# HybridRobotics/car-racing

Measured on AMD Instinct MI355X. Metric: NLP solves/sec (N=12, 6-state bicycle); p50 per-step solve latency, higher is better.
Workload: dtype f64

## Files before the change

car-racing_amd/csrc/crx_api.hip:

```cpp
#include <hip/hip_runtime.h>
#include <math.h>
#include <stdarg.h>
#include <stdio.h>
#include <string.h>

#include <dlfcn.h>

#include <chrono>
#include <mutex>
#include <vector>

#if __has_include(<rccl/rccl.h>)
#include <rccl/rccl.h>
#else
extern "C" {
typedef struct ncclComm* ncclComm_t;
typedef struct { char internal[128]; } ncclUniqueId;
typedef enum { ncclSuccess = 0 } ncclResult_t;
typedef enum { ncclInt8 = 0, ncclUint8 = 1, ncclInt32 = 2, ncclUint32 = 3, ncclInt64 = 4, ncclUint64 = 5, ncclFloat16 = 6, ncclFloat32 = 7, ncclFloat64 = 8 } ncclDataType_t;
}
#endif

#include "crx_kparams.h"

namespace {

thread_local char g_err[512] = "";
std::mutex g_mu;
int g_device = -1;
bool g_init = false;
hipStream_t g_stream = nullptr;

int fail(int code, const char* fmt, ...) {
    va_list ap;
    va_start(ap, fmt);
    vsnprintf(g_err, sizeof(g_err), fmt, ap);
    va_end(ap);
    return code;
}

#define HIP_TRY(expr)                                                                             \
    do {                                                                                          \
        hipError_t e_ = (expr);                                                                   \
        if (e_ != hipSuccess) return fail(CRX_ERR_HIP, "%s: %s", #expr, hipGetErrorString(e_));   \
    } while (0)

struct DevMem {
    static constexpr const char* name = "hipMalloc";
    static hipError_t alloc(void** p, size_t bytes) { return hipMalloc(p, bytes); }
    static hipError_t release(void* p) { return hipFree(p); }
};
struct PinMem {
    static constexpr const char* name = "hipHostMalloc";
    static hipError_t alloc(void** p, size_t bytes) { return hipHostMalloc(p, bytes, hipHostMallocDefault); }
    static hipError_t release(void* p) { return hipHostFree(p); }
};
template <typename Mem>
struct Buf {
    void* p = nullptr;
    size_t cap = 0;
    int ensure(size_t bytes) {
        if (bytes <= cap) return 0;
        release();
        size_t want = bytes + bytes / 2 + 256;
        hipError_t e = Mem::alloc(&p, want);
        if (e != hipSuccess) return fail(CRX_ERR_HIP, "%s(%zu): %s", Mem::name, want, hipGetErrorString(e));
        cap = want;
        return 0;
    }
    void release() {
        if (p) (void)Mem::release(p);
        p = nullptr;
        cap = 0;
    }
};
using DevBuf = Buf<DevMem>;
using PinBuf = Buf<PinMem>;
DevBuf g_in, g_out;
PinBuf g_hin, g_hout;
DevBuf g_trace;
int g_poison = 0;
int g_kkt_unscaled = 0;
int g_spec = 0;
int g_trace_rows = 0, g_trace_problem = 0;

int ensure_init() {
    if (g_init) return 0;
    return fail(CRX_ERR_NOT_INIT, "crx_init() has not been called (or failed)");
}

using arr = const void*;
template <typename... P>
bool any_null(const P*... p) { return (... || !p); }

struct Stage {
    enum Kind { IN, INOUT, OUT, SCRATCH };
    template <typename T>
    struct Ref { int i = -1; };
    struct Slot { Kind kind; const void* src; void* dst; size_t bytes, off; };
    static constexpr int MAX_SLOTS = 24;
    Slot slots[MAX_SLOTS];
    int n = 0;
    bool overrun = false;
    size_t end[4] = {0, 0, 0, 0};

    template <typename T>
    Ref<T> add(Kind kind, const T* src, T* dst, size_t count) {
        if (n == MAX_SLOTS) { overrun = true; return {}; }
        slots[n] = Slot{kind, src, dst, count * sizeof(T), 0};
        return Ref<T>{n++};
    }
    template <typename T>
    Ref<T> in(const T* src, size_t count) { return add(IN, src, (T*)nullptr, count); }
    template <typename T>
    Ref<T> out(T* host, size_t count) { return add(OUT, (const T*)nullptr, host, count); }
    template <typename T>
    Ref<T> inout(T* host, size_t count) { return add(INOUT, (const T*)host, host, count); }
    Ref<char> scratch(size_t bytes) { return add(SCRATCH, (const char*)nullptr, (char*)nullptr, bytes); }
    template <typename T>
    T* operator[](Ref<T> r) const {
        return r.i < 0 ? nullptr : (T*)((char*)(slots[r.i].kind == IN ? g_in.p : g_out.p) + slots[r.i].off);
    }

    int up(hipStream_t st) {
        if (overrun) return fail(CRX_ERR_ARG, "internal: more than %d staged arrays in one call", MAX_SLOTS);
        size_t cur = 0;
        for (int k = IN; k <= SCRATCH; k++) {
            if (k == INOUT) cur = 0;
            for (int i = 0; i < n; i++)
                if (slots[i].kind == k) {
                    slots[i].off = cur = (cur + 255) & ~size_t(255);
                    cur += slots[i].bytes;
                }
            end[k] = cur;
        }
        if (int rc = g_in.ensure(end[IN])) return rc;
        if (int rc = g_hin.ensure(end[IN])) return rc;
        if (int rc = g_out.ensure(end[SCRATCH])) return rc;
        if (int rc = g_hout.ensure(end[OUT])) return rc;
        for (int i = 0; i < n; i++) {
            const Slot& s = slots[i];
            if (s.kind > INOUT || !s.bytes) continue;
            char* pin = (char*)(s.kind == IN ? g_hin.p : g_hout.p) + s.off;
            if (s.src) memcpy(pin, s.src, s.bytes); else memset(pin, 0, s.bytes);
        }
        if (end[IN]) HIP_TRY(hipMemcpyAsync(g_in.p, g_hin.p, end[IN], hipMemcpyHostToDevice, st));
        if (end[INOUT]) HIP_TRY(hipMemcpyAsync(g_out.p, g_hout.p, end[INOUT], hipMemcpyHostToDevice, st));
        return 0;
    }
    int down(hipStream_t st) {
        if (end[OUT]) HIP_TRY(hipMemcpyAsync(g_hout.p, g_out.p, end[OUT], hipMemcpyDeviceToHost, st));
        HIP_TRY(hipStreamSynchronize(st));
        for (int i = 0; i < n; i++)
            if (slots[i].dst && slots[i].bytes) memcpy(slots[i].dst, (char*)g_hout.p + slots[i].off, slots[i].bytes);
        return 0;
    }
};

int check_opts(const crx_ipm_opts& o) {
    if (!(o.tol > 0) || o.max_iter < 1 || !(o.mu_init > 0) || !(o.tau_min > 0 && o.tau_min < 1) ||
        !(o.slack_push > 0) || !(o.kappa_mu > 0 && o.kappa_mu < 1) || !(o.theta_mu > 1) || !(o.grad_scale_max > 0) ||
        o.slack_start < 0 || o.slack_start > 3 || !(o.dual_inf_tol > 0) || !(o.constr_viol_tol > 0) || !(o.compl_inf_tol > 0) || o.stall_iters < 1 || o.qp_method < 0 || o.qp_method > 1)
        return fail(CRX_ERR_ARG, "invalid crx_ipm_opts (a descriptor built for libcrx <= 0.3.x? crx_ipm_opts grew in 0.2 and in 0.4: include/crx.h)");
    return 0;
}

void reach_bound(const double* A, const double* B, double delta_max, double a_max, int row, int n, double* gain, double (*rows)[6]) {
    double w[6] = {0, 0, 0, 0, 0, 0}, acc = 0.0;
    w[row] = 1.0;
    gain[0] = 0.0;
    if (rows) memcpy(rows[0], w, sizeof(w));
    for (int j = 1; j <= n; j++) {
        double v0 = 0.0, v1 = 0.0, wn[6] = {0, 0, 0, 0, 0, 0};
        for (int i = 0; i < 6; i++) { v0 += w[i] * B[i * 2]; v1 += w[i] * B[i * 2 + 1]; }
        acc += fabs(v0) * delta_max + fabs(v1) * a_max;
        gain[j] = acc;
        for (int a = 0; a < 6; a++)
            for (int i = 0; i < 6; i++) wn[a] += w[i] * A[i * 6 + a];
        memcpy(w, wn, sizeof(w));
        if (rows) memcpy(rows[j], w, sizeof(w));
    }
}

int fill_planner(crx_kparams& kp, const crx_planner_desc* d, int batch) {
    if (!d) return fail(CRX_ERR_ARG, "desc is NULL");
    if (d->N < 3 || d->N > CRX_MAX_N) return fail(CRX_ERR_ARG, "N=%d outside [3,%d]", d->N, CRX_MAX_N);
    if (batch < 0) return fail(CRX_ERR_ARG, "batch < 0");
    if (int rc = check_opts(d->opts)) return rc;
    memset(&kp, 0, sizeof(kp));
    kp.N = d->N; kp.batch = batch; kp.mode = 0; kp.n_obs_max = 0; kp.degree = 6;
    memcpy(kp.A, d->A, sizeof(kp.A)); memcpy(kp.B, d->B, sizeof(kp.B));
    kp.wq[4] = d->w_ref; kp.wq[5] = d->w_ref;
    kp.w_dey = d->w_dey; kp.w_prog = d->w_prog; kp.w_slack = 0.0;
    kp.delta_max = d->delta_max; kp.a_max = d->a_max; kp.v_min = -INFINITY; kp.v_max = d->vx_max; kp.ey_max = INFINITY;
    kp.alpha = 0.0; kp.margin = 0.0; kp.l_sum = 1.0; kp.w_sum = 1.0;
    kp.dt_ref = d->dt_ref; kp.fallback_gain = d->fallback_gain; kp.opts = d->opts;
    kp.reach_screen = d->opts.reach_screen ? 1 : 0;
    reach_bound(d->A, d->B, d->delta_max, d->a_max, 5, d->N - 1, kp.reach_gain, kp.reach_row);
    return 0;
}

int fill_cbf(crx_kparams& kp, const crx_cbf_desc* d, int batch) {
    if (!d) return fail(CRX_ERR_ARG, "desc is NULL");
    if (d->N < 3 || d->N > CRX_MAX_N) return fail(CRX_ERR_ARG, "N=%d outside [3,%d]", d->N, CRX_MAX_N);
    if (d->n_obs_max < 0 || d->n_obs_max > CRX_MAX_OBS) return fail(CRX_ERR_ARG, "n_obs_max=%d outside [0,%d]", d->n_obs_max, CRX_MAX_OBS);
    if (d->degree < 2 || d->degree > 8 || (d->degree & 1)) return fail(CRX_ERR_ARG, "degree must be 2, 4, 6 or 8");
    if (batch < 0) return fail(CRX_ERR_ARG, "batch < 0");
    if (!(d->alpha > 0.0 && d->alpha <= 1.0)) return fail(CRX_ERR_ARG, "alpha outside (0,1]");
    if (int rc = check_opts(d->opts)) return rc;
    memset(&kp, 0, sizeof(kp));
    kp.N = d->N; kp.batch = batch; kp.mode = 1; kp.per_stage_target = d->per_stage_target ? 1 : 0;
    kp.n_obs_max = d->n_obs_max; kp.degree = d->degree;
    memcpy(kp.A, d->A, sizeof(kp.A)); memcpy(kp.B, d->B, sizeof(kp.B));
    memcpy(kp.wq, d->Q, sizeof(kp.wq)); kp.wr[0] = d->R[0]; kp.wr[1] = d->R[1];
    kp.w_dey = 0.0; kp.w_prog = 0.0; kp.w_slack = d->w_slack;
    kp.delta_max = d->delta_max; kp.a_max = d->a_max; kp.v_min = d->v_min; kp.v_max = d->v_max; kp.ey_max = d->ey_max;
    kp.alpha = d->alpha; kp.margin = d->margin; kp.l_sum = d->l_sum; kp.w_sum = d->w_sum;
    kp.dt_ref = 0.1; kp.fallback_gain = 1.1; kp.opts = d->opts;
    kp.slack_start = d->opts.slack_start;
    reach_bound(d->A, d->B, d->delta_max, d->a_max, 4, d->N, kp.reach_s, nullptr);
    reach_bound(d->A, d->B, d->delta_max, d->a_max, 5, d->N, kp.reach_gain, nullptr);
    return 0;
}

int launched(hipError_t e, const char* what) {
    return e == hipSuccess ? CRX_OK : fail(CRX_ERR_HIP, "%s launch: %s", what, hipGetErrorString(e));
}

void apply_diagnostics(crx_kparams& kp) {
    if (g_trace_rows != 0) { kp.trace = (double*)g_trace.p; kp.trace_problem = g_trace_problem; kp.trace_rows = g_trace_rows; }
    kp.poison = g_poison;
    kp.kkt_unscaled = g_kkt_unscaled;
}
void apply_diagnostics(crx_lmpc_kparams& kp) {
    if (g_trace_rows > 0) { kp.trace = (double*)g_trace.p; kp.trace_problem = g_trace_problem; kp.trace_rows = g_trace_rows; }
    kp.poison = g_poison;
}

int launch_solve(const crx_kparams& kp, int tmpl, hipStream_t st) {
    crx_kparams kq = kp;
    apply_diagnostics(kq);
    size_t lds = crx_solve_lds_bytes(kp.N, tmpl);
    if (lds > 160 * 1024) return fail(CRX_ERR_ARG, "N=%d with %d obstacles needs %zu B of LDS (> 160 KiB)", kp.N, tmpl, lds);
    const bool spec = tmpl == 1 && kq.mode == 1 && kq.degree == 6 && (kq.N == 12 || kq.N == 10) && g_spec > 0;
    kq.spec_idle = g_spec == 2;
    return launched(spec ? crx_launch_solve_spec(kq, st) : crx_launch_solve(kq, tmpl, st), "solver");
}

}

extern "C" {

int crx_version(void) { return CRX_VERSION; }

const char* crx_last_error(void) { return g_err; }

int crx_device_count(void) {
    int n = 0;
    if (hipGetDeviceCount(&n) != hipSuccess) return 0;
    return n;
}

int crx_init(int device) {
    std::lock_guard<std::mutex> lk(g_mu);
    int n = 0;
    hipError_t e = hipGetDeviceCount(&n);
    if (e != hipSuccess || n <= 0)
        return fail(CRX_ERR_NO_DEVICE, "no HIP device visible (%s); libcrx has no CPU back-end",
                    e == hipSuccess ? "count = 0" : hipGetErrorString(e));
    if (device < 0 || device >= n) return fail(CRX_ERR_ARG, "device %d outside [0,%d)", device, n);
    HIP_TRY(hipSetDevice(device));
    if (g_init && g_device == device) return CRX_OK;
    if (g_init && g_device >= 0) {
        (void)hipSetDevice(g_device);
        if (g_stream) { (void)hipStreamDestroy(g_stream); g_stream = nullptr; }
        g_in.release(); g_out.release(); g_hin.release(); g_hout.release(); g_trace.release();
        g_trace_rows = 0;
        HIP_TRY(hipSetDevice(device));
    }
    HIP_TRY(hipStreamCreateWithFlags(&g_stream, hipStreamNonBlocking));
    g_device = device;
    g_init = true;
    return CRX_OK;
}

void crx_shutdown(void) {
    std::lock_guard<std::mutex> lk(g_mu);
    if (!g_init) return;
    (void)hipSetDevice(g_device);
    g_in.release(); g_out.release(); g_hin.release(); g_hout.release(); g_trace.release();
    g_trace_rows = 0;
    if (g_stream) (void)hipStreamDestroy(g_stream);
    g_stream = nullptr;
    g_init = false; g_device = -1;
}

int crx_trace_enable(int problem, int rows) {
    if (int rc = ensure_init()) return rc;
    g_trace_rows = 0;
    const bool sub = rows < 0;
    if (rows < 0) rows = -rows;
    if (rows == 0) return CRX_OK;
    if (int rc = g_trace.ensure((size_t)rows * 16 * sizeof(double))) return rc;
    HIP_TRY(hipMemset(g_trace.p, 0, (size_t)rows * 16 * sizeof(double)));
    g_trace_rows = sub ? -rows : rows; g_trace_problem = problem;
    return CRX_OK;
}
int crx_trace_read(double* host, int rows) {
    { int cap = g_trace_rows < 0 ? -g_trace_rows : g_trace_rows; if (rows > cap) rows = cap; }
    HIP_TRY(hipDeviceSynchronize());
    HIP_TRY(hipMemcpy(host, g_trace.p, (size_t)rows * 16 * sizeof(double), hipMemcpyDeviceToHost));
    return CRX_OK;
}

void crx_debug_poison_lds(int enable) { g_poison = enable != 0; }

void crx_debug_speculation(int mode) { g_spec = mode < 0 ? 0 : (mode > 2 ? 1 : mode); }

void crx_debug_kkt_unscaled(int mode) { g_kkt_unscaled = (mode >= 0 && mode <= 4) ? mode : 0; }

int crx_debug_wave_reduce(const double* in, double* out) {
    if (int rc = ensure_init()) return rc;
    if (!in || !out) return fail(CRX_ERR_ARG, "NULL array argument");
    std::lock_guard<std::mutex> lk(g_mu);
    HIP_TRY(hipSetDevice(g_device));
    Stage sg;
    auto din = sg.in(in, 256);
    auto dout = sg.out(out, 208);
    if (int rc = sg.up(g_stream)) return rc;
    hipError_t e = crx_launch_debug_reduce(sg[din], sg[dout], g_stream);
    if (e != hipSuccess) return fail(CRX_ERR_HIP, "debug reduce launch: %s", hipGetErrorString(e));
    return sg.down(g_stream);
}

long crx_debug_lds_bytes(int kind, int N, int n) {
    return kind == 0 ? (long)crx_solve_lds_bytes(N, n) : (long)crx_lmpc_lds_bytes(N, n);
}

int crx_debug_resident_per_cu(int kind, int N, int n) {
    if (ensure_init() != CRX_OK) return -1;
    return kind == 0 ? crx_solve_resident_per_cu(N, n) : crx_lmpc_resident_per_cu(N, n);
}

struct CrxTimer { hipEvent_t e0, e1; bool armed; };

int crx_timer_create(void** timer) {
    if (int rc = ensure_init()) return rc;
    if (!timer) return fail(CRX_ERR_ARG, "timer is NULL");
    HIP_TRY(hipSetDevice(g_device));
    CrxTimer* t = new CrxTimer{nullptr, nullptr, false};
    if (hipEventCreate(&t->e0) != hipSuccess || hipEventCreate(&t->e1) != hipSuccess) {
        if (t->e0) (void)hipEventDestroy(t->e0);
        delete t;
        return fail(CRX_ERR_HIP, "hipEventCreate failed");
    }
    *timer = t;
    return CRX_OK;
}
int crx_timer_destroy(void* timer) {
    CrxTimer* t = (CrxTimer*)timer;
    if (!t) return CRX_OK;
    (void)hipEventDestroy(t->e0); (void)hipEventDestroy(t->e1);
    delete t;
    return CRX_OK;
}
int crx_timer_begin(void* timer, void* stream) {
    CrxTimer* t = (CrxTimer*)timer;
    if (!t) return fail(CRX_ERR_ARG, "timer is NULL");
    t->armed = false;
    HIP_TRY(hipEventRecord(t->e0, (hipStream_t)stream));
    return CRX_OK;
}
int crx_timer_end(void* timer, void* stream) {
    CrxTimer* t = (CrxTimer*)timer;
    if (!t) return fail(CRX_ERR_ARG, "timer is NULL");
    HIP_TRY(hipEventRecord(t->e1, (hipStream_t)stream));
    t->armed = true;
    return CRX_OK;
}
double crx_timer_ms(void* timer) {
    CrxTimer* t = (CrxTimer*)timer;
    if (!t || !t->armed) return -1.0;
    float ms = 0.f;
    if (hipEventSynchronize(t->e1) != hipSuccess) return -1.0;
    if (hipEventElapsedTime(&ms, t->e0, t->e1) != hipSuccess) return -1.0;
    return (double)ms;
}

void crx_ipm_opts_default(crx_ipm_opts* o) {
    o->tol = 1e-8; o->max_iter = 200; o->restore_iters = 50; o->mu_init = 0.1; o->kappa_eps = 10.0;
    o->kappa_mu = 0.2; o->theta_mu = 1.5; o->tau_min = 0.99; o->slack_push = 1e-2; o->grad_scale_max = 100.0;
    o->reach_screen = 1; o->slack_start = 2;
    o->dual_inf_tol = 1.0; o->constr_viol_tol = 1e-4; o->compl_inf_tol = 1e-4;
    o->stall_iters = 100; o->qp_method = 0;
}

void crx_planner_desc_default(crx_planner_desc* d, int N, const double* A, const double* B) {
    memset(d, 0, sizeof(*d));
    d->N = N;
    memcpy(d->A, A, sizeof(d->A)); memcpy(d->B, B, sizeof(d->B));
    d->w_ref = 20.0; d->w_dey = 30.0; d->w_prog = 200.0; d->vx_max = 5.0; d->delta_max = 0.5; d->a_max = 1.5;
    d->dt_ref = 0.1; d->fallback_gain = 1.1;
    crx_ipm_opts_default(&d->opts);
}

void crx_cbf_desc_default(crx_cbf_desc* d, int N, int n_obs_max, const double* A, const double* B) {
    memset(d, 0, sizeof(*d));
    d->N = N; d->n_obs_max = n_obs_max; d->per_stage_target = 0; d->degree = 6;
    memcpy(d->A, A, sizeof(d->A)); memcpy(d->B, B, sizeof(d->B));
    const double Q[6] = {10.0, 0.0, 0.0, 4.0, 0.0, 40.0};
    memcpy(d->Q, Q, sizeof(Q)); d->R[0] = 0.1; d->R[1] = 0.1;
    d->delta_max = 0.5; d->a_max = 1.0; d->v_min = 0.0; d->v_max = 10.0; d->ey_max = 1.0;
    d->alpha = 0.8; d->margin = 0.2; d->l_sum = 0.4; d->w_sum = 0.2; d->w_slack = 1e4;
    crx_ipm_opts_default(&d->opts);
    if (N <= 12 && n_obs_max <= 1) { d->opts.stall_iters = 50; d->opts.restore_iters = 25; }
}

void crx_select_desc_default(crx_select_desc* d, int N, int n_veh_max, double lap_length) {
    d->N = N; d->n_veh_max = n_veh_max; d->veh_length = 0.4; d->veh_width = 0.2; d->lap_length = lap_length;
    d->w_prog = 10.0; d->w_coll = 100.0; d->w_switch = 100.0;
}

static bool planner_null(arr x0, arr bez_s, arr bez_ey, arr ey_lb, arr ey_ub, arr X, arr U, arr cost, arr status, arr kkt, arr iters) {
    return any_null(x0, bez_s, bez_ey, ey_lb, ey_ub, X, U, cost, status, kkt, iters);
}

static int check_planner(crx_kparams& kp, const crx_planner_desc* d, int batch, arr x0, arr bez_s, arr bez_ey, arr ey_lb, arr ey_ub, arr X, arr U,
                         arr cost, arr status, arr kkt, arr iters) {
    if (int rc = ensure_init()) return rc;
    if (int rc = fill_planner(kp, d, batch)) return rc;
    if (batch > 0 && planner_null(x0, bez_s, bez_ey, ey_lb, ey_ub, X, U, cost, status, kkt, iters))
        return fail(CRX_ERR_ARG, "NULL array argument");
    return 0;
}

static int planner_solve_masked(const crx_planner_desc* d, int batch, const int32_t* active, int active_div, const double* x0,
                                const double* bez_s, const double* bez_ey, const double* ey_lb, const double* ey_ub, double* X,
                                double* U, double* cost, int32_t* status, double* kkt, int32_t* iters, void* stream);

int crx_planner_solve_dev(const crx_planner_desc* d, int batch, const double* x0, const double* bez_s,
                          const double* bez_ey, const double* ey_lb, const double* ey_ub, double* X, double* U,
                          double* cost, int32_t* status, double* kkt, int32_t* iters, void* stream) {
    return planner_solve_masked(d, batch, nullptr, 0, x0, bez_s, bez_ey, ey_lb, ey_ub, X, U, cost, status, kkt, iters, stream);
}

static int planner_solve_masked(const crx_planner_desc* d, int batch, const int32_t* active, int active_div, const double* x0,
                                const double* bez_s, const double* bez_ey, const double* ey_lb, const double* ey_ub, double* X,
                                double* U, double* cost, int32_t* status, double* kkt, int32_t* iters, void* stream) {
    crx_kparams kp;
    if (int rc = check_planner(kp, d, batch, x0, bez_s, bez_ey, ey_lb, ey_ub, X, U, cost, status, kkt, iters)) return rc;
    if (batch == 0) return CRX_OK;
    kp.x0 = x0; kp.bez_s = bez_s; kp.bez_ey = bez_ey; kp.ey_lb = ey_lb; kp.ey_ub = ey_ub;
    kp.X = X; kp.U = U; kp.sigma = nullptr; kp.cost = cost; kp.status = status; kp.kkt = kkt; kp.iters = iters;
    kp.active = active; kp.active_div = active_div;
    return launch_solve(kp, 0, (hipStream_t)stream);
}

int crx_planner_solve(const crx_planner_desc* d, int batch, const double* x0, const double* bez_s,
                      const double* bez_ey, const double* ey_lb, const double* ey_ub, double* X, double* U,
                      double* cost, int32_t* status, double* kkt, int32_t* iters) {
    crx_kparams chk;
    if (int rc = check_planner(chk, d, batch, x0, bez_s, bez_ey, ey_lb, ey_ub, X, U, cost, status, kkt, iters)) return rc;
    if (batch == 0) return CRX_OK;
    std::lock_guard<std::mutex> lk(g_mu);
    HIP_TRY(hipSetDevice(g_device));
    const size_t B = (size_t)batch, N = (size_t)d->N;
    Stage sg;
    auto dx0 = sg.in(x0, B * 6); auto dbs = sg.in(bez_s, B * (N + 1)); auto dbe = sg.in(bez_ey, B * (N + 1));
    auto dlb = sg.in(ey_lb, B * N); auto dub = sg.in(ey_ub, B);
    auto dX = sg.out(X, B * (N + 1) * 6); auto dU = sg.out(U, B * N * 2); auto dc = sg.out(cost, B);
    auto dk = sg.out(kkt, B); auto ds = sg.out(status, B); auto di = sg.out(iters, B);
    if (int rc = sg.up(g_stream)) return rc;
    if (int rc = crx_planner_solve_dev(d, batch, sg[dx0], sg[dbs], sg[dbe], sg[dlb], sg[dub], sg[dX], sg[dU], sg[dc], sg[ds], sg[dk],
                                       sg[di], g_stream)) return rc;
    return sg.down(g_stream);
}

int crx_cbf_solve_dev(const crx_cbf_desc* d, int batch, const double* x0, const double* xt, const double* obs_s,
                      const double* obs_ey, const double* lap_off, const int32_t* n_obs, double* X, double* U,
                      double* sigma, double* cost, int32_t* status, double* kkt, int32_t* iters, void* stream) {
    return crx_cbf_solve_masked_dev(d, batch, nullptr, x0, xt, obs_s, obs_ey, lap_off, n_obs, X, U, sigma, cost, status, kkt, iters, stream);
}

int crx_cbf_solve_masked_dev(const crx_cbf_desc* d, int batch, const int32_t* active, const double* x0, const double* xt,
                             const double* obs_s, const double* obs_ey, const double* lap_off, const int32_t* n_obs, double* X,
                             double* U, double* sigma, double* cost, int32_t* status, double* kkt, int32_t* iters, void* stream) {
    return crx_cbf_solve_ordered_dev(d, batch, active, nullptr, x0, xt, obs_s, obs_ey, lap_off, n_obs, nullptr, X, U, sigma, cost, status, kkt, iters, stream);
}

int crx_cbf_solve_dims_dev(const crx_cbf_desc* d, int batch, const int32_t* active, const double* x0, const double* xt,
                           const double* obs_s, const double* obs_ey, const double* lap_off, const int32_t* n_obs,
                           const double* obs_dims, double* X, double* U, double* sigma, double* cost, int32_t* status, double* kkt,
                           int32_t* iters, void* stream) {
    return crx_cbf_solve_ordered_dev(d, batch, active, nullptr, x0, xt, obs_s, obs_ey, lap_off, n_obs, obs_dims, X, U, sigma, cost, status, kkt, iters, stream);
}

static int check_cbf(crx_kparams& kp, const crx_cbf_desc* d, int batch, arr x0, arr xt, arr obs_s, arr obs_ey, arr lap_off, arr n_obs, arr X, arr U,
                     arr sigma, arr cost, arr status, arr kkt, arr iters) {
    if (int rc = ensure_init()) return rc;
    if (int rc = fill_cbf(kp, d, batch)) return rc;
    if (batch == 0) return 0;
    if (any_null(x0, xt, X, U, cost, status, kkt, iters)) return fail(CRX_ERR_ARG, "NULL array argument");
    if (d->n_obs_max > 0 && any_null(obs_s, obs_ey, lap_off, n_obs, sigma))
        return fail(CRX_ERR_ARG, "NULL obstacle array with n_obs_max > 0");
    return 0;
}

int crx_cbf_solve_ordered_dev(const crx_cbf_desc* d, int batch, const int32_t* active, const int32_t* order, const double* x0,
                              const double* xt, const double* obs_s, const double* obs_ey, const double* lap_off,
                              const int32_t* n_obs, const double* obs_dims, double* X, double* U, double* sigma, double* cost,
                              int32_t* status, double* kkt, int32_t* iters, void* stream) {
    crx_kparams kp;
    if (int rc = check_cbf(kp, d, batch, x0, xt, obs_s, obs_ey, lap_off, n_obs, X, U, sigma, cost, status, kkt, iters)) return rc;
    if (batch == 0) return CRX_OK;
    kp.x0 = x0; kp.xt = xt; kp.obs_s = obs_s; kp.obs_ey = obs_ey; kp.lap_off = lap_off; kp.n_obs = n_obs;
    kp.X = X; kp.U = U; kp.sigma = sigma; kp.cost = cost; kp.status = status; kp.kkt = kkt; kp.iters = iters;
    kp.active = active; kp.order = order; kp.obs_dims = d->n_obs_max > 0 ? obs_dims : nullptr;
    return launch_solve(kp, d->n_obs_max, (hipStream_t)stream);
}

int crx_cbf_solve(const crx_cbf_desc* d, int batch, const double* x0, const double* xt, const double* obs_s,
                  const double* obs_ey, const double* lap_off, const int32_t* n_obs, double* X, double* U,
                  double* sigma, double* cost, int32_t* status, double* kkt, int32_t* iters) {
    return crx_cbf_solve_dims(d, batch, x0, xt, obs_s, obs_ey, lap_off, n_obs, nullptr, X, U, sigma, cost, status, kkt, iters);
}

int crx_cbf_solve_dims(const crx_cbf_desc* d, int batch, const double* x0, const double* xt, const double* obs_s,
                  const double* obs_ey, const double* lap_off, const int32_t* n_obs, const double* obs_dims, double* X, double* U,
                  double* sigma, double* cost, int32_t* status, double* kkt, int32_t* iters) {
    crx_kparams chk;
    if (int rc = check_cbf(chk, d, batch, x0, xt, obs_s, obs_ey, lap_off, n_obs, X, U, sigma, cost, status, kkt, iters)) return rc;
    if (batch == 0) return CRX_OK;
    const size_t B = (size_t)batch, N = (size_t)d->N, V = (size_t)d->n_obs_max;
    if (V > 0) {
        for (size_t b = 0; b < B; b++)
            if (n_obs[b] < 0 || n_obs[b] > (int)V) return fail(CRX_ERR_ARG, "n_obs[%zu]=%d outside [0,%zu]", b, n_obs[b], V);
        if (obs_dims)
            for (size_t b = 0; b < B; b++)
                for (int o = 0; o < n_obs[b]; o++)
                    if (!(obs_dims[(b * V + o) * 2] > 0.0) || !(obs_dims[(b * V + o) * 2 + 1] > 0.0))
                        return fail(CRX_ERR_ARG, "obs_dims[%zu][%d] must be positive", b, o);
    }
    std::lock_guard<std::mutex> lk(g_mu);
    HIP_TRY(hipSetDevice(g_device));
    const size_t n_ob = B * V * (N + 1);
    Stage sg;
    auto dx0 = sg.in(x0, B * 6); auto dxt = sg.in(xt, d->per_stage_target ? B * (N + 1) * 6 : B * 6);
    auto dos = sg.in(obs_s, n_ob); auto doe = sg.in(obs_ey, n_ob); auto dlo = sg.in(lap_off, B * V);
    auto ddm = (obs_dims && V > 0) ? sg.in(obs_dims, B * V * 2) : Stage::Ref<double>{};
    auto dno = sg.in(V > 0 ? n_obs : (const int32_t*)nullptr, B);
    auto dX = sg.out(X, B * (N + 1) * 6); auto dU = sg.out(U, B * N * 2); auto dsg = sg.out(sigma, n_ob);
    auto dc = sg.out(cost, B); auto dk = sg.out(kkt, B); auto ds = sg.out(status, B); auto di = sg.out(iters, B);
    if (int rc = sg.up(g_stream)) return rc;
    if (int rc = crx_cbf_solve_dims_dev(d, batch, nullptr, sg[dx0], sg[dxt], sg[dos], sg[doe], sg[dlo], sg[dno], sg[ddm], sg[dX], sg[dU],
                                        sg[dsg], sg[dc], sg[ds], sg[dk], sg[di], g_stream)) return rc;
    return sg.down(g_stream);
}

static int check_select(const crx_select_desc* d, int n_scen) {
    if (!d) return fail(CRX_ERR_ARG, "desc is NULL");
    if (d->N < 1 || d->N > CRX_MAX_N || d->n_veh_max < 0 || d->n_veh_max > CRX_MAX_VEH || n_scen < 0)
        return fail(CRX_ERR_ARG, "bad selection dimensions");
    if (!(d->lap_length > 0.0) || !isfinite(d->lap_length)) return fail(CRX_ERR_ARG, "lap_length must be positive and finite");
    if (!(d->veh_length >= 0.0) || !(d->veh_width >= 0.0)) return fail(CRX_ERR_ARG, "vehicle dimensions must be non-negative");
    return 0;
}

static bool select_null(const crx_select_desc* d, arr n_veh, arr X, arr obs_s, arr obs_ey, arr old_flag, arr flag, arr sel_cost, arr best_X) {
    return any_null(n_veh, X, old_flag, flag, sel_cost, best_X) || (d->n_veh_max > 0 && any_null(obs_s, obs_ey));
}

static int check_select_call(const crx_select_desc* d, int n_scen, arr n_veh, arr X, arr obs_s, arr obs_ey, arr old_flag, arr flag, arr sel_cost,
                             arr best_X) {
    if (int rc = ensure_init()) return rc;
    if (int rc = check_select(d, n_scen)) return rc;
    if (n_scen > 0 && select_null(d, n_veh, X, obs_s, obs_ey, old_flag, flag, sel_cost, best_X)) return fail(CRX_ERR_ARG, "NULL array argument");
    return 0;
}

int crx_select_dev(const crx_select_desc* d, int n_scen, const int32_t* n_veh, const double* X, const double* obs_s,
                   const double* obs_ey, const int32_t* old_flag, int32_t* flag, double* sel_cost, double* best_X,
                   void* stream) {
    if (int rc = check_select_call(d, n_scen, n_veh, X, obs_s, obs_ey, old_flag, flag, sel_cost, best_X)) return rc;
    if (n_scen == 0) return CRX_OK;
    crx_select_kparams sp;
    sp.N = d->N; sp.V = d->n_veh_max; sp.n_scen = n_scen;
    sp.veh_length = d->veh_length; sp.veh_width = d->veh_width; sp.lap_length = d->lap_length;
    sp.w_prog = d->w_prog; sp.w_coll = d->w_coll; sp.w_switch = d->w_switch;
    sp.n_veh = n_veh; sp.X = X; sp.obs_s = obs_s; sp.obs_ey = obs_ey; sp.old_flag = old_flag;
    sp.flag = flag; sp.sel_cost = sel_cost; sp.best_X = best_X;
    return launched(crx_launch_select(sp, (hipStream_t)stream), "selection");
}

int crx_select(const crx_select_desc* d, int n_scen, const int32_t* n_veh, const double* X, const double* obs_s,
               const double* obs_ey, const int32_t* old_flag, int32_t* flag, double* sel_cost, double* best_X) {
    if (int rc = check_select_call(d, n_scen, n_veh, X, obs_s, obs_ey, old_flag, flag, sel_cost, best_X)) return rc;
    if (n_scen == 0) return CRX_OK;
    const size_t S = (size_t)n_scen, N = (size_t)d->N, V = (size_t)d->n_veh_max, R = V + 1;
    for (size_t s = 0; s < S; s++)
        if (n_veh[s] < 0 || n_veh[s] > (int)V) return fail(CRX_ERR_ARG, "n_veh[%zu]=%d outside [0,%zu]", s, n_veh[s], V);
    std::lock_guard<std::mutex> lk(g_mu);
    HIP_TRY(hipSetDevice(g_device));
    Stage sg;
    auto dX = sg.in(X, S * R * (N + 1) * 6); auto dos = sg.in(obs_s, S * V * (N + 1)); auto doe = sg.in(obs_ey, S * V * (N + 1));
    auto dnv = sg.in(n_veh, S); auto dof = sg.in(old_flag, S);
    auto dfl = sg.out(flag, S); auto dsc = sg.out(sel_cost, S * R); auto dbX = sg.out(best_X, S * (N + 1) * 6);
    if (int rc = sg.up(g_stream)) return rc;
    if (int rc = crx_select_dev(d, n_scen, sg[dnv], sg[dX], sg[dos], sg[doe], sg[dof], sg[dfl], sg[dsc], sg[dbX], g_stream)) return rc;
    return sg.down(g_stream);
}

void crx_path_desc_default(crx_path_desc* d, int N, double alpha) {
    memset(d, 0, sizeof(*d));
    d->N = N; d->alpha = alpha; d->w_rate = 100.0;
    crx_ipm_opts_default(&d->opts);
}

static int fill_path(crx_path_kparams& pp, const crx_path_desc* d, int batch) {
    if (!d) return fail(CRX_ERR_ARG, "desc is NULL");
    if (d->N < 2 || d->N > CRX_MAX_N) return fail(CRX_ERR_ARG, "N=%d outside [2,%d]", d->N, CRX_MAX_N);
    if (!(d->alpha >= 0.0 && d->alpha <= 1.0) || !(d->w_rate >= 0.0)) return fail(CRX_ERR_ARG, "alpha outside [0,1] or w_rate < 0");
    if (batch < 0) return fail(CRX_ERR_ARG, "batch < 0");
    if (int rc = check_opts(d->opts)) return rc;
    memset(&pp, 0, sizeof(pp));
    pp.N = d->N; pp.batch = batch; pp.alpha = d->alpha; pp.w_rate = d->w_rate; pp.opts = d->opts;
    return 0;
}

static int check_path(crx_path_kparams& pp, const crx_path_desc* d, int batch, arr opt, arr bez, arr lb, arr ub, arr e0, arr eN, arr E, arr cost,
                      arr status, arr kkt, arr iters) {
    if (int rc = ensure_init()) return rc;
    if (int rc = fill_path(pp, d, batch)) return rc;
    if (batch > 0 && any_null(opt, bez, lb, ub, e0, eN, E, cost, status, kkt, iters)) return fail(CRX_ERR_ARG, "NULL array argument");
    return 0;
}

int crx_path_solve_dev(const crx_path_desc* d, int batch, const double* opt, const double* bez, const double* lb,
                       const double* ub, const double* e0, const double* eN, double* E, double* cost, int32_t* status,
                       double* kkt, int32_t* iters, void* stream) {
    crx_path_kparams pp;
    if (int rc = check_path(pp, d, batch, opt, bez, lb, ub, e0, eN, E, cost, status, kkt, iters)) return rc;
    if (batch == 0) return CRX_OK;
    pp.opt = opt; pp.bez = bez; pp.lb = lb; pp.ub = ub; pp.e0 = e0; pp.eN = eN;
// ... 942 lines not shown
```

car-racing_amd/csrc/crx_kernels.hip:

```cpp
#include <hip/hip_runtime.h>
#include <math.h>
#include <stdint.h>
#include <type_traits>

#include "crx_kparams.h"
#include "crx_wave.h"
#include "crx_num.h"
#include "crx_ipm.h"

#ifndef CRX_TU_GENERAL
#define CRX_TU_GENERAL 0
#endif
#ifndef CRX_OPAQUE_LANE
#define CRX_OPAQUE_LANE 1
#endif
#ifndef CRX_STATIC_LDS
#define CRX_STATIC_LDS 1
#endif
#ifndef CRX_SWEEP_MASK
#define CRX_SWEEP_MASK 1
#endif
#ifndef CRX_SWEEP_LOCAL_LANE
#define CRX_SWEEP_LOCAL_LANE 1
#endif
#define MAXF 12

__device__ __forceinline__ double ipow_d(double a, int p) {
    const double a2 = a * a;
    const int h = p >> 1;
    double r = sel(p & 1, a, 1.0);
    r = sel(h >= 1, r * a2, r);
    r = sel(h >= 2, r * a2, r);
    r = sel(h >= 3, r * a2, r);
    r = sel(h >= 4, r * a2, r);
    asm volatile("" : "+v"(r));
    return r;
}

#define ROWS(j, jv, lane_, m_) _Pragma("unroll") for (int q_ = 0; q_ < (L::MR + WAVE - 1) / WAVE; q_++) \
    if (const bool jv = (lane_) + q_ * WAVE < (m_); true) if (const int j = jv ? (lane_) + q_ * WAVE : 0; true)

#define COORDS(e, ev, lane_, n_) _Pragma("unroll") for (int q_ = 0; q_ < (L::NV + WAVE - 1) / WAVE; q_++) \
    if (const bool ev = (lane_) + q_ * WAVE < (n_); true) if (const int e = ev ? (lane_) + q_ * WAVE : 0; true)

#define SINK(cond, off) seli((cond), (off), L::dmy)
#define CBF_ROWS(j, k, ob, ev, lane_, n_) _Pragma("unroll") for (int q_ = 0; q_ < (NMAX * NOBS + WAVE - 1) / WAVE; q_++) \
    if (const bool ev = (lane_) + q_ * WAVE < (n_) * NOBS; true) if (const int e_ = ev ? (lane_) + q_ * WAVE : 0; true) \
    if (const int k = e_ / L::NO; true) if (const int ob = e_ - k * L::NO; true) if (const int j = k * NR + 8 + NOBS + ob; true)
#define ROW_LOADS_DONE() do { if (NOBS == 0) __builtin_amdgcn_sched_barrier(0); } while (0)
#define ROW_IS_CBF(j, n_) (NOBS > 0 && (j) < (n_) * NR && (j) % NR >= 8 + NOBS)
#define LOADS_DONE() __builtin_amdgcn_sched_barrier(0)
#define STAGE_FENCE() __builtin_amdgcn_sched_barrier(0)

#define RIV_SIMPLE (1 << 13)
#define RIV_NEG (1 << 14)
#define RIV_IDX(pk) ((pk) & 0x1FFF)
#define RIV_SGN(pk) (((pk) & RIV_SIMPLE) ? (((pk) & RIV_NEG) ? -1.0 : 1.0) : 0.0)
#define SH16(si_) ((unsigned short*)((si_) + L::SH_OFF))
#define RIVT(si_, j) ((int)SH16(si_)[L::riv + (j)])
#define UPDP(si_, l_) ((int)SH16(si_)[L::updP + (l_)])
#define VROW(si_) ((typename L::vrow_t*)(SH16(si_) + L::END_S16))

template <int NOBS, int NMAX>
struct Lay {
    static constexpr int NX = 6 + NOBS, NU = 2 + NOBS, NZ = NX + NU, NR = 8 + 2 * NOBS;
    static constexpr int NO = NOBS ? NOBS : 1;
    static constexpr int MR = NMAX * NR + NOBS;
    static constexpr int NV = (NMAX + 1) * NZ;
    static constexpr int M = 0;
    static constexpr int Z = M + NX * NZ;
    static constexpr int dZ = Z + NV;
    static constexpr int xr = dZ + NV;
    static constexpr int wc = xr + (NMAX + 1) * 6;
    static constexpr int obs_s = wc + NMAX;
    static constexpr int obs_e = obs_s + NOBS * (NMAX + 1);
    static constexpr int rt = obs_e + NOBS * (NMAX + 1);
    static constexpr int rnu = rt + MR;
    static constexpr int rc = rnu + MR;
    static constexpr int rdt = rc + MR;
    static constexpr int rtt = rdt + MR;
    static constexpr bool SLIM = NOBS == 3 && NMAX == 20;
    static constexpr int MRS = SLIM ? 0 : MR;
    static constexpr int rsig = rtt + MR;
    static constexpr int rw = rsig + MRS;
    static constexpr int rsc = rw + MRS;
    static constexpr int csc = rsc + MRS;
    static constexpr int rb = csc + (SLIM ? NMAX * NOBS : 0);
    static constexpr int Gpos = rb + MRS;
    static constexpr int Hd = Gpos + (SLIM ? 0 : NMAX * NOBS * 4);
    static constexpr int hg = Hd + NV;
    static constexpr int ga = hg;
    static constexpr int Jc = hg + NV;
    static constexpr int kS = (Jc + NMAX * NOBS * NZ + 1) & ~1;
    static constexpr int kE = kS + 1;
    static constexpr int HS = NZ + 1;
    static constexpr int TS = NZ;
    static constexpr bool PT_ALIAS = NX * NX + NX + NX * TS <= MR, H_ALIAS = NZ * HS <= NV;
    static constexpr int WORK = kS + (NOBS ? 2 * NMAX : 0);
    static constexpr int P = PT_ALIAS ? rdt : WORK;
    static constexpr int pv = P + NX * NX;
    static constexpr int T = pv + NX;
    static constexpr int WORK2 = PT_ALIAS ? WORK : T + NX * TS;
    static constexpr int H = H_ALIAS ? dZ : WORK2;
    static constexpr int Kk = H_ALIAS ? WORK2 : H + NZ * HS;
    static constexpr int G = SLIM ? Kk : Gpos;
    static constexpr int sigS = (SLIM && H_ALIAS && NZ * HS + NMAX * NO <= NV) ? dZ + NZ * HS : -1;
    static_assert(NMAX * NOBS * 4 <= NMAX * NU * NX, "G fits inside Kk");
    static constexpr int kf = Kk + NMAX * NU * NX;
    static constexpr int Fth = kf + NMAX * NU;
    static constexpr int Fph = Fth + MAXF;
    static constexpr int cst = Fph + MAXF;
    static constexpr int dmy = cst + 16 + 2 * NOBS;
    static constexpr int END_D = dmy + 2;
    static constexpr int triH = 0;
    static constexpr int END_I = triH + ((NZ * NZ <= WAVE || SLIM) ? 0 : NZ * (NZ + 1) / 2);
    static constexpr int SH_OFF = (END_I + 1) & ~1;
    static constexpr int riv = 0;
    static constexpr int updP = riv + MR;
    static constexpr int UCNT = (NX * (NX + 1) / 2 + NX + NX + 1 + WAVE - 1) / WAVE;
    static constexpr int END_S16 = (updP + 64 * UCNT + 1) & ~1;
    using vrow_t = std::conditional_t<(MR <= 127), signed char, short>;
    static constexpr int vlo = 0;
    static constexpr int vhi = vlo + NV;
    static constexpr int END_V = SLIM ? 0 : vhi + NV;
    static constexpr size_t BYTES = (size_t)END_D * 8 + (size_t)SH_OFF * 4 + (size_t)END_S16 * 2 + (((size_t)END_V * sizeof(vrow_t) + 7) & ~(size_t)7);
    static_assert(!SLIM || BYTES <= 40960, "the slim layout exists to fit four problems per CU (160 KB / 4)");
    static constexpr int R2 = (int)((BYTES + 15) / 16) * 2;
    static constexpr int P2 = R2, pv2 = P2 + NX * NX, T2 = pv2 + NX, H2 = (T2 + NX * TS + 1) & ~1, Kk2 = H2 + NZ * HS, kf2 = Kk2 + NMAX * NU * NX,
                         dZ2 = kf2 + NMAX * NU, ctl = dZ2 + NZ, R2_END = ctl + 4;
    static constexpr size_t BYTES_SPEC = (size_t)R2_END * 8;
};

struct Ctx {
    int N, lane, nobs, m;
    double lin_sN, cconst, wsig, alpha, om, cm;
    int degree;
    double b_d, b_a, b_vlo, b_vhi, b_e;
};

template <class L>
__device__ __forceinline__ double row_scale(const double* sm, const int* si, int j, int N) {
    if constexpr (L::SLIM) {
        const bool cbf = j < N * L::NR && j % L::NR >= 8 + L::NO;
        const int k = j / L::NR, ob = j - k * L::NR - 8 - L::NO;
        const double cs = sm[L::csc + seli(cbf, k * L::NO + ob, 0)];
        return sel(cbf, cs, sel((RIVT(si, j) & RIV_SIMPLE) != 0, 1.0, 0.0));
    } else {
        return sm[L::rsc + j];
    }
}
template <class L>
__device__ __forceinline__ double cbf_scale(const double* sm, int k, int ob) {
    if constexpr (L::SLIM) return sm[L::csc + k * L::NO + ob];
    else return sm[L::rsc + k * L::NR + 8 + L::NO + ob];
}
template <class L>
__device__ __forceinline__ double row_bound(const double* sm, const Ctx& c, int j) {
    if constexpr (L::SLIM) {
        const int r = j < c.N * L::NR ? j % L::NR : 8;
        const double ub = sel(r < 2, c.b_d, c.b_a) * sel((r & 1) != 0, 1.0, -1.0);
        const double xb = sel(r == 4, c.b_vlo, sel(r == 5, c.b_vhi, sel(r == 6, -c.b_e, c.b_e)));
        return sel(r < 4, ub, sel(r < 8, xb, 0.0));
    } else {
        return sm[L::rb + j];
    }
}
template <class L>
__device__ __forceinline__ void row_sig_w(const double* sm, int j, bool on, double mu, double t, double nu, double rti, double cj,
                                          double& sig, double& w) {
    if constexpr (L::SLIM) {
        const double sg = nu * rti;
        sig = sel(on, sg, 0.0);
        w = sel(on, nu - mu * rti + sg * (cj - t), 0.0);
    } else {
        sig = sm[L::rsig + j];
        w = sm[L::rw + j];
    }
}
template <class L>
__device__ __forceinline__ void coord_rows(const int* si, const Ctx& c, int e, int k, int a, int& rl, int& rh) {
    if constexpr (L::SLIM) {
        constexpr int NX = L::NX, NR = L::NR;
        const int N = c.N;
        const bool isx = a < 6, iss0 = a >= 6 && a < NX, isu = a >= NX && a < NX + 2;
        const bool xb = isx && k >= 1 && (a == 0 || a == 5);
        int jl = seli(xb, (k - 1) * NR + seli(a == 0, 4, 6), -1);
        jl = seli(iss0 && k == 0, N * NR + (a - 6), jl);
        jl = seli(isu && k < N, k * NR + 2 * (a - NX), jl);
        jl = seli(a >= NX + 2 && k < N, k * NR + 8 + (a - NX - 2), jl);
        const int jh = seli(xb || (isu && k < N), jl + 1, -1);
        rl = seli(jl >= 0 && (RIVT(si, seli(jl >= 0, jl, 0)) & RIV_SIMPLE) != 0, jl, -1);
        rh = seli(jh >= 0 && (RIVT(si, seli(jh >= 0, jh, 0)) & RIV_SIMPLE) != 0, jh, -1);
    } else {
        rl = VROW(si)[L::vlo + e];
        rh = VROW(si)[L::vhi + e];
    }
}
__device__ __forceinline__ void tri_decode(int e, int& r, int& a) {
    int q = (int)((__builtin_sqrtf(8.0f * (float)e + 1.0f) - 1.0f) * 0.5f);
    q += ((q + 1) * (q + 2) / 2 <= e) ? 1 : 0;
    q -= (q * (q + 1) / 2 > e) ? 1 : 0;
    r = q; a = e - q * (q + 1) / 2;
}

#define LD(off) sm[(off)]
#ifndef CRX_ROWDPP
#define CRX_ROWDPP 1
#endif
template <class L> constexpr bool ROWDPP = CRX_ROWDPP && L::NZ <= 16;

#ifdef CRX_PHASE_CLOCKS
#define CLK() clock64()
#else
#define CLK() 0LL
#endif

template <int NOBS, int NMAX>
__device__ __forceinline__ void cbf_dist(const double* sm, const Ctx& c, int k, int o, double al, double& dsc,
                                         double& dec, double& dsn, double& den) {
    using L = Lay<NOBS, NMAX>;
    const int N1 = c.N + 1;
    const double sc = LD(L::Z + k * L::NZ + 4) + al * LD(L::dZ + k * L::NZ + 4);
    const double ec = LD(L::Z + k * L::NZ + 5) + al * LD(L::dZ + k * L::NZ + 5);
    const double sn = LD(L::Z + (k + 1) * L::NZ + 4) + al * LD(L::dZ + (k + 1) * L::NZ + 4);
    const double en = LD(L::Z + (k + 1) * L::NZ + 5) + al * LD(L::dZ + (k + 1) * L::NZ + 5);
    const double rLs = LD(L::cst + 16 + o), rWs = LD(L::cst + 16 + L::NO + o);
    dsc = (sc - LD(L::obs_s + o * N1 + k) - LD(L::cst + 8 + o)) * rLs;
    dec = (ec - LD(L::obs_e + o * N1 + k)) * rWs;
    dsn = (sn - LD(L::obs_s + o * N1 + k + 1)) * rLs;
    den = (en - LD(L::obs_e + o * N1 + k + 1)) * rWs;
}

template <int NOBS, int NMAX>
__device__ __forceinline__ double cbf_value(const double* sm, const Ctx& c, int k, int o, double al) {
    using L = Lay<NOBS, NMAX>;
    double dsc, dec, dsn, den;
    cbf_dist<NOBS, NMAX>(sm, c, k, o, al, dsc, dec, dsn, den);
    const int q = c.degree;
    const double gc = ipow_d(dsc, q) + ipow_d(dec, q), gn = ipow_d(dsn, q) + ipow_d(den, q);
    const double sk = LD(L::Z + k * L::NZ + 6 + o) + al * LD(L::dZ + k * L::NZ + 6 + o);
    const double sk1 = LD(L::Z + k * L::NZ + L::NX + 2 + o) + al * LD(L::dZ + k * L::NZ + L::NX + 2 + o);
    return gn - sk1 - c.om * (gc - sk) - c.alpha * c.cm;
}

template <int NOBS, int NMAX>
__device__ __forceinline__ double cost_value(const double* sm, const Ctx& c, double al) {
    using L = Lay<NOBS, NMAX>;
    const int N = c.N;
    double acc = 0.0;
    for (int e = c.lane; e < (N + 1) * 6; e += WAVE) {
        const int k = e / 6, i = e - k * 6;
        const double v = LD(L::Z + k * L::NZ + i) + al * LD(L::dZ + k * L::NZ + i);
        const double d = v - LD(L::xr + e);
        acc += LD(L::cst + i) * d * d;
        if (k == N && i == 4) acc += c.lin_sN * v;
    }
    for (int e = c.lane; e < N * 2; e += WAVE) {
        const int k = e >> 1, i = e & 1;
        const double v = LD(L::Z + k * L::NZ + L::NX + i) + al * LD(L::dZ + k * L::NZ + L::NX + i);
        acc += LD(L::cst + 6 + i) * v * v;
    }
    for (int k = c.lane; k < N; k += WAVE) {
        const double wck = LD(L::wc + k);
        const double e1 = LD(L::Z + (k + 1) * L::NZ + 5) + al * LD(L::dZ + (k + 1) * L::NZ + 5);
        const double e0 = LD(L::Z + k * L::NZ + 5) + al * LD(L::dZ + k * L::NZ + 5);
        acc += wck * (e1 - e0) * (e1 - e0);
    }
    if (NOBS) {
        for (int e = c.lane; e < (N + 1) * NOBS; e += WAVE) {
            const int k = e / L::NO, o = e - k * L::NO;
            if (o < c.nobs) acc += c.wsig * (LD(L::Z + k * L::NZ + 6 + o) + al * LD(L::dZ + k * L::NZ + 6 + o));
        }
    }
    return wave_sum(acc) + c.cconst;
}

template <int NOBS, int NMAX>
__device__ __forceinline__ double cost_dir(const double* sm, const Ctx& c, double& qq) {
    using L = Lay<NOBS, NMAX>;
    const int N = c.N;
    double acc = 0.0, q = 0.0;
    COORDS(e, ev, c.lane, N * L::NZ + L::NX) {
        const int k = e / L::NZ, a = e - k * L::NZ;
        const bool isx = a < 6, isu = a >= L::NX && a < L::NX + 2, iss0 = a >= 6 && a < L::NX;
        const bool cpl = a == 5 && k >= 1;
        const double dv = LD(L::dZ + e), z = LD(L::Z + e);
        const double w = sel(isx || isu, LD(L::cst + (isx ? a : (isu ? 6 + a - L::NX : 0))), 0.0);
        const double ref = sel(isx, LD(L::xr + k * 6 + (isx ? a : 0)), 0.0);
        const int ep = seli(cpl, e - L::NZ, e);
        const double de = z - LD(L::Z + ep), dd = dv - LD(L::dZ + ep);
        const double wk = sel(cpl, LD(L::wc + seli(cpl, k - 1, 0)), 0.0);
        double t = 2.0 * (w * (z - ref) * dv + wk * de * dd);
        t += sel(k == N && a == 4, c.lin_sN * dv, 0.0);
        if (NOBS) t += sel(iss0 && a - 6 < c.nobs, c.wsig * dv, 0.0);
        acc += sel(ev, t, 0.0);
        q += sel(ev, w * dv * dv + wk * dd * dd, 0.0);
    }
    qq = q;
    return acc;
}

template <int NOBS, int NMAX>
__device__ __forceinline__ void eval_rows(double* sm, const int* si, const Ctx& c) {
    using L = Lay<NOBS, NMAX>;
    for (int j = c.lane; j < c.m; j += WAVE) {
        const double sc = row_scale<L>(sm, si, j, c.N);
        const int pk = RIVT(si, j);
        double v = RIV_SGN(pk) * (LD(L::Z + RIV_IDX(pk)) - row_bound<L>(sm, c, j));
        if (NOBS && j < c.N * L::NR) {
            const int k = j / L::NR, r = j - k * L::NR;
            if (r >= 8 + NOBS && sc != 0.0) v = sc * cbf_value<NOBS, NMAX>(sm, c, k, r - 8 - NOBS, 0.0);
        }
        LD(L::rc + j) = (sc != 0.0) ? v : 1.0;
    }
}

template <int NOBS, int NMAX>
__device__ __forceinline__ void first_order(double* sm, const int* si, const Ctx& c) {
    using L = Lay<NOBS, NMAX>;
    const int N = c.N;
    if (NOBS) {
#pragma unroll
        for (int q_ = 0; q_ < (NMAX * NOBS + WAVE - 1) / WAVE; q_++) {
            const int e0 = c.lane + q_ * WAVE;
            const int e = e0 < N * NOBS ? e0 : 0;
            const int k = e / L::NO, o = e - k * L::NO;
            double* G = sm + L::G + (k * L::NO + o) * 4;
            double* J = sm + L::Jc + (k * L::NO + o) * L::NZ;
            const bool here = o < c.nobs;
            double dsc, dec, dsn, den;
            cbf_dist<NOBS, NMAX>(sm, c, k, o, 0.0, dsc, dec, dsn, den);
            const int q = c.degree;
            const double qd = (double)q, qq = (double)(q * (q - 1));
            const double p2sn = ipow_d(dsn, q - 2), p2en = ipow_d(den, q - 2);
            const double p2sc = ipow_d(dsc, q - 2), p2ec = ipow_d(dec, q - 2);
            const double rLs = LD(L::cst + 16 + o), rWs = LD(L::cst + 16 + L::NO + o);
            const double gsn = qd * p2sn * dsn * rLs, gen = qd * p2en * den * rWs;
            const double gsc = qd * p2sc * dsc * rLs, gec = qd * p2ec * dec * rWs;
            const double d = cbf_scale<L>(sm, k, o);
            double m4[L::NZ], m5[L::NZ];
#pragma unroll
            for (int a = 0; a < L::NZ; a++) { m4[a] = LD(L::M + 4 * L::NZ + a); m5[a] = LD(L::M + 5 * L::NZ + a); }
            G[0] = sel(here, qq * p2sn * rLs * rLs, 0.0); G[1] = sel(here, qq * p2en * rWs * rWs, 0.0);
            G[2] = sel(here, qq * p2sc * rLs * rLs, 0.0); G[3] = sel(here, qq * p2ec * rWs * rWs, 0.0);
#pragma unroll
            for (int a = 0; a < L::NZ; a++) {
                double v = d * (gsn * m4[a] + gen * m5[a]);
                if (a == 4) v -= d * c.om * gsc;
                if (a == 5) v -= d * c.om * gec;
                v += sel(a == 6 + o, d * c.om, 0.0);
                v -= sel(a == L::NX + 2 + o, d, 0.0);
                J[a] = sel(here, v, 0.0);
            }
        }
        SYNC();
    }
    COORDS(e, ev, c.lane, N * L::NZ + L::NX) {
        (void)ev;
        const int k = e / L::NZ, a = e - k * L::NZ;
        const bool isx = a < 6, isu = a >= L::NX && a < L::NX + 2, iss0 = a >= 6 && a < L::NX, iss1 = a >= L::NX + 2;
        const int o = iss0 ? a - 6 : (iss1 ? a - L::NX - 2 : 0);
        const bool sig_on = (o < c.nobs) && ((iss0 && k == 0) || (iss1 && k < N));
        const double cw = LD(L::cst + (isx ? a : (isu ? 6 + a - L::NX : 0))), xrv = LD(L::xr + k * 6 + (isx ? a : 0));
        const double w2 = sel(isx || isu, 2.0 * cw, 0.0);
        const double ref = sel(isx, xrv, 0.0);
        double g = w2 * (LD(L::Z + e) - ref);
        g += (k == N && a == 4) ? c.lin_sN : 0.0;
        g += sig_on ? c.wsig : 0.0;
        int rl, rh;
        coord_rows<L>(si, c, e, k, a, rl, rh);
        const double nl = LD(L::rnu + (rl >= 0 ? rl : 0)), nh = LD(L::rnu + (rh >= 0 ? rh : 0));
        g -= sel(rl >= 0, nl, 0.0);
        g += sel(rh >= 0, nh, 0.0);
        const int kk = k < N ? k : N - 1;
        if (NOBS == 0) {
            const double de = LD(L::Z + (kk + 1) * L::NZ + 5) - LD(L::Z + kk * L::NZ + 5);
            const double wck = LD(L::wc + kk), m5 = LD(L::M + 5 * L::NZ + a);
            g += sel(k < N, 2.0 * wck * de * (m5 - (a == 5 ? 1.0 : 0.0)), 0.0);
        } else {
#pragma unroll
            for (int ob = 0; ob < NOBS; ob++) {
                const double nuv = LD(L::rnu + kk * L::NR + 8 + NOBS + ob), jv2 = LD(L::Jc + (kk * L::NO + ob) * L::NZ + a);
                g -= sel(k < N, nuv * jv2, 0.0);
            }
        }
        g = (k == N && a >= L::NX) ? 0.0 : g;
        LD(L::ga + e) = g;
    }
    SYNC();
}

template <int NOBS, int NMAX, int UNR = 1>
__device__ __forceinline__ double dual_infeasibility(double* sm, const Ctx& c) {
    using L = Lay<NOBS, NMAX>;
    const int N = c.N;
    int lane = c.lane;
#if CRX_SWEEP_LOCAL_LANE & 2
    if (NOBS > 0) asm volatile("" : "+v"(lane));
#endif
    double emax = 0.0;
    double tot = 0.0;
    if (!CRX_SWEEP_MASK || lane < L::NZ) {
    constexpr bool MK = CRX_SWEEP_MASK;
    const bool in = MK || lane < L::NZ;
    const int la = in ? lane : 0;
    double mcol[L::NX];
#pragma unroll
    for (int i = 0; i < L::NX; i++) mcol[i] = LD(L::M + i * L::NZ + la);
    tot = LD(L::ga + N * L::NZ + la);
    double gk = LD(L::ga + (N - 1) * L::NZ + la);
    LD(SINK(in, L::ga + N * L::NZ + lane)) = 0.0;
    auto stage = [&](int k) {
        const double gn = LD(L::ga + (k >= 1 ? k - 1 : 0) * L::NZ + la);
        double t = gk;
        if constexpr (ROWDPP<L>) {
            t = row_dot<L::NX, 0>(tot, mcol, t);
        } else {
#pragma unroll
            for (int i = 0; i < L::NX; i++) t += mcol[i] * lane_f64(tot, i);
        }
        tot = t;
        emax = fmax(emax, sel(lane >= L::NX && in, fabs(tot), 0.0));
        const bool keep = lane >= L::NX || (k == 0 && lane >= 6);
        LD(SINK(in, L::ga + k * L::NZ + lane)) = sel(keep, tot, 0.0);
        gk = gn;
        STAGE_FENCE();
    };
    if constexpr (UNR > 1) {
#pragma unroll UNR
        for (int k = N - 1; k >= 0; k--) stage(k);
    } else {
        for (int k = N - 1; k >= 0; k--) stage(k);
    }
    }
    SYNC();
    if (NOBS && lane >= 6 && lane < 6 + c.nobs) emax = fmax(emax, fabs(tot));
    return wave_max(emax);
}

template <int NOBS, int NMAX>
__device__ __forceinline__ double box_certificate(double* sm, const int* si, const Ctx& c, double delta_max, double a_max) {
    using L = Lay<NOBS, NMAX>;
    const int N = c.N, lane = c.lane;
    double S = 0.0;
    COORDS(e, ev, lane, N * L::NZ + L::NX) {
        const int k = e / L::NZ, a = e - k * L::NZ;
        const int rl = VROW(si)[L::vlo + e], rh = VROW(si)[L::vhi + e];
        const int il = rl >= 0 ? rl : 0, ih = rh >= 0 ? rh : 0;
        const double nl = LD(L::rnu + il), nh = LD(L::rnu + ih), cl = LD(L::rc + il), ch = LD(L::rc + ih);
        const bool st = ev && a < 6;
        const bool hl = st && rl >= 0, hh = st && rh >= 0;
        S += sel(hl, nl * cl, 0.0) + sel(hh, nh * ch, 0.0);
        LD(SINK(ev, L::dZ + e)) = sel(hh, nh, 0.0) - sel(hl, nl, 0.0);
        (void)k;
    }
    SYNC();
    double mcol[L::NX];
#pragma unroll
    for (int i = 0; i < L::NX; i++) mcol[i] = LD(L::M + i * L::NZ + (lane < L::NZ ? lane : 0));
    const int la = lane < L::NZ ? lane : 0;
    const bool isu = lane >= L::NX && lane < L::NX + 2;
    const double hi = lane == L::NX ? delta_max : a_max;
    double tot = LD(L::dZ + N * L::NZ + la);
    double gk = LD(L::dZ + (N - 1) * L::NZ + la), uk = LD(L::Z + (N - 1) * L::NZ + la);
    for (int k = N - 1; k >= 0; k--) {
        const int kn = k >= 1 ? k - 1 : 0;
        const double gn = LD(L::dZ + kn * L::NZ + la), un = LD(L::Z + kn * L::NZ + la);
        double t = gk;
        if constexpr (ROWDPP<L>) {
            t = row_dot<L::NX, 0>(tot, mcol, t);
        } else {
#pragma unroll
            for (int i = 0; i < L::NX; i++) t += mcol[i] * lane_f64(tot, i);
        }
        tot = t;
        const double w = -tot;
        S += sel(isu, w * (sel(w > 0.0, hi, -hi) - uk), 0.0);
        gk = gn; uk = un;
    }
    SYNC();
    return wave_sum(S);
}

template <int NOBS, int NMAX>
__device__ __forceinline__ void assemble_newton(double* sm, const int* si, const Ctx& c, double mu) {
    using L = Lay<NOBS, NMAX>;
    const int N = c.N;
    ROWS(j, jv, c.lane, c.m) {
        (void)jv;
        const double t = LD(L::rt + j), nu = LD(L::rnu + j);
        const double rti = frcp(t);
        LD(L::rtt + j) = rti;
        if constexpr (!L::SLIM) {
            const double sig = nu * rti;
            const bool on = LD(L::rsc + j) != 0.0;
            LD(L::rsig + j) = sel(on, sig, 0.0);
            const double cj = LD(L::rc + j);
            LD(L::rw + j) = sel(on, nu - mu * rti + sig * (cj - t), 0.0);
        } else {
            const bool on = row_scale<L>(sm, si, j, N) != 0.0;
            const double sg = nu * rti, cj = LD(L::rc + j);
            LD(L::rdt + j) = sel(on, nu - mu * rti + sg * (cj - t), 0.0);
        }
    }
    SYNC();
    COORDS(e, ev, c.lane, N * L::NZ + L::NX) {
        const int k = e / L::NZ, a = e - k * L::NZ;
        const bool isx = a < 6, isu = a >= L::NX && a < L::NX + 2, iss0 = a >= 6 && a < L::NX, iss1 = a >= L::NX + 2;
        const int o = iss0 ? a - 6 : (iss1 ? a - L::NX - 2 : 0);
        double g = LD(L::ga + e);
        const double cw = LD(L::cst + (isx ? a : (isu ? 6 + a - L::NX : 0)));
        double h = sel(isx || isu, 2.0 * cw, 0.0);
        h += ((iss0 && k == 0 && o >= c.nobs) || (iss1 && o >= c.nobs)) ? 1.0 : 0.0;
        int rl, rh;
        coord_rows<L>(si, c, e, k, a, rl, rh);
        const int il = rl >= 0 ? rl : 0, ih = rh >= 0 ? rh : 0;
        double sgl, sgh, wl, wh;
        if constexpr (L::SLIM) {
            sgl = LD(L::rnu + il) * LD(L::rtt + il); wl = LD(L::rdt + il);
            sgh = LD(L::rnu + ih) * LD(L::rtt + ih); wh = LD(L::rdt + ih);
        } else {
            sgl = LD(L::rsig + il); sgh = LD(L::rsig + ih); wl = LD(L::rw + il); wh = LD(L::rw + ih);
        }
        h += sel(rl >= 0, sgl, 0.0) + sel(rh >= 0, sgh, 0.0);
        g += sel(rl >= 0, wl, 0.0) - sel(rh >= 0, wh, 0.0);
        if (NOBS) {
            const int kk = k < N ? k : N - 1;
#pragma unroll
            for (int ob = 0; ob < NOBS; ob++) {
                const int j = kk * L::NR + 8 + NOBS + ob;
                const double csj = cbf_scale<L>(sm, kk, ob);
                const double jca = LD(L::Jc + (kk * L::NO + ob) * L::NZ + a);
                double rsj_, rwj;
                if constexpr (L::SLIM) {
                    rwj = LD(L::rdt + j);
                } else {
                    row_sig_w<L>(sm, j, csj != 0.0, mu, LD(L::rt + j), LD(L::rnu + j), LD(L::rtt + j), LD(L::rc + j), rsj_, rwj);
                    (void)rsj_;
                }
                g += sel(k < N, jca * rwj, 0.0);
                const double cur = LD(L::rnu + j) * csj * c.om * LD(L::G + (kk * L::NO + ob) * 4 + (a == 4 ? 2 : 3));
                h += sel(k < N && (a == 4 || a == 5), cur, 0.0);
            }
        }
        const bool tail = k == N && a >= L::NX;
        LD(L::Hd + e) = sel(tail, 0.0, h);
        LD(SINK(ev, L::hg + e)) = sel(tail, 0.0, g);
    }
    if (NOBS) {
        const int k = c.lane < N ? c.lane : 0;
        double ks = 0.0, ke = 0.0;
#pragma unroll
        for (int o = 0; o < NOBS; o++) {
            const int j = k * L::NR + 8 + NOBS + o;
            const double nd = LD(L::rnu + j) * cbf_scale<L>(sm, k, o);
            ks -= nd * LD(L::G + (k * L::NO + o) * 4 + 0);
            ke -= nd * LD(L::G + (k * L::NO + o) * 4 + 1);
            if constexpr (L::sigS >= 0) LD(L::sigS + k * L::NO + o) = sel(LD(L::csc + k * L::NO + o) != 0.0, LD(L::rnu + j) * LD(L::rtt + j), 0.0);
        }
        LD(L::kS + 2 * k) = ks;
        LD(L::kE + 2 * k) = ke;
    }
    SYNC();
}

template <int NOBS, int NMAX, int UNR = 1, int REG = 0, bool CVX = false, bool KEEPF = false>
__device__ __forceinline__ bool riccati_backward(double* sm, const int* si, const Ctx& c, double dw, long long* tsub = nullptr, bool convex = false) {
    using L = Lay<NOBS, NMAX>;
    constexpr int NX = L::NX, NU = L::NU, NZ = L::NZ, HS = L::HS;
    constexpr int oP = REG ? L::P2 : L::P, opv = REG ? L::pv2 : L::pv, oT = REG ? L::T2 : L::T, oH = REG ? L::H2 : L::H, oKk = REG ? L::Kk2 : L::Kk,
                  okf = REG ? L::kf2 : L::kf, odZ = REG ? L::dZ2 : L::dZ;
    const int N = c.N, lane = c.lane;
    const long long qs = CLK();
    constexpr bool PTR = ROWDPP<L> && L::UCNT == 1 && NX <= 7;
    constexpr bool PREG = !PTR && ROWDPP<L> && L::UCNT == 1;
    constexpr int PVF = (NX * 8) & 15;
    static_assert(!PTR || (NX * 8) / 16 == 3, "p sits in DPP row 3, where hv is formed");
    int lo = lane;
    if constexpr (PTR) asm volatile("" : "+v"(lo));
    const int g8 = lo >> 3, c8 = lo & 7;
    const bool isPm = g8 < NX && c8 < NX, isPv = g8 == NX && c8 < NX;
    double preg = 0.0, pn = 0.0;
    {
        double kSn = NOBS ? LD(L::kS + 2 * (N - 1)) : 0.0, kEn = NOBS ? LD(L::kE + 2 * (N - 1)) : 0.0;
        if constexpr (CVX) { kSn = sel(convex, 0.0, kSn); kEn = sel(convex, 0.0, kEn); }
        kEn += 2.0 * LD(L::wc + N - 1);
        if constexpr (PTR) {
            const double hd = LD(L::Hd + N * NZ + seli(isPm, g8, 0));
            const double hgN = LD(L::hg + N * NZ + seli(c8 < NX, c8, 0));
            pn = sel(isPv, hgN, sel(isPm && g8 == c8, hd + sel(g8 == 4, kSn, sel(g8 == 5, kEn, 0.0)), 0.0));
            if (NOBS) {
                LD(SINK(lo < NX, oT + lo * L::TS + 6)) = 0.0;
                LD(SINK(isPm && c8 == 6, oT + g8 * L::TS + NX + 2)) = pn;
            }
        } else {
#pragma unroll
            for (int q_ = 0; q_ < (NX * NX + WAVE - 1) / WAVE; q_++) {
                const int e0 = lane + q_ * WAVE;
                const int e = e0 < NX * NX ? e0 : 0;
                const int i = e / NX, j = e - i * NX;
                const double hd = LD(L::Hd + N * NZ + i);
                LD(oP + e) = sel(i == j, hd + sel(i == 4, kSn, sel(i == 5, kEn, 0.0)), 0.0);
            }
            const double hgN = LD(L::hg + N * NZ + (lane < NX ? lane : 0));
            LD(SINK(lane < NX, opv + lane)) = hgN;
            preg = hgN;
        }
    }
    SYNC();
    bool ok = true;
    constexpr bool FULL = NZ * NZ <= WAVE;
    constexpr int NTRI = FULL ? NZ * NZ : NZ * (NZ + 1) / 2;
    constexpr int HCNT = (NTRI + WAVE - 1) / WAVE;
    int hr[HCNT], ha[HCNT], hst[HCNT];
#pragma unroll
    for (int q = 0; q < HCNT; q++) {
        const int e0 = lane + q * WAVE;
        const int e = e0 < NTRI ? e0 : 0;
        if (FULL) { hr[q] = e / NZ; ha[q] = e - hr[q] * NZ; }
        else if constexpr (L::SLIM) tri_decode(e, hr[q], ha[q]);
        else { const int pk = si[L::triH + e]; hr[q] = pk >> 8; ha[q] = pk & 255; }
        hst[q] = SINK(e0 < NTRI, oH + hr[q] * HS + ha[q]);
    }
    const bool hvl = PTR ? (lane >= 48 && lane < 48 + NZ) : lane < NZ;
    const int lz = hvl ? (PTR ? lane - 48 : lane) : 0;
    const int hvst = SINK(hvl, oH + lz * HS + NZ);
    constexpr int TCNT = (NX * 8 + WAVE - 1) / WAVE;
    double mT[TCNT][6], mH[HCNT][NX];
    int tld[TCNT], tst[TCNT];
#pragma unroll
    for (int q = 0; q < TCNT; q++) {
        const int e = lane + q * WAVE;
        const int cc = e & 7;
        const int a = cc < 6 ? cc : NX + (cc - 6);
        const int i = (e >> 3) < NX ? (e >> 3) : 0;
        tld[q] = oP + i * NX;
        tst[q] = SINK(e < NX * 8, oT + i * L::TS + a);
#pragma unroll
        for (int j = 0; j < 6; j++) mT[q][j] = LD(L::M + j * NZ + a);
    }
#pragma unroll
    for (int q = 0; q < HCNT; q++)
#pragma unroll
        for (int i = 0; i < NX; i++) mH[q][i] = LD(L::M + i * NZ + hr[q]);
    double m5a[HCNT], m5r[HCNT];
#pragma unroll
    for (int q = 0; q < HCNT; q++) { m5a[q] = NOBS ? 0.0 : LD(L::M + 5 * NZ + ha[q]); m5r[q] = NOBS ? 0.0 : LD(L::M + 5 * NZ + hr[q]); }
    double mz[NX];
#pragma unroll
    for (int i = 0; i < NX; i++) mz[i] = LD(L::M + i * NZ + lz);
    constexpr int T2CNT = NOBS ? (NX * 2 * NOBS + WAVE - 1) / WAVE : 1;
    int t2ld[T2CNT], t2st[T2CNT];
    bool t2nxt[T2CNT];
#pragma unroll
    for (int q = 0; q < T2CNT; q++) {
        t2ld[q] = oP; t2st[q] = L::dmy; t2nxt[q] = false;
        if (NOBS) {
            const int l2 = lane + q * WAVE;
            const bool v2 = l2 < NX * 2 * NOBS;
            const int e2 = v2 ? l2 : 0;
            const int i2 = e2 / (2 * L::NO), cc = e2 - i2 * (2 * L::NO);
            t2nxt[q] = cc >= NOBS;
            const int o = t2nxt[q] ? cc - NOBS : cc;
            t2ld[q] = oP + i2 * NX + 6 + o;
            t2st[q] = SINK(v2, oT + i2 * L::TS + seli(t2nxt[q], NX + 2 + o, 6 + o));
        }
    }
    constexpr int NP = NX * (NX + 1) / 2 + NX, UCNT = L::UCNT;
    int yiA[UCNT], yjA[UCNT], s0A[UCNT], pst1[UCNT], pst2[UCNT], kstr[UCNT], kstep[UCNT], kst[UCNT];
    bool exSl[UCNT], exEl[UCNT];
    double mSl[UCNT], mEl[UCNT], mdg[HCNT];
#pragma unroll
    for (int q = 0; q < HCNT; q++) mdg[q] = hr[q] == ha[q] ? 1.0 : 0.0;
#pragma unroll
    for (int q = 0; q < UCNT; q++) {
        const int l = lane + q * WAVE;
        int ui, uj; bool isP, isK;
        if constexpr (PTR) {
            isP = isPm || isPv;
            isK = NX == 7 ? c8 == 7 : (g8 == 7 && c8 <= NX);
            ui = seli(isPm, g8 < c8 ? g8 : c8, seli(isPv, c8, 0));
            uj = seli(isPm, g8 < c8 ? c8 : g8, seli(isPv, NX, seli(isK, NX == 7 ? g8 : c8, 0)));
        } else {
            const int upk = UPDP(si, l);
            ui = upk >> 8; uj = upk & 255;
            isP = l < NP; isK = !isP && l < NP + NX + 1;
        }
        const bool gcol = uj >= NX;
        const int ujj = gcol ? NZ : uj;
        yiA[q] = oH + NX * HS + ui; yjA[q] = oH + NX * HS + ujj;
        s0A[q] = FULL ? oH + ui * HS + ujj : seli(gcol, oH + ui * HS + ujj, oH + uj * HS + ui);
        pst1[q] = SINK(isP, seli(gcol, opv + ui, oP + ui * NX + uj));
        pst2[q] = SINK(isP, seli(gcol, opv + ui, oP + uj * NX + ui));
        kstr[q] = seli(isK, seli(gcol, 1, NX), 0); kstep[q] = seli(isK, seli(gcol, NU, NU * NX), 0);
        kst[q] = SINK(isK, seli(gcol, okf, oKk + uj) + (N - 1) * kstep[q]);
        exSl[q] = isP && !gcol && ui == uj && ui == 4; exEl[q] = isP && !gcol && ui == uj && ui == 5;
        mSl[q] = exSl[q] ? 1.0 : 0.0; mEl[q] = exEl[q] ? 1.0 : 0.0;
    }
    if (tsub) tsub[2] += CLK() - qs;
#pragma unroll UNR
    for (int k = N - 1; k >= 0; k--) {
        long long q0 = CLK();
        if constexpr (PTR) {
            __builtin_amdgcn_wave_barrier();
            LD(tst[0]) = halfrow_dot6(pn, mT[0], (lane & 8) != 0);
        } else {
            double pl[TCNT][6];
#pragma unroll
            for (int q = 0; q < TCNT; q++)
#pragma unroll
                for (int j = 0; j < 6; j++) pl[q][j] = LD(tld[q] + j);
            double p2[T2CNT];
#pragma unroll
            for (int q = 0; q < T2CNT; q++) p2[q] = NOBS ? LD(t2ld[q]) : 0.0;
            LOADS_DONE();
#pragma unroll
            for (int q = 0; q < TCNT; q++) {
                double t = 0.0;
#pragma unroll
                for (int j = 0; j < 6; j++) t += pl[q][j] * mT[q][j];
                LD(tst[q]) = t;
            }
            if (NOBS) {
#pragma unroll
                for (int q = 0; q < T2CNT; q++) LD(t2st[q]) = sel(t2nxt[q], p2[q], 0.0);
            }
        }
        SYNC();
        long long q1 = CLK();
        {
            double hvs = LD(L::hg + k * NZ + lz), pvv[NX];
            if constexpr (PTR) __builtin_amdgcn_sched_barrier(0);
            const double kc = (NOBS == 0) ? 2.0 * LD(L::wc + k) : 0.0;
            double tc[HCNT][NX], hd[HCNT], jr[HCNT][L::NO], ja[HCNT][L::NO], rs[L::NO];
#pragma unroll
            for (int q = 0; q < HCNT; q++) {
#pragma unroll
                for (int i = 0; i < NX; i++) tc[q][i] = LD(oT + i * L::TS + ha[q]);
                hd[q] = LD(L::Hd + k * NZ + hr[q]);
                if (NOBS) {
#pragma unroll
                    for (int o = 0; o < NOBS; o++) {
                        jr[q][o] = LD(L::Jc + (k * L::NO + o) * NZ + hr[q]);
                        ja[q][o] = LD(L::Jc + (k * L::NO + o) * NZ + ha[q]);
                    }
                }
            }
            if (NOBS) {
#pragma unroll
                for (int o = 0; o < NOBS; o++) {
                    if constexpr (L::sigS >= 0) {
                        rs[o] = LD(L::sigS + k * L::NO + o);
                    } else if constexpr (L::SLIM) {
                        const int j = k * L::NR + 8 + NOBS + o;
                        rs[o] = sel(LD(L::csc + k * L::NO + o) != 0.0, LD(L::rnu + j) * LD(L::rtt + j), 0.0);
                    } else {
                        rs[o] = LD(L::rsig + k * L::NR + 8 + NOBS + o);
                    }
                }
            }
            if constexpr (!PREG && !PTR) {
#pragma unroll
                for (int i = 0; i < NX; i++) pvv[i] = LD(opv + i);
            }
            LOADS_DONE();
            if constexpr (PTR) {
                hvs = row_dot<NX, PVF>(pn, mz, hvs);
                __builtin_amdgcn_sched_barrier(0);
            }
            double hs[HCNT];
#pragma unroll
            for (int q = 0; q < HCNT; q++) {
                const int r = hr[q], a = ha[q];
                double t = 0.0;
#pragma unroll
                for (int i = 0; i < NX; i++) t += mH[q][i] * tc[q][i];
                const double dg = hd[q] + sel(r >= NX || (k == 0 && r >= 6), dw, 0.0);
                t = fma(mdg[q], dg, t);
                if (NOBS) {
#pragma unroll
                    for (int o = 0; o < NOBS; o++) t += rs[o] * jr[q][o] * ja[q][o];
                } else {
                    t -= kc * (sel(r == 5, m5a[q], 0.0) + sel(a == 5, m5r[q], 0.0) - ((r == 5 && a == 5) ? 1.0 : 0.0));
                }
                hs[q] = t;
            }
            if constexpr (PTR) {
            } else if constexpr (PREG) {
                hvs = row_dot<NX, 0>(preg, mz, hvs);
            } else {
#pragma unroll
                for (int i = 0; i < NX; i++) hvs += mz[i] * pvv[i];
            }
#pragma unroll
            for (int q = 0; q < HCNT; q++) LD(hst[q]) = hs[q];
            LD(hvst) = hvs;
        }
        SYNC();
        long long q2 = CLK();
        {
            double Lf[NU][NU], Dp[NU], rD[NU], yi[UCNT][NU], yj[UCNT][NU], t[UCNT];
#pragma unroll
            for (int a = 0; a < NU; a++)
#pragma unroll
                for (int b2 = 0; b2 <= a; b2++) Lf[a][b2] = LD(oH + (NX + a) * HS + NX + b2);
            __builtin_amdgcn_sched_barrier(0);
#pragma unroll
            for (int q = 0; q < UCNT; q++) {
#pragma unroll
                for (int a = 0; a < NU; a++) { yi[q][a] = LD(yiA[q] + a * HS); yj[q][a] = LD(yjA[q] + a * HS); }
                t[q] = LD(s0A[q]);
            }
            const int km = k >= 1 ? k - 1 : 0;
            double kSv = NOBS ? LD(L::kS + 2 * km) : 0.0, kEv = NOBS ? LD(L::kE + 2 * km) : 0.0;
            const double wcv = NOBS ? 0.0 : LD(L::wc + km);
            if constexpr (CVX) { kSv = sel(convex, 0.0, kSv); kEv = sel(convex, 0.0, kEv); }
            LOADS_DONE();
            const double exS = sel(k >= 1, kSv, 0.0), exE = sel(k >= 1, NOBS ? kEv : kEv + 2.0 * wcv, 0.0);
// ... 165 lines not shown
    int lane = c.lane;
#if CRX_SWEEP_LOCAL_LANE & 1
    if (NOBS > 0) asm volatile("" : "+v"(lane));
#endif
    if constexpr (ROWDPP<L> && CRX_SWEEP_MASK && NOBS > 0) {
        if (lane < NZ) {
            const bool isx = lane < NX;
            const int ua = isx ? 0 : lane - NX;
            int cad = isx ? L::M + lane * NZ : L::Kk + ua * NX;
            const int cstep = isx ? 0 : NU * NX;
            const int kfad = L::kf + ua;
            const int sad = L::dZ + lane + (isx ? NZ : 0);
            const double one = isx ? 0.0 : 1.0;
            double mu_[NU];
#pragma unroll
            for (int a = 0; a < NU; a++) mu_[a] = sel(isx, LD(L::M + (isx ? lane : 0) * NZ + NX + a), 0.0);
            double y = LD(L::dZ + (isx ? lane : 0));
            double coef[NX], kfv;
#pragma unroll
            for (int j = 0; j < NX; j++) coef[j] = LD(cad + j);
            kfv = LD(kfad);
            auto stage = [&](int k) {
                double cnx[NX], kfn;
                const int kn = k + 1 < N ? k + 1 : k;
                cad += (k + 1 < N) ? cstep : 0;
#pragma unroll
                for (int j = 0; j < NX; j++) cnx[j] = LD(cad + j);
                kfn = LD(kfad + kn * NU);
                double acc = fma(kfv, one, 0.0);
                acc = row_dot<NX, 0>(y, coef, acc);
                const double du = acc;
                acc = row_dot<NU, NX>(du, mu_, acc);
                y = acc;
                LD(sad + k * NZ) = y;
#pragma unroll
                for (int j = 0; j < NX; j++) coef[j] = cnx[j];
                kfv = kfn;
                STAGE_FENCE();
            };
            if constexpr (UNR > 1) {
#pragma unroll UNR
                for (int k = 0; k < N; k++) stage(k);
            } else {
                for (int k = 0; k < N; k++) stage(k);
            }
            LD(SINK(!isx, L::dZ + N * NZ + lane)) = 0.0;
        }
        SYNC();
        return;
    }
    if (!CRX_SWEEP_MASK || lane < NZ) {
    constexpr bool MK = CRX_SWEEP_MASK;
    const bool in = MK || lane < NZ;
    double mrow[NZ];
#pragma unroll
    for (int j = 0; j < NZ; j++) mrow[j] = LD(L::M + (lane < NX ? lane : 0) * NZ + j);
    const bool isu = lane >= NX && in;
    const int ua = isu ? lane - NX : 0;
    double zx = LD(L::dZ + (lane < NX ? lane : 0));
    double kr[NX], kfa;
#pragma unroll
    for (int j = 0; j < NX; j++) kr[j] = LD(L::Kk + ua * NX + j);
    kfa = LD(L::kf + ua);
    auto stage = [&](int k) {
        double krn[NX], kfn;
        const int kn = k + 1 < N ? k + 1 : k;
#pragma unroll
        for (int j = 0; j < NX; j++) krn[j] = LD(L::Kk + (kn * NU + ua) * NX + j);
        kfn = LD(L::kf + kn * NU + ua);
        double du = kfa, xn = 0.0;
        if constexpr (ROWDPP<L>) {
            du = row_dot<NX, 0>(zx, kr, du);
            xn = row_dot<NX, 0>(zx, mrow, xn);
            xn = row_dot<NU, NX>(du, mrow + NX, xn);
        } else {
            double xs[NX];
#pragma unroll
            for (int j = 0; j < NX; j++) xs[j] = lane_f64(zx, j);
#pragma unroll
            for (int j = 0; j < NX; j++) du += kr[j] * xs[j];
#pragma unroll
            for (int j = 0; j < NX; j++) xn += mrow[j] * xs[j];
#pragma unroll
            for (int a = 0; a < NU; a++) xn += mrow[NX + a] * lane_f64(du, NX + a);
        }
        LD(SINK(in, L::dZ + k * NZ + lane)) = sel(isu, du, zx);
        zx = xn;
#pragma unroll
        for (int j = 0; j < NX; j++) kr[j] = krn[j];
        kfa = kfn;
        STAGE_FENCE();
    };
    if constexpr (UNR > 1) {
#pragma unroll UNR
        for (int k = 0; k < N; k++) stage(k);
    } else {
        for (int k = 0; k < N; k++) stage(k);
    }
    LD(SINK(in, L::dZ + N * NZ + lane)) = sel(lane < NX, zx, 0.0);
    }
    SYNC();
}

template <int NOBS, int NMAX>
__device__ __forceinline__ bool restore_slacks(double* sm, const Ctx& c, double slack_push) {
    using L = Lay<NOBS, NMAX>;
    constexpr int NX = L::NX, NZ = L::NZ, NR = L::NR;
    const int N = c.N;
    if (NOBS == 0 || !(c.om > 1e-6)) return false;
    for (int e = c.lane; e < N * NOBS; e += WAVE) {
        const int k = e / L::NO, ob = e - k * L::NO;
        double dsc, dec, dsn, den;
        cbf_dist<NOBS, NMAX>(sm, c, k, ob, 0.0, dsc, dec, dsn, den);
        const int q = c.degree;
        LD(L::rdt + k * NR + 8 + NOBS + ob) = ipow_d(dsn, q) + ipow_d(den, q) - c.om * (ipow_d(dsc, q) + ipow_d(dec, q)) - c.alpha * c.cm;
    }
    SYNC();
    bool changed = false;
    for (int ob = 0; ob < c.nobs; ob++) {
        double snext = LD(L::Z + N * NZ + 6 + ob);
        for (int i = N - 1; i >= 0; i--) {
            const int j = i * NR + 8 + NOBS + ob;
            const double G = LD(L::rdt + j), push = slack_push / cbf_scale<L>(sm, i, ob);
            const double need = (snext - G + push) / c.om;
            double si = LD(L::Z + i * NZ + 6 + ob);
            if (need > si) {
                si = need;
                changed = true;
                if (c.lane == 0) {
                    LD(L::Z + i * NZ + 6 + ob) = si;
                    if (i >= 1) LD(L::Z + (i - 1) * NZ + NX + 2 + ob) = si;
                }
            }
            snext = si;
        }
    }
    SYNC();
    return changed;
}

template <int NOBS, int NMAX>
__device__ __forceinline__ int crash_search(double* sm, const Ctx& c, const crx_kparams& kp) {
    using L = Lay<NOBS, NMAX>;
    constexpr int NX = L::NX, NZ = L::NZ, G1 = 5;
    (void)NX; (void)NZ;
    constexpr int SPAN = (L::SLIM ? 5 : 7) * L::MR;
    constexpr int CH = 32 * 2 * (NMAX + 1) <= SPAN ? 32 : 16;
    static_assert(L::rnu == L::rt + L::MR && L::rtt == L::rt + 4 * L::MR && (L::SLIM || L::rw == L::rt + 6 * L::MR), "rt, rnu, rc, rdt, rtt, rsig, rw are contiguous");
    static_assert(NOBS == 0 || CH * 2 * (NMAX + 1) <= SPAN, "the candidates' (s, ey) samples fit in the row arrays");
    if (NOBS == 0) return -1;
    const int N = c.N, N1 = N + 1, lane = c.lane;
    double* scr = sm + L::rt;
    const int q = c.degree;
    double best = INFINITY;
    int bestc = -1;
    for (int r = 0; r * CH < G1 * G1; r++) {
        const int cand = r * CH + lane;
        const int a = cand / G1, b = cand - a * G1;
        const double u0 = 0.9 * (2.0 * a / (G1 - 1) - 1.0) * kp.delta_max, u1 = 0.9 * (2.0 * b / (G1 - 1) - 1.0) * kp.a_max;
        double val = INFINITY;
        if (lane < CH && cand < G1 * G1) {
            double x[6], v = 0.0;
            bool inside = true;
#pragma unroll
            for (int i = 0; i < 6; i++) x[i] = LD(L::Z + i);
            scr[0 * CH + lane] = x[4]; scr[1 * CH + lane] = x[5];
#pragma unroll 1
            for (int k = 1; k <= N; k++) {
                double xn[6];
#pragma unroll
                for (int i = 0; i < 6; i++) {
                    double t = 0.0;
#pragma unroll
                    for (int j = 0; j < 6; j++) t += kp.A[i * 6 + j] * x[j];
                    t += kp.B[i * 2] * u0 + kp.B[i * 2 + 1] * u1;
                    xn[i] = t;
                }
#pragma unroll
                for (int i = 0; i < 6; i++) x[i] = xn[i];
                inside = inside && x[0] > kp.v_min + 1e-3 && x[0] < kp.v_max - 1e-3 && x[5] > -kp.ey_max + 1e-3 && x[5] < kp.ey_max - 1e-3;
#pragma unroll
                for (int i = 0; i < 6; i++) { const double e = x[i] - LD(L::xr + k * 6 + i); v += LD(L::cst + i) * e * e; }
                scr[(2 * k) * CH + lane] = x[4]; scr[(2 * k + 1) * CH + lane] = x[5];
            }
#pragma unroll 1
            for (int k = 0; k < N; k++) v += kp.wr[0] * u0 * u0 + kp.wr[1] * u1 * u1;
            double casc = 0.0;
#pragma unroll 1
            for (int ob = 0; ob < c.nobs; ob++) {
                const double rLs = LD(L::cst + 16 + ob), rWs = LD(L::cst + 16 + L::NO + ob), lo = LD(L::cst + 8 + ob);
                double snext = 0.0;
#pragma unroll 1
                for (int i = N - 1; i >= 0; i--) {
                    const double dsc = (scr[(2 * i) * CH + lane] - LD(L::obs_s + ob * N1 + i) - lo) * rLs;
                    const double dec = (scr[(2 * i + 1) * CH + lane] - LD(L::obs_e + ob * N1 + i)) * rWs;
                    const double dsn = (scr[(2 * i + 2) * CH + lane] - LD(L::obs_s + ob * N1 + i + 1)) * rLs;
                    const double den = (scr[(2 * i + 3) * CH + lane] - LD(L::obs_e + ob * N1 + i + 1)) * rWs;
                    const double G = ipow_d(dsn, q) + ipow_d(den, q) - c.om * (ipow_d(dsc, q) + ipow_d(dec, q)) - c.alpha * c.cm;
                    double si = (snext - G) / c.om;
                    si = si < 0.0 ? 0.0 : si;
                    casc += si;
                    snext = si;
                }
            }
            v += c.wsig * casc;
            val = inside ? v : INFINITY;
        }
        const double vm = wave_min(val);
        if (vm < best) {
            const unsigned long long hit = __ballot(val == vm);
            bestc = r * CH + (__ffsll((long long)hit) - 1);
            best = vm;
        }
    }
    return bestc;
}
template <int NOBS, int NMAX, bool cascade>
__device__ __forceinline__ void crash_write(double* sm, const Ctx& c, const crx_kparams& kp, int bestc) {
    using L = Lay<NOBS, NMAX>;
    constexpr int NX = L::NX, NZ = L::NZ, G1 = 5;
    if (NOBS == 0) return;
    const int N = c.N, lane = c.lane, q = c.degree;
    const int a = bestc / G1, b = bestc - a * G1;
    const double u0 = 0.9 * (2.0 * a / (G1 - 1) - 1.0) * kp.delta_max, u1 = 0.9 * (2.0 * b / (G1 - 1) - 1.0) * kp.a_max;
    SYNC();
    for (int e = lane; e < N * 2; e += WAVE) LD(L::Z + (e >> 1) * NZ + NX + (e & 1)) = (e & 1) ? u1 : u0;
    SYNC();
    for (int k = 0; k < N; k++) {
        if (lane < 6) {
            double t = 0.0;
#pragma unroll
            for (int j = 0; j < 6; j++) t += LD(L::M + lane * NZ + j) * LD(L::Z + k * NZ + j);
            t += LD(L::M + lane * NZ + NX) * u0 + LD(L::M + lane * NZ + NX + 1) * u1;
            LD(L::Z + (k + 1) * NZ + lane) = t;
        }
        SYNC();
    }
    if (lane < c.nobs) {
        const int ob = lane;
        const double push = kp.opts.slack_push;
        double snext = push;
        LD(L::Z + N * NZ + 6 + ob) = push;
        LD(L::Z + (N - 1) * NZ + NX + 2 + ob) = push;
        for (int i = N - 1; i >= 0; i--) {
            double si = push;
            if constexpr (cascade) {
                double dsc, dec, dsn, den;
                cbf_dist<NOBS, NMAX>(sm, c, i, ob, 0.0, dsc, dec, dsn, den);
                const double G = ipow_d(dsn, q) + ipow_d(den, q) - c.om * (ipow_d(dsc, q) + ipow_d(dec, q)) - c.alpha * c.cm;
                si = (snext - G + push) / c.om;
                si = si < push ? push : si;
            }
            LD(L::Z + i * NZ + 6 + ob) = si;
            if (i >= 1) LD(L::Z + (i - 1) * NZ + NX + 2 + ob) = si;
            snext = si;
        }
    }
    SYNC();
}

template <class L>
__device__ __forceinline__ void planner_fallback(double* sm, const crx_kparams& kp, int b, int lane, int N) {
    double* Xb = kp.X + (size_t)b * (N + 1) * 6;
    double* Ub = kp.U + (size_t)b * N * 2;
    const double vx0 = kp.x0[(size_t)b * 6];
    double* bs = sm + L::hg;
    double* be = sm + L::Hd;
    for (int j = lane; j <= N; j += WAVE) {
        bs[j] = kp.bez_s[(size_t)b * (N + 1) + j];
        be[j] = kp.bez_ey[(size_t)b * (N + 1) + j];
    }
    SYNC();
    const double s0 = bs[0];
    for (int e = lane; e < (N + 1) * 6; e += WAVE) {
        const int j = e / 6, i = e - j * 6;
        const double st = s0 + kp.fallback_gain * j * kp.dt_ref * vx0;
        double v = 0.0;
        if (i == 0) v = kp.fallback_gain * vx0;
        else if (i == 4) v = st;
        else if (i == 5) v = interp1d<INTERP_SCAN>(bs, be, N + 1, fmin(fmax(st, bs[0]), bs[N]));
        Xb[e] = v;
    }
    for (int e = lane; e < N * 2; e += WAVE) Ub[e] = 0.0;
    if (lane == 0) kp.cost[b] = INFINITY;
}

#ifndef CRX_PLANNER_WAVES
#define CRX_PLANNER_WAVES 3
#endif
#ifndef CRX_OBS1_WAVES
#define CRX_OBS1_WAVES 2
#endif
#ifndef CRX_KERNEL_EXTRA_ATTR
#define CRX_KERNEL_EXTRA_ATTR
#endif
#ifndef CRX_GEN_WAVES
#define CRX_GEN_WAVES 0
#endif
template <int NOBS, int NMAX> struct MinWaves {
    static constexpr int v = CRX_GEN_WAVES ? CRX_GEN_WAVES : ((NOBS == 1 && NMAX == 12) ? CRX_OBS1_WAVES : ((NOBS == 0 && NMAX == 12) ? CRX_PLANNER_WAVES : 1));
};

template <int NFIX> constexpr int StageUnroll = NFIX == 0 ? 1 : NFIX;
template <int NOBS, int NMAX, int DEG = 0, int NFIX = 0, int SPEC = 0, int QPM = 0>
__global__ void __launch_bounds__(WAVE * (1 + SPEC)) __attribute__((amdgpu_waves_per_eu(MinWaves<NOBS, NMAX>::v))) CRX_KERNEL_EXTRA_ATTR
crx_solve_kernel(const crx_kparams kp) {
    static_assert(NFIX <= NMAX, "fixed horizon inside the layout");
    using L = Lay<NOBS, NMAX>;
    static_assert(!SPEC || (NOBS > 0 && !L::SLIM && CRX_STATIC_LDS), "the speculating wave exists for the obstacle instantiations of the full, static layout");
    constexpr int NX = L::NX, NZ = L::NZ, NR = L::NR;
#if CRX_STATIC_LDS
    __shared__ __attribute__((aligned(16))) double sm[((SPEC ? L::BYTES_SPEC : L::BYTES) + 7) / 8];
#else
    extern __shared__ __attribute__((aligned(16))) double sm[];
#endif
    int* si = (int*)(sm + L::END_D);
    const int lane = SPEC ? (int)(threadIdx.x & (WAVE - 1)) : (int)threadIdx.x, N = NFIX ? NFIX : kp.N;
    if ((int)blockIdx.x >= kp.batch) return;
    const int b = kp.order ? min(max(kp.order[blockIdx.x], 0), kp.batch - 1) : (int)blockIdx.x;
    if (kp.active && kp.active[kp.active_div > 1 ? b / kp.active_div : b] == 0) {
        if (lane == 0) { kp.status[b] = CRX_SKIPPED; kp.iters[b] = 0; }
        return;
    }
    if (NOBS == 0 && kp.mode == 0 && kp.reach_screen) {
        bool out = false;
        for (int j = lane; j < N; j += WAVE) {
            double fr = 0.0;
#pragma unroll
            for (int i = 0; i < 6; i++) fr += kp.reach_row[j][i] * kp.x0[(size_t)b * 6 + i];
            const double g = kp.reach_gain[j];
            out = out || kp.ey_lb[(size_t)b * N + j] > fr + g + 1e-6 || kp.ey_ub[b] < fr - g - 1e-6;
        }
        if (__ballot(out) != 0ull) {
            planner_fallback<L>(sm, kp, b, lane, N);
            if (lane == 0) { kp.status[b] = CRX_INFEASIBLE; kp.kkt[b] = INFINITY; kp.iters[b] = 0; }
            return;
        }
    }
    if constexpr (SPEC) {
        if (threadIdx.x >= WAVE) {
            Ctx c1 = {};
            c1.N = N; c1.lane = lane;
            for (;;) {
                __syncthreads();
                const int cmd = __builtin_amdgcn_readfirstlane((int)LD(L::ctl));
                if (cmd == 0) break;
                bool ok1 = false;
                if (cmd == 1) ok1 = riccati_backward<NOBS, NMAX, StageUnroll<NFIX>, 1, true>(sm, si, c1, LD(L::ctl + 1), nullptr, LD(L::ctl + 2) != 0.0);
                if (lane == 0) LD(L::ctl + 3) = ok1 ? 1.0 : 0.0;
                __syncthreads();
            }
            return;
        }
    }
    if (kp.poison) {
        for (int e = lane; e < (int)(L::BYTES / 8); e += WAVE) sm[e] = __longlong_as_double(0x7ff8dead0000beefLL);
        SYNC();
    }
    Ctx c;
    c.N = N; c.lane = lane; c.m = N * NR + NOBS; c.nobs = 0;
    const int m = c.m;
    c.alpha = kp.alpha; c.om = 1.0 - kp.alpha; c.cm = 1.0 + kp.margin;
    c.degree = DEG ? DEG : kp.degree; c.wsig = kp.w_slack; c.lin_sN = 0.0; c.cconst = 0.0;
    c.b_d = kp.delta_max; c.b_a = kp.a_max; c.b_vlo = kp.v_min; c.b_vhi = kp.v_max; c.b_e = kp.ey_max;

    for (int e = lane; e < NX * NZ; e += WAVE) {
        const int i = e / NZ, a = e - i * NZ;
        double v = 0.0;
        if (i < 6) {
            if (a < 6) v = kp.A[i * 6 + a];
            else if (a >= NX && a < NX + 2) v = kp.B[i * 2 + (a - NX)];
        } else if (a == NX + 2 + (i - 6)) v = 1.0;
        LD(L::M + e) = v;
    }
    for (int e = lane; e < (N + 1) * NZ; e += WAVE) {
        LD(L::Z + e) = 0.0; LD(L::dZ + e) = 0.0;
        if constexpr (!L::SLIM) { VROW(si)[L::vlo + e] = -1; VROW(si)[L::vhi + e] = -1; }
    }
    if (lane < 16) {
        double v = 0.0;
        if (lane < 6) v = kp.wq[lane];
        else if (lane < 8) v = kp.wr[lane - 6];
        LD(L::cst + lane) = v;
    }
    {
        constexpr int NTRI = (NZ * NZ <= WAVE || L::SLIM) ? 0 : NZ * (NZ + 1) / 2;
        for (int e = lane; e < NTRI; e += WAVE) {
            int r = 0;
            while ((r + 1) * (r + 2) / 2 <= e) r++;
            si[L::triH + e] = (r << 8) | (e - r * (r + 1) / 2);
        }
        constexpr int NP = NX * (NX + 1) / 2 + NX;
        for (int l = lane; l < WAVE * L::UCNT; l += WAVE) {
            int i = 0, j = l - NP;
            if (ROWDPP<L> && L::UCNT == 1) {
                if (l < NX) { i = l; j = NX; }
                else if (l < NP) {
                    int rem = l - NX;
                    while (rem >= NX - i) { rem -= NX - i; i++; }
                    j = i + rem;
                }
            } else if (l < NP) {
                int rem = l;
                while (rem >= NX + 1 - i) { rem -= NX + 1 - i; i++; }
                j = i + rem;
            }
            if (j < 0 || j > NX) j = 0;
            SH16(si)[L::updP + l] = (unsigned short)((i << 8) | j);
        }
    }
    SYNC();
    if (lane < 6) LD(L::Z + lane) = kp.x0[(size_t)b * 6 + lane];
    SYNC();
    for (int k = 0; k < N; k++) {
        if (lane < 6) {
            double s = 0.0;
#pragma unroll
            for (int j = 0; j < 6; j++) s += LD(L::M + lane * NZ + j) * LD(L::Z + k * NZ + j);
            LD(L::Z + (k + 1) * NZ + lane) = s;
        }
        SYNC();
    }
    int infeas0 = 0;
    if (kp.mode == 0) {
        double* bs = sm + L::hg;
        double* be = sm + L::Hd;
        for (int j = lane; j <= N; j += WAVE) {
            bs[j] = kp.bez_s[(size_t)b * (N + 1) + j];
            be[j] = kp.bez_ey[(size_t)b * (N + 1) + j];
        }
        SYNC();
        const double s0 = LD(L::Z + 4), vx0 = LD(L::Z + 0);
        for (int j = lane; j <= N; j += WAVE) {
            double st = s0 + 1.0 * j * vx0 * kp.dt_ref;
            st = fmin(fmax(st, bs[0]), bs[N]);
#pragma unroll
            for (int i = 0; i < 6; i++) LD(L::xr + j * 6 + i) = 0.0;
            LD(L::xr + j * 6 + 4) = st;
            LD(L::xr + j * 6 + 5) = interp1d<INTERP_SCAN>(bs, be, N + 1, st);
            if (j < N) LD(L::wc + j) = (j >= 1 && j <= N - 2) ? kp.w_dey : 0.0;
        }
        c.lin_sN = -kp.w_prog;
        c.cconst = kp.w_prog * s0;
        const double e0 = LD(L::Z + 5);
        if (e0 < kp.ey_lb[(size_t)b * N] - kp.opts.tol || e0 > kp.ey_ub[b] + kp.opts.tol) infeas0 = 1;
    } else {
        c.nobs = kp.n_obs ? min(max(kp.n_obs[b], 0), min(NOBS, kp.n_obs_max)) : NOBS;
        for (int e = lane; e < (N + 1) * 6; e += WAVE)
            LD(L::xr + e) = kp.per_stage_target ? kp.xt[(size_t)b * (N + 1) * 6 + e] : kp.xt[(size_t)b * 6 + (e % 6)];
        for (int j = lane; j < N; j += WAVE) LD(L::wc + j) = 0.0;
        if (NOBS) {
            for (int e = lane; e < NOBS * (N + 1); e += WAVE) {
                const int o = e / (N + 1);
                const bool on = o < c.nobs;
                LD(L::obs_s + e) = on ? kp.obs_s[((size_t)b * kp.n_obs_max) * (N + 1) + e] : 0.0;
                LD(L::obs_e + e) = on ? kp.obs_ey[((size_t)b * kp.n_obs_max) * (N + 1) + e] : 0.0;
            }
            if (lane < NOBS) {
                LD(L::cst + 8 + lane) = lane < c.nobs ? kp.lap_off[(size_t)b * kp.n_obs_max + lane] : 0.0;
                const bool own = kp.obs_dims != nullptr && lane < c.nobs;
                double ls = own ? kp.obs_dims[((size_t)b * kp.n_obs_max + lane) * 2] : kp.l_sum;
                double ws = own ? kp.obs_dims[((size_t)b * kp.n_obs_max + lane) * 2 + 1] : kp.w_sum;
                ls = dim_or_default(ls, kp.l_sum); ws = dim_or_default(ws, kp.w_sum);
                LD(L::cst + 16 + lane) = 1.0 / ls;
                LD(L::cst + 16 + NOBS + lane) = 1.0 / ws;
            }
        }
        const double v0 = LD(L::Z + 0), e0 = LD(L::Z + 5);
        if (v0 < kp.v_min - kp.opts.tol || v0 > kp.v_max + kp.opts.tol || e0 < -kp.ey_max - kp.opts.tol ||
            e0 > kp.ey_max + kp.opts.tol)
            infeas0 = 1;
    }
    SYNC();
    for (int j = lane; j < m; j += WAVE) {
        int iv = 0;
        double sg = 0.0, bd = 0.0, on = 0.0;
        bool simple = true;
        if (j >= N * NR) {
            const int o = j - N * NR;
            iv = 6 + o; sg = 1.0; bd = 0.0; on = (o < c.nobs) ? 1.0 : 0.0;
        } else {
            const int k = j / NR, r = j - k * NR;
            if (r < 4) {
                const int i = r >> 1;
                iv = k * NZ + NX + i;
                sg = (r & 1) ? -1.0 : 1.0;
                bd = (i == 0 ? kp.delta_max : kp.a_max) * ((r & 1) ? 1.0 : -1.0);
                on = 1.0;
            } else if (r < 8) {
                const int comp = (r < 6) ? 0 : 5;
                iv = (k + 1) * NZ + comp;
                sg = (r & 1) ? -1.0 : 1.0;
                if (kp.mode == 0) {
                    if (r == 5) { bd = kp.v_max; on = 1.0; }
                    else if (r == 6 && k + 1 < N) { bd = kp.ey_lb[(size_t)b * N + k + 1]; on = 1.0; }
                    else if (r == 7 && k + 1 < N) { bd = kp.ey_ub[b]; on = 1.0; }
                } else {
                    bd = (r == 4) ? kp.v_min : (r == 5) ? kp.v_max : (r == 6) ? -kp.ey_max : kp.ey_max;
                    on = 1.0;
                }
                if (!isfinite(bd)) on = 0.0;
            } else if (r < 8 + NOBS) {
                const int o = r - 8;
                iv = k * NZ + NX + 2 + o; sg = 1.0; bd = 0.0; on = (o < c.nobs) ? 1.0 : 0.0;
            } else {
                simple = false;
                on = ((r - 8 - NOBS) < c.nobs) ? 1.0 : 0.0;
            }
        }
        if constexpr (!L::SLIM) {
            if (simple && on != 0.0) {
                if (sg > 0.0) VROW(si)[L::vlo + iv] = (typename L::vrow_t)j; else VROW(si)[L::vhi + iv] = (typename L::vrow_t)j;
            }
        }
        if (on == 0.0 || !simple) { sg = 0.0; bd = 0.0; iv = 0; }
        SH16(si)[L::riv + j] = (unsigned short)(iv | (sg != 0.0 ? RIV_SIMPLE : 0) | (sg < 0.0 ? RIV_NEG : 0));
        if constexpr (L::SLIM) {
            if (!simple) { const int k = j / NR; LD(L::csc + k * L::NO + (j - k * NR - 8 - NOBS)) = on; }
        } else {
            LD(L::rb + j) = bd;
            LD(L::rsc + j) = on;
            LD(L::rsig + j) = 0.0; LD(L::rw + j) = 0.0;
        }
        LD(L::rnu + j) = on;
        LD(L::rt + j) = 1.0;
        LD(L::rc + j) = 1.0;
        LD(L::rdt + j) = 0.0; LD(L::rtt + j) = 1.0;
    }
    SYNC();
    const crx_ipm_opts o = kp.opts;
    int crash_state = 0;
    if (NOBS && kp.slack_start && c.om > 1e-6) {
        bool any = false;
        if (lane < c.nobs) {
            const int ob = lane, q = c.degree;
            double Lb = 0.0;
            for (int i = N - 1; i >= 0; i--) {
                double dsc, dec, dsn, den;
                cbf_dist<NOBS, NMAX>(sm, c, i, ob, 0.0, dsc, dec, dsn, den);
                const double rLs = LD(L::cst + 16 + ob), rWs = LD(L::cst + 16 + L::NO + ob);
                const double rsc = kp.reach_s[i] * rLs, rec = kp.reach_gain[i] * rWs, rsn = kp.reach_s[i + 1] * rLs, ren = kp.reach_gain[i + 1] * rWs;
                const double mx_sn = fmax(fabs(dsn - rsn), fabs(dsn + rsn)), mx_en = fmax(fabs(den - ren), fabs(den + ren));
                const double mn_sc = fabs(dsc) > rsc ? fabs(dsc) - rsc : 0.0, mn_ec = fabs(dec) > rec ? fabs(dec) - rec : 0.0;
                const double Gmax = ipow_d(mx_sn, q) + ipow_d(mx_en, q) - c.om * (ipow_d(mn_sc, q) + ipow_d(mn_ec, q)) - c.alpha * c.cm;
                Lb = (Lb - Gmax) / c.om;
                Lb = Lb > 0.0 ? Lb : 0.0;
                if (Lb > 0.0) {
                    any = true;
                    if (kp.slack_start == 1) {
                        LD(L::Z + i * NZ + 6 + ob) = Lb;
                        if (i >= 1) LD(L::Z + (i - 1) * NZ + NX + 2 + ob) = Lb;
                    }
                }
            }
        }
        crash_state = __ballot(any) != 0ull;
        SYNC();
    }
    const bool crash_path = NOBS > 0 && kp.slack_start >= 2 && o.restore_iters >= 0 && c.om > 1e-6 && c.nobs > 0;
    int crash = 0;
    double mu = o.mu_init, dw_last = 0.0, E0 = INFINITY, theta_min = 0.0, theta_max = INFINITY;
    double f = 0.0;
    int nf = 0, status = 1, it = 0;
    double mact = 0.0;
    for (int j = lane; j < m; j += WAVE) mact += (LD(L::rnu + j) != 0.0) ? 1.0 : 0.0;
    mact = wave_sum(mact);
    const double smax = 100.0;
    long long tph[8] = {0, 0, 0, 0, 0, 0, 0, 0};

    double nus = 0.0, e_p = 0.0, cmax = 0.0, cmin = INFINITY, logsum_t = 0.0;
    auto row_stats = [&]() {
        nus = 0.0; e_p = 0.0; cmax = 0.0; cmin = INFINITY;
        LogAcc lgs;
        for (int j = lane; j < m; j += WAVE) {
            const bool on = row_scale<L>(sm, si, j, N) != 0.0;
            const double t = LD(L::rt + j), nu = LD(L::rnu + j);
            nus += nu;
            e_p = fmax(e_p, on ? fabs(LD(L::rc + j) - t) : 0.0);
            cmax = fmax(cmax, on ? t * nu : 0.0);
            cmin = fmin(cmin, on ? t * nu : INFINITY);
            lgs.mul(on ? t : 1.0);
        }
        nus = wave_sum(nus); e_p = wave_max(e_p); cmax = wave_max(cmax); cmin = wave_min(cmin);
        logsum_t = lgs.wave_total();
    };
    constexpr int JAM_COUNT = 5;
    const int STALL_ITERS = o.stall_iters;
    const double JAM_ALPHA = 1e-3;
    int n_restore = 0, ls_failed = 0, jam = 0, jam_on = (NOBS > 0 && o.restore_iters >= 0), it_limit = 0, cvx_run = 0;
    constexpr int CVX_PROBE = 4;
    int scaled = 0;
    auto init_point = [&]() {
        if (NOBS && !scaled) {
            for (int e = lane; e < N * NOBS; e += WAVE) {
                const int k = e / NOBS, ob = e - k * NOBS;
                if (ob < c.nobs) {
                    double dsc, dec, dsn, den;
                    cbf_dist<NOBS, NMAX>(sm, c, k, ob, 0.0, dsc, dec, dsn, den);
                    const int q = c.degree;
                    double gm = 1.0;
                    const double rLs = LD(L::cst + 16 + ob), rWs = LD(L::cst + 16 + NOBS + ob);
                    gm = fmax(gm, fabs(q * ipow_d(dsn, q - 1) * rLs));
                    gm = fmax(gm, fabs(q * ipow_d(den, q - 1) * rWs));
                    if (k > 0) {
                        gm = fmax(gm, fabs(c.om * q * ipow_d(dsc, q - 1) * rLs));
                        gm = fmax(gm, fabs(c.om * q * ipow_d(dec, q - 1) * rWs));
                    }
                    LD(L::SLIM ? L::csc + k * L::NO + ob : L::rsc + k * NR + 8 + NOBS + ob) = fmin(1.0, o.grad_scale_max / gm);
                }
            }
            SYNC();
        }
        scaled = 1;
        eval_rows<NOBS, NMAX>(sm, si, c);
        SYNC();
        for (int j = lane; j < m; j += WAVE) {
            const bool on = row_scale<L>(sm, si, j, N) != 0.0;
            LD(L::rt + j) = on ? fmax(fabs(LD(L::rc + j)), o.slack_push) : 1.0;
            LD(L::rtt + j) = on ? 1.0 : 0.0;
            LD(L::rnu + j) = 0.0;
            LD(L::rdt + j) = 0.0;
        }
        SYNC();
        first_order<NOBS, NMAX>(sm, si, c);
        (void)dual_infeasibility<NOBS, NMAX>(sm, c);
        for (int j = lane; j < m; j += WAVE) {
            double nu = LD(L::rtt + j);
            const int pk = RIVT(si, j);
            if (nu != 0.0 && (pk & RIV_SIMPLE)) {
                const int iv = RIV_IDX(pk);
                const int kk = iv / NZ, a = iv - kk * NZ;
                if (a >= NX || (kk == 0 && a >= 6)) {
                    const double gg = RIV_SGN(pk) * LD(L::ga + iv);
                    if (gg > 1.0) nu = gg;
                }
            }
            LD(L::rnu + j) = nu;
            LD(L::rtt + j) = 1.0;
        }
        SYNC();
        first_order<NOBS, NMAX>(sm, si, c);
        f = cost_value<NOBS, NMAX>(sm, c, 0.0);
        row_stats();
        mu = o.mu_init; nf = 0; dw_last = 0.0; status = 1; jam = 0;
        theta_min = -1.0; theta_max = INFINITY;
    };
    int crash_cand = -1;
    if (NOBS && crash_path) {
        bool viol = false;
        for (int e = lane; e < N * NOBS; e += WAVE) {
            const int k = e / L::NO, ob = e - k * L::NO;
            if (ob < c.nobs) {
                double dsc, dec, dsn, den;
                cbf_dist<NOBS, NMAX>(sm, c, k, ob, 0.0, dsc, dec, dsn, den);
                const int q = c.degree;
                viol = viol || (ipow_d(dsn, q) + ipow_d(den, q) - c.om * (ipow_d(dsc, q) + ipow_d(dec, q)) - c.alpha * c.cm < 0.0);
            }
        }
        if (crash_state || __ballot(viol) != 0ull) crash_cand = __builtin_amdgcn_readfirstlane(crash_search<NOBS, NMAX>(sm, c, kp));
        if ((crash_state || kp.slack_start == 3) && crash_cand >= 0) { crash_write<NOBS, NMAX, true>(sm, c, kp, crash_cand); crash = 1; n_restore = 1; it_limit = 1 + 3 * o.restore_iters; }
    }
    init_point();
    if constexpr (NOBS == 0 && QPM == 0) {
    (void)theta_min; (void)theta_max; (void)nf; (void)dw_last; (void)logsum_t; (void)cmin; (void)mu; (void)crash; (void)crash_path;
    double gap = 0.0;
    for (int j = lane; j < m; j += WAVE) gap += (row_scale<L>(sm, si, j, N) != 0.0) ? LD(L::rt + j) * LD(L::rnu + j) : 0.0;
    gap = wave_sum(gap);
    constexpr int RP = (L::MR + WAVE - 1) / WAVE;
    for (;; it++) {
#if CRX_OPAQUE_LANE
        asm volatile("" : "+v"(c.lane));
        const int lane = c.lane;
#endif
        const double sd = fmax(smax, nus / fmax(mact, 1.0)) / smax;
        const double e_du = dual_infeasibility<NOBS, NMAX, (StageUnroll<NFIX> > 2 ? StageUnroll<NFIX> : 1)>(sm, c);
        E0 = fmax(e_du / sd, fmax(e_p, cmax / sd));
        if (E0 <= o.tol && e_du <= o.dual_inf_tol && e_p <= o.constr_viol_tol && cmax <= o.compl_inf_tol) { status = 0; break; }
        if (it >= o.max_iter) break;
        const double mu_k = gap / fmax(mact, 1.0);
        assemble_newton<NOBS, NMAX>(sm, si, c, 0.0);
        if (!riccati_backward<NOBS, NMAX, StageUnroll<NFIX>, 0, false, true>(sm, si, c, 0.0)) break;
        riccati_forward<NOBS, NMAX, StageUnroll<NFIX>>(sm, c);
        double dta[RP], dna[RP], rpm = 0.0, rdm = 0.0;
#pragma unroll
        for (int q_ = 0; q_ < RP; q_++) {
            const bool jv = lane + q_ * WAVE < m;
            const int j = jv ? lane + q_ * WAVE : 0;
            const int pk = RIVT(si, j);
            const bool on = jv && LD(L::rsc + j) != 0.0;
            const double jd = RIV_SGN(pk) * LD(L::dZ + RIV_IDX(pk));
            const double t = LD(L::rt + j), nu = LD(L::rnu + j), rti = LD(L::rtt + j), rcj = LD(L::rc + j), rsj = LD(L::rsig + j), rwj = LD(L::rw + j);
            const double rp = rcj - t;
            dta[q_] = sel(on, jd + rp, 0.0);
            dna[q_] = sel(on, -rwj + rsj * (rp - dta[q_]), 0.0);
            rpm = fmax(rpm, -dta[q_] * rti);
            rdm = fmax(rdm, sel(on, -dna[q_] * frcp(nu), 0.0));
        }
        wave_max2(rpm, rdm);
        const double apa = rpm > 1.0 ? 1.0 / rpm : 1.0, ada = rdm > 1.0 ? 1.0 / rdm : 1.0;
        double ga_ = 0.0;
#pragma unroll
        for (int q_ = 0; q_ < RP; q_++) {
            const bool jv = lane + q_ * WAVE < m;
            const int j = jv ? lane + q_ * WAVE : 0;
            ga_ += sel(jv && LD(L::rsc + j) != 0.0, (LD(L::rt + j) + apa * dta[q_]) * (LD(L::rnu + j) + ada * dna[q_]), 0.0);
        }
        const double mu_aff = wave_sum(ga_) / fmax(mact, 1.0);
        double sigma = mu_aff / mu_k;
        sigma = sigma * sigma * sigma;
        const double smu = fmax(sigma * mu_k, o.tol / 10.0);
        constexpr double PC_SHORT_STEP = 0.2;
        double cr[RP], s_new = smu, s_old = 0.0, c_old = 0.0, a_p = 1.0, a_d = 1.0;
#pragma unroll
        for (int q_ = 0; q_ < RP; q_++) cr[q_] = dta[q_] * dna[q_];
        const double tau = ipm_tau(mu_k, o.tau_min);
        for (int pass = 0;; pass++) {
            const double c_new = pass == 0 ? 1.0 : 0.0;
            SYNC();
#pragma unroll
            for (int q_ = 0; q_ < RP; q_++) {
                const bool jv = lane + q_ * WAVE < m;
                const int j = jv ? lane + q_ * WAVE : 0;
                const bool on = jv && LD(L::rsc + j) != 0.0;
                const double dwj = sel(on, -((s_new - c_new * cr[q_]) - (s_old - c_old * cr[q_])) * LD(L::rtt + j), 0.0);
                const double rwj = LD(L::rw + j);
                LD(SINK(jv, L::rw + j)) = rwj + dwj;
                LD(SINK(jv, L::dZ + j)) = dwj;
            }
            SYNC();
            COORDS(e, ev, lane, N * NZ + NX) {
                const int k = e / NZ, a = e - k * NZ;
                int rl, rh;
                coord_rows<L>(si, c, e, k, a, rl, rh);
                const double dl = LD(L::dZ + (rl >= 0 ? rl : 0)), dh = LD(L::dZ + (rh >= 0 ? rh : 0)), g0 = LD(L::hg + e);
                LD(SINK(ev && !(k == N && a >= NX), L::hg + e)) = g0 + sel(rl >= 0, dl, 0.0) - sel(rh >= 0, dh, 0.0);
            }
            SYNC();
            riccati_backward_vec<NOBS, NMAX, StageUnroll<NFIX>>(sm, c);
            riccati_forward<NOBS, NMAX, StageUnroll<NFIX>>(sm, c);
            rpm = 0.0; rdm = 0.0;
#pragma unroll
            for (int q_ = 0; q_ < RP; q_++) {
                const bool jv = lane + q_ * WAVE < m;
                const int j = jv ? lane + q_ * WAVE : 0;
                const int pk = RIVT(si, j);
                const bool on = jv && LD(L::rsc + j) != 0.0;
                const double jd = RIV_SGN(pk) * LD(L::dZ + RIV_IDX(pk));
                const double t = LD(L::rt + j), nu = LD(L::rnu + j), rti = LD(L::rtt + j), rcj = LD(L::rc + j), rsj = LD(L::rsig + j), rwj = LD(L::rw + j);
                const double rp = rcj - t;
                dta[q_] = sel(on, jd + rp, 0.0);
                dna[q_] = sel(on, -rwj + rsj * (rp - dta[q_]), 0.0);
                rpm = fmax(rpm, -dta[q_] * rti);
                rdm = fmax(rdm, sel(on, -dna[q_] * frcp(nu), 0.0));
            }
            wave_max2(rpm, rdm);
            a_p = rpm > tau ? tau / rpm : 1.0; a_d = rdm > tau ? tau / rdm : 1.0;
            if (pass == 0 && fmin(a_p, a_d) < PC_SHORT_STEP) { s_old = s_new; c_old = 1.0; s_new = fmax(mu_k, o.tol / 10.0); continue; }
            break;
        }
        static_assert(L::MR <= L::NV, "row scratch inside dZ");
        if (kp.trace && b == kp.trace_problem && it < (kp.trace_rows < 0 ? -kp.trace_rows : kp.trace_rows) && lane == 0) {
            double* tr = kp.trace + (size_t)it * 16;
            tr[0] = e_du / sd; tr[1] = e_p; tr[2] = cmax / sd; tr[3] = mu_k; tr[4] = a_p; tr[5] = a_d; tr[6] = sigma; tr[7] = 1.0;
        }
        SYNC();
        COORDS(e, ev, lane, N * NZ + NX) {
            const double zn = LD(L::Z + e) + a_p * LD(L::dZ + e);
            LD(SINK(ev, L::Z + e)) = zn;
        }
        SYNC();
        double numax = 0.0, th = 0.0, gs = 0.0;
        nus = 0.0; cmax = 0.0;
#pragma unroll
        for (int q_ = 0; q_ < RP; q_++) {
            const bool jv = lane + q_ * WAVE < m;
            const int j = jv ? lane + q_ * WAVE : 0;
            const int pk = RIVT(si, j);
            const bool on = jv && LD(L::rsc + j) != 0.0;
            const double v = RIV_SGN(pk) * (LD(L::Z + RIV_IDX(pk)) - LD(L::rb + j));
            double tn = LD(L::rt + j) + a_p * dta[q_];
            tn = sel(v > tn, v, tn);
            const double nn = LD(L::rnu + j) + a_d * dna[q_];
            LD(SINK(on, L::rt + j)) = tn;
            LD(SINK(on, L::rnu + j)) = nn;
            LD(SINK(jv, L::rc + j)) = sel(on, v, 1.0);
            numax = fmax(numax, sel(on, nn, 0.0));
            th = fmax(th, sel(on, fabs(v - tn), 0.0));
            nus += sel(on, nn, 0.0);
            gs += sel(on, tn * nn, 0.0);
            cmax = fmax(cmax, sel(on, tn * nn, 0.0));
        }
        SYNC();
        {
            double z0 = 0.0;
            wave_max4(numax, th, cmax, z0);
            double z1 = 0.0, z2 = 0.0;
            wave_sum4(nus, gs, z1, z2);
        }
        gap = gs;
        e_p = th;
        first_order<NOBS, NMAX>(sm, si, c);
        if (numax > 1e12 && th > 1e-6) { status = CRX_STALLED; it++; break; }
        if (th > 1e-6) {
            if (box_certificate<NOBS, NMAX>(sm, si, c, kp.delta_max, kp.a_max) < -1e-8 * numax) { status = 2; it++; break; }
        }
    }
    f = cost_value<NOBS, NMAX>(sm, c, 0.0);
    } else {
    if (NOBS && crash) {
        double sc = 0.0;
        for (int j = lane; j < m; j += WAVE) sc += LD(L::rt + j) * LD(L::rnu + j);
        sc = wave_sum(sc);
        mu = fmin(fmax(0.1 * sc / fmax(mact, 1.0), o.mu_init), 1e6);
    }
    for (;;) {
    ls_failed = 0;
    asm volatile("" ::: "memory");

    for (;; it++) {
        long long tc0 = CLK();
#if CRX_OPAQUE_LANE
        if (NOBS == 0 || CRX_OPAQUE_LANE >= 2) asm volatile("" : "+v"(c.lane));
        const int lane = c.lane;
#endif
        double e_c = cmax;
        const double sd = fmax(smax, nus / fmax(mact, 1.0)) / smax;
        long long tc1 = CLK();
        const double e_du = dual_infeasibility<NOBS, NMAX, (StageUnroll<NFIX> > 2 ? StageUnroll<NFIX> : 1)>(sm, c);
        const double e_d = e_du / sd;
        long long tc2 = CLK();
        e_c /= sd;
        E0 = fmax(e_d, fmax(e_p, e_c));
        if (E0 <= o.tol) {
            double vu = e_p;
            if (NOBS) {
                for (int e = lane; e < N * NOBS; e += WAVE) {
                    const int k = e / L::NO, ob = e - k * L::NO, j = k * NR + 8 + NOBS + ob;
                    const double sc = cbf_scale<L>(sm, k, ob);
                    if (sc != 0.0) vu = fmax(vu, fabs(LD(L::rc + j) - LD(L::rt + j)) / sc);
                }
                vu = wave_max(vu);
            }
            if (e_du <= o.dual_inf_tol && vu <= o.constr_viol_tol && cmax <= o.compl_inf_tol) { status = 0; break; }
        }
        if (it >= o.max_iter) break;
        if (NOBS && n_restore > 0 && it >= it_limit) { status = 3; break; }
        for (;;) {
            const double e_cm = fmax(cmax - mu, mu - cmin) / sd;
            const double Emu = fmax(e_d, fmax(e_p, e_cm));
            if (ipm_mu_reached(Emu, mu, o.kappa_eps, o.tol)) {
                mu = ipm_next_mu<true>(mu, o.kappa_mu, o.theta_mu, o.tol);
                nf = 0;
            } else
                break;
        }
        const double tau = ipm_tau(mu, o.tau_min);
        long long tc3 = CLK();
        assemble_newton<NOBS, NMAX>(sm, si, c, mu);
        long long tc4 = CLK();
        double dw = 0.0;
        long long tsub[4] = {0, 0, 0, 0};
        bool ok;
        int used_convex = 0;
        if (NOBS && crash && cvx_run > 0 && (cvx_run % CVX_PROBE) != 0) {
            if constexpr (!SPEC) {
                for (int k = lane; k < N; k += WAVE) { LD(L::kS + 2 * k) = 0.0; LD(L::kE + 2 * k) = 0.0; }
                SYNC();
            }
            used_convex = 1;
        }
        if constexpr (SPEC) {
            double sdw = 0.0;
            int cz = used_convex, avail = (crash && !used_convex) ? 1 : 0, tries = 0;
            for (;;) {
                double ndw = sdw;
                int ncz = cz, ntries = tries;
                if (avail) ncz = 1;
                else { ndw = tries == 0 ? (dw_last == 0.0 ? 1e-4 : fmax(1e-20, dw_last / 3.0)) : sdw * (dw_last == 0.0 ? 100.0 : 8.0); ntries = tries + 1; }
                const bool nvalid = !(ndw > 1e40);
                const bool post = nvalid && kp.spec_idle == 0;
                if (lane == 0) { LD(L::ctl) = post ? 1.0 : 2.0; LD(L::ctl + 1) = ndw; LD(L::ctl + 2) = ncz ? 1.0 : 0.0; }
                __syncthreads();
                ok = riccati_backward<NOBS, NMAX, StageUnroll<NFIX>, 0, true>(sm, si, c, sdw, tsub, cz != 0);
                __syncthreads();
                if (ok) { dw = sdw; used_convex = cz; break; }
                dw = ndw;
                if (!nvalid) break;
                if (!post) { sdw = ndw; cz = ncz; avail = 0; tries = ntries; continue; }
                if (__builtin_amdgcn_readfirstlane((int)LD(L::ctl + 3)) != 0) {
                    for (int e = lane; e < N * L::NU * NX; e += WAVE) LD(L::Kk + e) = LD(L::Kk2 + e);
                    for (int e = lane; e < N * L::NU; e += WAVE) LD(L::kf + e) = LD(L::kf2 + e);
                    if (lane < NZ) LD(L::dZ + lane) = LD(L::dZ2 + lane);
                    SYNC();
                    ok = true; used_convex = ncz;
                    break;
                }
                sdw = ntries == 0 ? (dw_last == 0.0 ? 1e-4 : fmax(1e-20, dw_last / 3.0)) : ndw * (dw_last == 0.0 ? 100.0 : 8.0);
                cz = ncz; avail = 0; tries = ntries + 1;
                dw = sdw;
                if (sdw > 1e40) break;
            }
        } else
        for (int tries = 0, convex = (NOBS > 0 && crash && !used_convex) ? 0 : 1;; ) {
            ok = riccati_backward<NOBS, NMAX, StageUnroll<NFIX>>(sm, si, c, dw, tsub);
            if (ok) break;
            if (NOBS && !convex) {
                used_convex = 1;
                convex = 1;
                for (int k = lane; k < N; k += WAVE) { LD(L::kS + 2 * k) = 0.0; LD(L::kE + 2 * k) = 0.0; }
                SYNC();
                continue;
            }
            dw = tries == 0 ? (dw_last == 0.0 ? 1e-4 : fmax(1e-20, dw_last / 3.0)) : dw * (dw_last == 0.0 ? 100.0 : 8.0);
            tries++;
            if (dw > 1e40) break;
        }
        if (!ok) break;
        if (dw != 0.0) dw_last = dw;
        cvx_run = used_convex ? cvx_run + 1 : 0;
        long long tc5 = CLK();
        riccati_forward<NOBS, NMAX, StageUnroll<NFIX>>(sm, c);
        long long tc6 = CLK();
        double rp_max = 0.0, rd_max = 0.0, theta = 0.0, Dphi = 0.0;
        auto row_step = [&](int j, bool cnt, bool store, double sc, double jd) {
            const bool on = sc != 0.0;
            const double t = LD(L::rt + j), nu = LD(L::rnu + j), rti = LD(L::rtt + j), rcj = LD(L::rc + j);
            double rwj, rsj;
            row_sig_w<L>(sm, j, on, mu, t, nu, rti, rcj, rsj, rwj);
            ROW_LOADS_DONE();
            const double rp = rcj - t;
            const double dt = sel(on, jd + rp, 0.0);
            const double dnu = sel(on, -rwj + rsj * (rp - dt), 0.0);
            LD(SINK(store, L::rdt + j)) = dt;
            const double dtr = dt * rti;
            rp_max = fmax(rp_max, sel(cnt, -dtr, 0.0));
            rd_max = fmax(rd_max, sel(cnt && on, -dnu * frcp(nu), 0.0));
            theta += sel(cnt && on, fabs(rp), 0.0);
            Dphi -= sel(cnt && on, mu * dtr, 0.0);
        };
        ROWS(j, jv, lane, m) {
            const bool simple = !ROW_IS_CBF(j, N);
            const int pk = RIVT(si, j);
            const double sc = row_scale<L>(sm, si, j, N), jd = RIV_SGN(pk) * LD(L::dZ + RIV_IDX(pk));
            row_step(j, jv && simple, simple, sc, jd);
        }
        if (NOBS) {
            CBF_ROWS(j, k, ob, ev, lane, N) {
                const double* J = sm + L::Jc + (k * L::NO + ob) * NZ;
                double jc = 0.0;
#pragma unroll
                for (int a = 0; a < NZ; a++) jc += J[a] * LD(L::dZ + k * NZ + a);
                row_step(j, ev, true, cbf_scale<L>(sm, k, ob), jc);
            }
        }
        wave_max2(rp_max, rd_max);
        const double a_p = (rp_max > tau) ? tau / rp_max : 1.0;
        const double a_d = (rd_max > tau) ? tau / rd_max : 1.0;
        double cost_qq;
        double cost_d = cost_dir<NOBS, NMAX>(sm, c, cost_qq);
        wave_sum4(theta, Dphi, cost_d, cost_qq);
        Dphi += cost_d;
        const double phi0 = f - mu * logsum_t;
        if (theta_min < 0.0) ipm_theta_bounds(theta, theta_min, theta_max);
        long long tc7 = CLK();
        double al = a_p, fn = f, lt_acc = logsum_t;
        int acc = 0, ftype = 0;
        const bool sw_try = (theta <= theta_min) && (Dphi < 0.0);
        const double sw_gap = sw_try ? IPM_S_PHI * log2_fast(-Dphi) - IPM_S_THETA * log2_fast(theta) : 0.0;
        for (int ls = 0; ls < IPM_MAX_BACKTRACK && al >= IPM_ALPHA_MIN; ls++) {
            fn = f + al * (cost_d + al * cost_qq);
            double thn = 0.0;
            LogAcc lg;
            auto row_trial = [&](int j, bool cnt, bool store, double sc, double cn, double t, double dt) {
                double tn = t + al * dt;
                tn = sel(cn > tn, cn, tn);
                const bool off = sc == 0.0;
                tn = sel(off, 1.0, tn);
                cn = sel(off, 1.0, cn);
                LD(SINK(store, L::rtt + j)) = tn;
                lg.mul(sel(cnt, tn, 1.0));
                thn += sel(cnt, fabs(cn - tn), 0.0);
            };
            ROWS(j, jv, lane, m) {
                const bool simple = !ROW_IS_CBF(j, N);
                const double sc = row_scale<L>(sm, si, j, N), t = LD(L::rt + j), dt = LD(L::rdt + j), cj = LD(L::rc + j);
                ROW_LOADS_DONE();
                row_trial(j, jv && simple, simple, sc, cj + al * (dt - (cj - t)), t, dt);
            }
            if (NOBS) {
                CBF_ROWS(j, k, ob, ev, lane, N) {
                    const double sc = cbf_scale<L>(sm, k, ob), t = LD(L::rt + j), dt = LD(L::rdt + j);
                    row_trial(j, ev, true, sc, sc * cbf_value<NOBS, NMAX>(sm, c, k, ob, al), t, dt);
                }
            }
            lt_acc = lg.wave_total_with(thn);
            const double phin = fn - mu * lt_acc;
            int okf = (thn <= theta_max) && (phin == phin);
            {
                const bool iv = lane < nf;
                const int i = iv ? lane : 0;
                const double fth = LD(L::Fth + i), fph = LD(L::Fph + i);
                if (__any(iv && !(thn < fth || phin < fph))) okf = 0;
            }
            if (okf) {
                if (sw_try && log2_fast(al) + sw_gap > 0.0) {
                    if (phin <= phi0 + IPM_ETA_PHI * al * Dphi + 10.0 * IPM_EPS * fabs(phi0)) { acc = 1; ftype = 1; }
                } else if (ipm_sufficient_decrease(theta, thn, phi0, phin)) {
                    acc = 1;
                }
            }
            if (acc) break;
            al *= 0.5;
        }
        long long tc8 = CLK();
        tph[0] = tc1 - tc0; tph[1] = tc2 - tc1; tph[2] = tc3 - tc2; tph[3] = tc4 - tc3; tph[4] = tc5 - tc4;
        tph[5] = tc6 - tc5; tph[6] = tc7 - tc6; tph[7] = tc8 - tc7;
        if (kp.trace_rows < 0) { tph[0] = tsub[0]; tph[1] = tsub[1]; tph[2] = tsub[2]; tph[3] = tsub[3]; }
        if (kp.trace && b == kp.trace_problem && it < (kp.trace_rows < 0 ? -kp.trace_rows : kp.trace_rows) && lane == 0) {
            double* tr = kp.trace + (size_t)it * 16;
            for (int q = 0; q < 8; q++) tr[8 + q] = (double)(tph[q]);
            tr[0] = e_d; tr[1] = e_p; tr[2] = e_c; tr[3] = mu; tr[4] = al; tr[5] = a_d; tr[6] = dw; tr[7] = acc ? (ftype ? 2.0 : 1.0) : 0.0;
        }
        if (acc && !ftype && nf < MAXF) {
            if (lane == 0) { LD(L::Fth + nf) = ipm_filter_theta(theta); LD(L::Fph + nf) = ipm_filter_phi(theta, phi0); }
            nf++;
        }
        if (!acc) { ls_failed = 1; break; }
        if (NOBS) {
            jam = (jam_on && al < JAM_ALPHA && e_p > o.tol) ? jam + 1 : 0;
            if (jam_on && n_restore == 0 && it >= STALL_ITERS && e_p > 1e-6) jam = JAM_COUNT;
            if (jam >= JAM_COUNT && n_restore < 2) { ls_failed = 2; break; }
        }
        SYNC();
        COORDS(e, ev, lane, N * NZ + NX) {
            const double zn = LD(L::Z + e) + al * LD(L::dZ + e);
            LD(SINK(ev, L::Z + e)) = zn;
        }
        SYNC();
        f = fn;
        logsum_t = lt_acc;
        double numax = 0.0, th = 0.0;
        nus = 0.0; cmax = 0.0; cmin = INFINITY;
        auto row_accept = [&](int j, bool own, double sc, double v) {
            const bool on = sc != 0.0, cnt = own && on;
            const double tn = LD(L::rtt + j), rcj = LD(L::rc + j), rtj = LD(L::rt + j);
            const double rdj = LD(L::rdt + j), rnj = LD(L::rnu + j);
            double rwj, rsj;
            row_sig_w<L>(sm, j, on, mu, rtj, rnj, L::SLIM ? frcp(rtj) : 0.0, rcj, rsj, rwj);
            ROW_LOADS_DONE();
            const double mut = mu * frcp(tn);
            const double rp = rcj - rtj;
            const double dnu = -rwj + rsj * (rp - rdj);
            double nn = rnj + a_d * dnu;
            nn = ipm_dual_safeguard(nn, mut);
            LD(SINK(cnt, L::rt + j)) = tn;
            LD(SINK(cnt, L::rnu + j)) = nn;
            numax = fmax(numax, sel(cnt, nn, 0.0));
            th = fmax(th, sel(cnt, fabs(v - tn), 0.0));
            nus += sel(cnt, nn, 0.0);
            cmax = fmax(cmax, sel(cnt, tn * nn, 0.0));
            cmin = fmin(cmin, sel(cnt, tn * nn, INFINITY));
            LD(SINK(own, L::rc + j)) = sel(on, v, 1.0);
        };
        ROWS(j, jv, lane, m) {
            const int pk = RIVT(si, j);
            const double sc = row_scale<L>(sm, si, j, N), v = RIV_SGN(pk) * (LD(L::Z + RIV_IDX(pk)) - row_bound<L>(sm, c, j));
            row_accept(j, jv && !ROW_IS_CBF(j, N), sc, v);
        }
        if (NOBS) {
            CBF_ROWS(j, k, ob, ev, lane, N) {
                const double sc = cbf_scale<L>(sm, k, ob);
                row_accept(j, ev, sc, sc * cbf_value<NOBS, NMAX>(sm, c, k, ob, 0.0));
            }
        }
        SYNC();
        {
            double ncmin = -cmin;
            wave_max4(numax, th, cmax, ncmin);
            cmin = -ncmin;
        }
        nus = wave_sum(nus);
        e_p = th;
        first_order<NOBS, NMAX>(sm, si, c);
        if (kp.trace && b == kp.trace_problem && it < (kp.trace_rows < 0 ? -kp.trace_rows : kp.trace_rows) && lane == 0 && kp.trace_rows > 0)
            kp.trace[(size_t)it * 16 + 8] = (double)(tph[0] + (CLK() - tc8));
        if (numax > 1e12 && th > 1e-6) { status = CRX_STALLED; it++; break; }
        if (NOBS == 0 && th > 1e-6) {
            if (box_certificate<NOBS, NMAX>(sm, si, c, kp.delta_max, kp.a_max) < -1e-8 * numax) { status = 2; it++; break; }
        }
    }
    if (!ls_failed) break;
    int full = 0;
    if (NOBS && crash_path && n_restore == 0 && !crash && crash_cand >= 0) {
        crash_write<NOBS, NMAX, false>(sm, c, kp, crash_cand);
        crash = 1; full = 1;
    }
    if (NOBS && o.restore_iters >= 0 && n_restore < 2 && (__builtin_amdgcn_readfirstlane((int)restore_slacks<NOBS, NMAX>(sm, c, o.slack_push)) | full)) {
        eval_rows<NOBS, NMAX>(sm, si, c);
        SYNC();
        for (int j = lane; j < m; j += WAVE) {
            const bool cbf = ROW_IS_CBF(j, N);
            const int r = j < N * NR ? j % NR : 8;
            const bool sig = NOBS && (j >= N * NR || (r >= 8 && r < 8 + NOBS));
            if (row_scale<L>(sm, si, j, N) != 0.0) {
                const double t = fmax(fabs(LD(L::rc + j)), o.slack_push);
                if (cbf || sig) {
                    LD(L::rt + j) = t;
                    LD(L::rnu + j) = fmin(fmax(o.mu_init / t, 1e-8), 1e8);
                } else if (full) {
                    LD(L::rt + j) = t;
                    LD(L::rnu + j) = 1.0;
                }
            }
        }
        SYNC();
        first_order<NOBS, NMAX>(sm, si, c);
        f = cost_value<NOBS, NMAX>(sm, c, 0.0);
        row_stats();
        if (n_restore++ == 0) it_limit = it + 1 + o.restore_iters;
        mu = o.mu_init; nf = 0; theta_min = -1.0; theta_max = INFINITY; dw_last = 0.0; status = 1; jam = 0;
        it++;
        continue;
    }
    if (ls_failed == 2) {
        jam_on = 0; jam = 0;
        if constexpr (L::SLIM) first_order<NOBS, NMAX>(sm, si, c);
        continue;
    }
    if (e_p > 1e-6) status = CRX_STALLED;
    break;
    }
    }
    if constexpr (SPEC) {
        if (lane == 0) LD(L::ctl) = 0.0;
        __syncthreads();
    }
    if (infeas0) status = CRX_INFEASIBLE;

    SYNC();
    int lane_wb = threadIdx.x;
    asm volatile("" : "+v"(lane_wb));
    {
    const int lane = lane_wb;
    double* Xb = kp.X + (size_t)b * (N + 1) * 6;
    double* Ub = kp.U + (size_t)b * N * 2;
    if (kp.mode == 0 && status != 0) {
        planner_fallback<L>(sm, kp, b, lane, N);
    } else {
        for (int e = lane; e < (N + 1) * 6; e += WAVE) { const int k = e / 6, i = e - k * 6; Xb[e] = LD(L::Z + k * NZ + i); }
        for (int e = lane; e < N * 2; e += WAVE) Ub[e] = LD(L::Z + (e >> 1) * NZ + NX + (e & 1));
        if (lane == 0) kp.cost[b] = f;
    }
    if (kp.mode == 1 && kp.sigma) {
        for (int e = lane; e < kp.n_obs_max * (N + 1); e += WAVE) {
            const int ob = e / (N + 1), k = e - ob * (N + 1);
            kp.sigma[(size_t)b * kp.n_obs_max * (N + 1) + e] = (NOBS && ob < c.nobs) ? LD(L::Z + k * NZ + 6 + ob) : 0.0;
        }
    }
    double Eout = E0;
    if (kp.kkt_unscaled && status == 0) {
        double ed = 0.0, ev = 0.0, ec = 0.0;
        for (int e = lane; e < N * NZ + NX; e += WAVE) ed = fmax(ed, fabs(LD(L::ga + e)));
        for (int j = lane; j < m; j += WAVE) {
            const double sc = row_scale<L>(sm, si, j, N);
            if (sc != 0.0) { ev = fmax(ev, fabs(LD(L::rc + j) - LD(L::rt + j)) / sc); ec = fmax(ec, LD(L::rt + j) * LD(L::rnu + j)); }
        }
        const int km = kp.kkt_unscaled;
        Eout = wave_max(km == 2 ? ed : km == 3 ? ev : km == 4 ? ec : fmax(ed, fmax(ev, ec)));
    }
    if (lane == 0) { kp.status[b] = status; kp.kkt[b] = Eout; kp.iters[b] = it; }
    }
}

#ifndef CRX_TU_OBSTACLES
__global__ void __launch_bounds__(WAVE) crx_select_kernel(const crx_select_kparams sp) {
    const int s = blockIdx.x, lane = threadIdx.x;
    if (s >= sp.n_scen) return;
    const int N = sp.N, V = sp.V, R = V + 1;
    const int nv = min(max(sp.n_veh[s], 0), V);
    const double r2 = sp.veh_length * sp.veh_length + sp.veh_width * sp.veh_width;
    double best_c = INFINITY;
    int best = 0;
    for (int r = 0; r < R; r++) {
        double cst = INFINITY;
        if (r <= nv) {
            const double* Xr = sp.X + (((size_t)s * R + r) * (N + 1)) * 6;
            double hits = 0.0;
            for (int e = lane; e < 2 * (N + 1); e += WAVE) {
                const int side = e / (N + 1), j = e - side * (N + 1);
                const int v = side == 0 ? r - 1 : r;
                if (v < 0 || v >= nv) continue;
                double os = sp.obs_s[((size_t)s * V + v) * (N + 1) + j];
                os = wrap_above(os, sp.lap_length);
                const double ds = Xr[6 * j + 4] - os;
                const double de = Xr[6 * j + 5] - sp.obs_ey[((size_t)s * V + v) * (N + 1) + j];
                if (!(ds * ds + de * de - r2 >= 0.0)) hits += 1.0;
            }
            hits = wave_sum(hits);
            cst = -sp.w_prog * (Xr[6 * N + 4] - Xr[4]) + sp.w_coll * hits;
            if (sp.old_flag[s] >= 0 && sp.old_flag[s] != r) cst += sp.w_switch;
            if (cst < best_c) { best_c = cst; best = r; }
        }
        if (lane == 0) sp.sel_cost[(size_t)s * R + r] = cst;
    }
    if (lane == 0) sp.flag[s] = best;
    const double* Xb = sp.X + (((size_t)s * R + best) * (N + 1)) * 6;
    for (int e = lane; e < (N + 1) * 6; e += WAVE) sp.best_X[(size_t)s * (N + 1) * 6 + e] = Xb[e];
}

#endif

#ifdef CRX_PROBE_ONE
template __global__ void crx_solve_kernel<CRX_PROBE_ONE>(const crx_kparams);
#else
template <int NOBS, int NMAX, int DEG = 0, int NFIX = 0, int SPEC = 0, int QPM = 0>
static hipError_t launch_t(const crx_kparams& kp, hipStream_t st) {
    if constexpr (NOBS == 0 && QPM == 0) {
        if (kp.opts.qp_method != 0) return launch_t<NOBS, NMAX, DEG, NFIX, SPEC, 1>(kp, st);
    }
#if CRX_STATIC_LDS
    hipLaunchKernelGGL((crx_solve_kernel<NOBS, NMAX, DEG, NFIX, SPEC, QPM>), dim3(kp.batch), dim3(WAVE * (1 + SPEC)), 0, st, kp);
#else
    static_assert(SPEC == 0, "the two-wave instantiations are static-LDS kernels");
    const size_t bytes = Lay<NOBS, NMAX>::BYTES;
    static int attr_set_on = -1;
    int dev = -1;
    if (hipGetDevice(&dev) != hipSuccess) return hipErrorInvalidDevice;
    if (attr_set_on != dev) {
        hipError_t e = hipFuncSetAttribute((const void*)crx_solve_kernel<NOBS, NMAX, DEG, NFIX, 0, QPM>, hipFuncAttributeMaxDynamicSharedMemorySize, (int)bytes);
        if (e != hipSuccess) return e;
        attr_set_on = dev;
    }
    hipLaunchKernelGGL((crx_solve_kernel<NOBS, NMAX, DEG, NFIX, 0, QPM>), dim3(kp.batch), dim3(WAVE), bytes, st, kp);
#endif
    return hipGetLastError();
}
template <int NOBS, int NMAX, int DEG, int NFIX>
static int occ_t() {
    int n = 0;
#if CRX_STATIC_LDS
    const size_t bytes = 0;
#else
    const size_t bytes = Lay<NOBS, NMAX>::BYTES;
    if (hipFuncSetAttribute((const void*)crx_solve_kernel<NOBS, NMAX, DEG, NFIX>, hipFuncAttributeMaxDynamicSharedMemorySize, (int)bytes) != hipSuccess) return -1;
#endif
    if (hipOccupancyMaxActiveBlocksPerMultiprocessor(&n, crx_solve_kernel<NOBS, NMAX, DEG, NFIX>, WAVE, bytes) != hipSuccess) return -1;
    return n;
}

template <int NOBS, int NMAX, int DEG, int NFIX> struct Inst { static constexpr int nobs = NOBS, nmax = NMAX, deg = DEG, nfix = NFIX; };
constexpr int horizon_class(int nobs, int N) { return N <= 12 ? 12 : ((nobs == 3 && N <= 20) ? 20 : CRX_MAX_N); }
#ifndef CRX_NFIX_LIST
#define CRX_NFIX_LIST 10, 12, 20
#endif
#ifndef CRX_NFIX_LIST
#define CRX_NFIX_LIST 10, 12, 20
#endif
template <int NOBS, int DEG, int... NFS, class F>
static bool select_fixed(int N, F&& f) {
    return ((N == NFS ? (f(Inst<NOBS, horizon_class(NOBS, NFS), DEG, NFS>{}), true) : false) || ...);
}
template <int NOBS, int DEG, class F>
static void select_class(int N, F&& f) {
    constexpr int MID = horizon_class(NOBS, 20);
    const int cls = horizon_class(NOBS, N);
    if (cls == 12) f(Inst<NOBS, 12, DEG, 0>{});
    else if (cls == MID) f(Inst<NOBS, MID, DEG, 0>{});
    else f(Inst<NOBS, CRX_MAX_N, DEG, 0>{});
}
template <class F>
static bool select_general(int nobs_template, int N, int degree, F&& f) {
    const bool d6 = degree == 6;
    switch (nobs_template) {
        case 0: select_class<0, 0>(N, f); return true;
        case 1: d6 ? select_class<1, 6>(N, f) : select_class<1, 0>(N, f); return true;
        case 2: d6 ? select_class<2, 6>(N, f) : select_class<2, 0>(N, f); return true;
        case 3: d6 ? select_class<3, 6>(N, f) : select_class<3, 0>(N, f); return true;
        case 4: case 5: case 6: select_class<6, 0>(N, f); return true;
        default: return false;
    }
}
static int query_slots(int nobs_template) { return nobs_template >= 0 && nobs_template <= 3 ? nobs_template : CRX_MAX_OBS; }

hipError_t crx_launch_solve_obs(const crx_kparams& kp, int nobs_template, hipStream_t st);
int crx_solve_resident_per_cu_obs(int N, int nobs_template);
hipError_t crx_launch_solve_general(const crx_kparams& kp, int nobs_template, hipStream_t st);
int crx_solve_resident_per_cu_general(int N, int nobs_template);

#if defined(CRX_TU_SPEC)
hipError_t crx_launch_solve_spec(const crx_kparams& kp, hipStream_t st) {
    if (kp.batch == 0) return hipSuccess;
    if (kp.degree != 6) return hipErrorInvalidValue;
    if (kp.N == 12) return launch_t<1, 12, 6, 12, 1>(kp, st);
    if (kp.N == 10) return launch_t<1, 12, 6, 10, 1>(kp, st);
    return hipErrorInvalidValue;
}
#else
#if CRX_TU_GENERAL
#define CRX_UNIT(name) name##_general
template <class F>
static bool select_inst(int nobs_template, int N, int degree, F&& f) { return select_general(nobs_template, N, degree, f); }
static hipError_t next_unit_launch(const crx_kparams&, int, hipStream_t) { return hipErrorInvalidValue; }
static int next_unit_resident(int, int) { return -1; }
#elif defined(CRX_TU_OBSTACLES)
#define CRX_UNIT(name) name##_obs
template <class F>
static bool select_inst(int nobs_template, int N, int degree, F&& f) {
    if (degree != 6) return false;
    switch (nobs_template) {
        case 1: return select_fixed<1, 6, CRX_NFIX_LIST>(N, f);
        case 2: return select_fixed<2, 6, CRX_NFIX_LIST>(N, f);
        case 3: return select_fixed<3, 6, CRX_NFIX_LIST>(N, f);
        default: return false;
    }
}
static hipError_t next_unit_launch(const crx_kparams& kp, int nobs_template, hipStream_t st) { return crx_launch_solve_general(kp, nobs_template, st); }
static int next_unit_resident(int N, int nobs_template) { return crx_solve_resident_per_cu_general(N, nobs_template); }
#else
#define CRX_UNIT(name) name
template <class F>
static bool select_inst(int nobs_template, int N, int, F&& f) { return nobs_template == 0 && select_fixed<0, 0, CRX_NFIX_LIST>(N, f); }
static hipError_t next_unit_launch(const crx_kparams& kp, int nobs_template, hipStream_t st) { return crx_launch_solve_obs(kp, nobs_template, st); }
static int next_unit_resident(int N, int nobs_template) { return crx_solve_resident_per_cu_obs(N, nobs_template); }
#endif

hipError_t CRX_UNIT(crx_launch_solve)(const crx_kparams& kp, int nobs_template, hipStream_t st) {
    if (kp.batch == 0) return hipSuccess;
    hipError_t e = hipSuccess;
    if (select_inst(nobs_template, kp.N, kp.degree, [&](auto i) { e = launch_t<i.nobs, i.nmax, i.deg, i.nfix>(kp, st); })) return e;
    return next_unit_launch(kp, nobs_template, st);
}
int CRX_UNIT(crx_solve_resident_per_cu)(int N, int nobs_template) {
    int n = 0;
    if (select_inst(query_slots(nobs_template), N, 6, [&](auto i) { n = occ_t<i.nobs, i.nmax, i.deg, i.nfix>(); })) return n;
    return next_unit_resident(N, nobs_template);
}

#ifndef CRX_TU_OBSTACLES
size_t crx_solve_lds_bytes(int N, int nobs_template) {
    size_t bytes = 0;
    select_general(query_slots(nobs_template), N, 6, [&](auto i) { bytes = Lay<i.nobs, i.nmax>::BYTES; });
    return bytes;
}

hipError_t crx_launch_select(const crx_select_kparams& sp, hipStream_t st) {
    if (sp.n_scen == 0) return hipSuccess;
    hipLaunchKernelGGL(crx_select_kernel, dim3(sp.n_scen), dim3(WAVE), 0, st, sp);
    return hipGetLastError();
}

__global__ void __launch_bounds__(WAVE) crx_debug_reduce_kernel(const double* in, double* out) {
    const int lane = threadIdx.x;
    double a = in[lane], b = in[64 + lane], c = in[128 + lane], d = in[192 + lane];
    double s0 = a, s1 = b, s2 = c, s3 = d;
    wave_sum4(s0, s1, s2, s3);
    double m0 = a, m1 = b, m2 = c, m3 = d;
    wave_max4(m0, m1, m2, m3);
    double p0 = a, p1 = b;
    wave_sum2(p0, p1);
    double q0 = c, q1 = d;
    wave_max2(q0, q1);
    int ex;
    const double r0 = wave_sum(a), r1 = wave_max(b), r2 = wave_min(c), r3 = wave_prod(frexp(fabs(d) + 1.0, &ex));
    if (lane == 0) {
        out[0] = s0; out[1] = s1; out[2] = s2; out[3] = s3; out[4] = m0; out[5] = m1; out[6] = m2; out[7] = m3;
        out[8] = p0; out[9] = p1; out[10] = q0; out[11] = q1; out[12] = r0; out[13] = r1; out[14] = r2; out[15] = r3;
    }
    double m[7];
#pragma unroll
    for (int i = 0; i < 7; i++) m[i] = (double)(i + 1) * b + d;
    out[16 + lane] = row_dot<7, 0>(a, m, c);
    double masked = __longlong_as_double(0x7ff8000000000000LL), chained = masked;
    if (lane < 10) {
        masked = row_dot<7, 3>(a, m, c);
        const double first = row_dot<7, 0>(a, m, c);
        chained = row_dot<3, 7>(first, m, first);
    }
    out[80 + lane] = masked;
    out[144 + lane] = chained;
}

hipError_t crx_launch_debug_reduce(const double* in, double* out, hipStream_t st) {
    hipLaunchKernelGGL(crx_debug_reduce_kernel, dim3(1), dim3(WAVE), 0, st, in, out);
    return hipGetLastError();
}
#endif
#endif
#endif
```

car-racing_amd/csrc/crx_kparams.h:

```cpp
#ifndef CRX_KPARAMS_H
#define CRX_KPARAMS_H
#include <stdint.h>

#include "../../include/crx.h"

struct crx_kparams {
    int N, batch, mode , per_stage_target, n_obs_max, degree;
    double A[36], B[12];
    double wq[6], wr[2];
    double w_dey, w_prog, w_slack;
    double delta_max, a_max, v_min, v_max, ey_max;
    double alpha, margin, l_sum, w_sum;
    double dt_ref, fallback_gain;
    crx_ipm_opts opts;
    const double *x0, *bez_s, *bez_ey, *ey_lb, *ey_ub;
    const double *xt, *obs_s, *obs_ey, *lap_off;
    const int32_t* n_obs;
    const double* obs_dims;
    double *X, *U, *sigma, *cost, *kkt;
    int32_t *status, *iters;
    double* trace;
    int trace_problem, trace_rows;
    int poison;
    int kkt_unscaled;
    int spec_idle;
    const int32_t* active;
    int active_div;
    const int32_t* order;
    int reach_screen;
    double reach_gain[CRX_MAX_N + 1];
    double reach_row[CRX_MAX_N][6];
    int slack_start;
    double reach_s[CRX_MAX_N + 1];
};

struct crx_lmpc_kparams {
    int N, batch, n_ss_max;
    double Q[6], R[2], dR[2], x_track[6];
    double v_max, ey_max, delta_max, a_max, w_x0;
    crx_ipm_opts opts;
    const double *x0, *u_old, *A, *B, *C, *ss, *qfun;
    const int32_t* n_ss;
    double *X, *U, *lambda, *cost, *kkt;
    int32_t *status, *iters;
    double* trace;
    int trace_problem, trace_rows;
    int poison;
    const int32_t* active;
    const int32_t* order;
    int reach_screen;
};

struct crx_select_kparams {
    int N, V, n_scen;
    double veh_length, veh_width, lap_length, w_prog, w_coll, w_switch;
    const int32_t* n_veh;
    const double *X, *obs_s, *obs_ey;
    const int32_t* old_flag;
    int32_t* flag;
    double *sel_cost, *best_X;
};

struct crx_prep_kparams {
    int N, V, n_scen, n_opt;
    double prediction_factor, lookahead, track_width, lap_length, veh_length, veh_width, safety_margin, dt_ref;
    const double *x_wrapped, *x_raw, *veh_info, *max_dv, *obs_s, *obs_ey, *opt_s, *opt_ey;
    const int32_t* n_veh;
    double *x0, *bez_s, *bez_ey, *ey_lb, *ey_ub;
};

struct crx_path_kparams {
    int N, batch;
    double alpha, w_rate;
    crx_ipm_opts opts;
    const double *opt, *bez, *lb, *ub, *e0, *eN;
    double *E, *cost, *kkt;
    int32_t *status, *iters;
};

struct crx_plant_kparams {
    crx_plant_desc d;
    int batch, u_stride, wrap;
    const double *track, *xglob, *xcurv, *u;
    double *xglob_next, *xcurv_next;
    int32_t* laps;
    const double* noise_z;
};

struct crx_cbfprep_kparams {
    int N, V, batch;
    double lap_length, t, dt, safety_time;
    const double *xcurv, *car_s0, *car_v, *car_ey;
    double *obs_s, *obs_ey, *lap_off;
    int32_t* n_obs;
};

struct crx_trackprep_kparams {
    int N, V, batch;
    double lap_length, safety_time, dt_ref;
    const double *x, *obs_s_in, *obs_ey_in, *traj;
    const int32_t* n_veh;
    double *xt, *obs_s, *obs_ey, *lap_off;
    int32_t* n_obs;
};

struct crx_scene_kparams {
    crx_scene_desc d;
    int n_scen;
    const double *ego_xcurv, *veh_xcurv, *pred_s, *pred_ey;
    const int32_t* n_all;
    int32_t *n_veh, *overflow, *order;
    double *veh_info, *max_dv, *obs_s, *obs_ey;
};

struct crx_lmpcprep_kparams {
    crx_lmpcprep_desc d;
    int batch, from_plan;
    const double *ss_xcurv, *u_ss, *qfun;
    const int32_t *time_ss, *iter;
    const double *x, *lin_points, *lin_input, *track;
    double *A, *B, *C, *ss_sel, *q_sel;
    int32_t* status;
    const int32_t* active;
};

#ifdef __HIPCC__
#include <hip/hip_runtime.h>
hipError_t crx_launch_solve(const crx_kparams& kp, int nobs_template, hipStream_t st);
hipError_t crx_launch_solve_spec(const crx_kparams& kp, hipStream_t st);
hipError_t crx_launch_select(const crx_select_kparams& sp, hipStream_t st);
hipError_t crx_launch_debug_reduce(const double* in, double* out, hipStream_t st);
hipError_t crx_launch_lmpc_addtraj(const crx_lmpcprep_desc& d, int batch, const int32_t* crossed, double* log_x, const double* log_u,
                                   int32_t* n_log, double* ss_xcurv, double* u_ss, double* qfun, int32_t* time_ss, int32_t* iter,
                                   int32_t* step, const double* x, int32_t* status, hipStream_t st);
size_t crx_solve_lds_bytes(int N, int nobs_template);
int crx_solve_resident_per_cu(int N, int nobs_template);
hipError_t crx_launch_path(const crx_path_kparams& pp, hipStream_t st);
hipError_t crx_launch_cbfprep(const crx_cbfprep_kparams& cp, hipStream_t st);

struct crx_order_kparams {
    int batch, mode;
    const int32_t *iters, *active;
    int32_t* order;
    int V, stride, degree, per_stage_target;
    double margin, l_sum, w_sum, ds_per_vx;
    const double *x0, *xt, *obs_s, *obs_ey, *lap_off, *obs_dims;
    const int32_t* n_obs;
};
hipError_t crx_launch_order(const crx_order_kparams& op, hipStream_t st);

struct crx_game_kparams {
    int N, Np, batch, n_cars, n_points;
    double lap_length, t, dt;
    const double *car_s0, *car_v, *car_ey;
    double *veh_xcurv, *pred_s, *pred_ey;
    const int32_t *n_veh, *overflow;
    int32_t *m_overtake, *m_lmpc, *overflow_seen;
    const int32_t* overtake;
    const double *U_track, *X_lmpc, *U_lmpc;
    const int32_t* flag;
    double *u, *u_old, *u_prev, *lin_points, *lin_input;
    int32_t *step_no, *addpoint_step, *old_flag;
    const double* xcurv;
    const int32_t* laps;
    int32_t *laps_prev, *n_log, *crossed;
    double *log_x, *log_u;
};
hipError_t crx_launch_game(int which, const crx_game_kparams& gp, hipStream_t st);
hipError_t crx_launch_plant(const crx_plant_kparams& pk, hipStream_t st);
hipError_t crx_launch_prep(const crx_prep_kparams& pp, hipStream_t st);
hipError_t crx_launch_scene(const crx_scene_kparams& sp, hipStream_t st);
hipError_t crx_launch_trackprep(const crx_trackprep_kparams& tp, hipStream_t st);
hipError_t crx_launch_lmpc(const crx_lmpc_kparams& kp, hipStream_t st);
hipError_t crx_launch_lmpcprep(const crx_lmpcprep_kparams& kp, hipStream_t st);
size_t crx_lmpcprep_lds_bytes(int n_points);
hipError_t crx_launch_lmpc_addpoint(const crx_lmpcprep_desc& d, int batch, double* ss_xcurv, double* u_ss, const int32_t* time_ss,
                                    const int32_t* iter, const int32_t* step, const double* x, const double* u, int u_stride,
                                    hipStream_t st);
size_t crx_lmpc_lds_bytes(int N, int n_ss_max);
int crx_lmpc_resident_per_cu(int N, int n_ss_max);
struct crx_ilqr_kparams {
    int N, batch, n_obs_max, max_iter;
    double A[36], B[12], Q[36], R[4];
    double eps, lamb_init, lamb_factor, lamb_max, margin, q1, q2, l_sum, w_sum;
    const double *x0, *xt, *obs_s, *obs_ey, *lap_off;
    const int32_t *n_obs, *active;
    double *X, *U, *cost;
    int32_t *status, *iters;
};
hipError_t crx_launch_ilqr(const crx_ilqr_kparams& kp, hipStream_t st);
size_t crx_ilqr_lds_bytes(int N);
int crx_ilqr_resident_per_cu(int N);
struct crx_sysid_kparams {
    int n_logs, n_groups, first_row, chunk, tpl;
    double lamb;
    const int64_t* log_off;
    const int32_t* grp_off;
    const double *x, *u;
    double *ws_gram, *ws_res, *ws_W;
    double *A, *B, *err;
    int64_t* n_pairs;
    int32_t* status;
};
hipError_t crx_launch_sysid(const crx_sysid_kparams& kp, hipStream_t st);
struct crx_pid_kparams {
    int batch, T, row;
    const double *vt, *eyt, *xcurv, *u_prev;
    double *u_next, *x_log, *u_log;
};
hipError_t crx_launch_pid_log(const crx_pid_kparams& kp, hipStream_t st);
#endif
#endif
```

Measured before the change: 588,400.

## Add lone-wave solver variant caching loop-invariant LDS values in registers

Adds a SPEC==2 instantiation of the obstacle solver for N=12/10 that runs at one wave per EU and preloads loop-invariant quantities (M rows, obstacle offsets, row scales, bounds, cost weights, coordinate row indices) into registers. The CBF trial value is reused in the accept step instead of being recomputed. It is selected automatically when the batch is at most four blocks per CU. It trades occupancy for fewer LDS reads per IPM iteration, and relies on each lane owning a fixed set of rows and coordinates.

```diff
diff --git a/car-racing_amd/csrc/crx_api.hip b/car-racing_amd/csrc/crx_api.hip
--- a/car-racing_amd/csrc/crx_api.hip
+++ b/car-racing_amd/csrc/crx_api.hip
@@ -82,6 +82,9 @@
 int g_poison = 0;
 int g_kkt_unscaled = 0;
 int g_spec = 0;
+int g_lone = 0;
+int g_lone_cap = -1;
+int g_lone_last[2] = {0, 0};
 int g_trace_rows = 0, g_trace_problem = 0;
 
 int ensure_init() {
@@ -237,14 +240,28 @@
     kp.poison = g_poison;
 }
 
+int lone_cap() {
+    if (g_lone_cap < 0) {
+        int cus = 0;
+        g_lone_cap = hipDeviceGetAttribute(&cus, hipDeviceAttributeMultiprocessorCount, g_device) == hipSuccess ? 4 * cus : 0;
+    }
+    return g_lone_cap;
+}
+
 int launch_solve(const crx_kparams& kp, int tmpl, hipStream_t st) {
     crx_kparams kq = kp;
     apply_diagnostics(kq);
     size_t lds = crx_solve_lds_bytes(kp.N, tmpl);
     if (lds > 160 * 1024) return fail(CRX_ERR_ARG, "N=%d with %d obstacles needs %zu B of LDS (> 160 KiB)", kp.N, tmpl, lds);
-    const bool spec = tmpl == 1 && kq.mode == 1 && kq.degree == 6 && (kq.N == 12 || kq.N == 10) && g_spec > 0;
+    const bool tuned1 = tmpl == 1 && kq.mode == 1 && kq.degree == 6 && (kq.N == 12 || kq.N == 10);
+    const bool spec = tuned1 && g_spec > 0;
     kq.spec_idle = g_spec == 2;
-    return launched(spec ? crx_launch_solve_spec(kq, st) : crx_launch_solve(kq, tmpl, st), "solver");
+    bool lone = false;
+    if (tuned1 && !spec) {
+        lone = g_lone == 1 || (g_lone == 0 && kq.batch <= lone_cap());
+        g_lone_last[kq.N == 12 ? 0 : 1] = lone;
+    }
+    return launched(spec ? crx_launch_solve_spec(kq, st) : lone ? crx_launch_solve_lone(kq, st) : crx_launch_solve(kq, tmpl, st), "solver");
 }
 
 }
@@ -280,6 +297,7 @@
     }
     HIP_TRY(hipStreamCreateWithFlags(&g_stream, hipStreamNonBlocking));
     g_device = device;
+    g_lone_cap = -1;
     g_init = true;
     return CRX_OK;
 }
@@ -316,6 +334,8 @@
 void crx_debug_poison_lds(int enable) { g_poison = enable != 0; }
 
 void crx_debug_speculation(int mode) { g_spec = mode < 0 ? 0 : (mode > 2 ? 1 : mode); }
+
+void crx_debug_lone_wave(int mode) { g_lone = (mode >= 0 && mode <= 2) ? mode : 0; }
 
 void crx_debug_kkt_unscaled(int mode) { g_kkt_unscaled = (mode >= 0 && mode <= 4) ? mode : 0; }
 
@@ -339,6 +359,8 @@
 
 int crx_debug_resident_per_cu(int kind, int N, int n) {
     if (ensure_init() != CRX_OK) return -1;
+    if (kind == 0 && n == 1 && (N == 12 || N == 10) && g_spec == 0 && (g_lone == 1 || (g_lone == 0 && g_lone_last[N == 12 ? 0 : 1])))
+        return crx_solve_resident_per_cu_lone(N);
     return kind == 0 ? crx_solve_resident_per_cu(N, n) : crx_lmpc_resident_per_cu(N, n);
 }
 
diff --git a/car-racing_amd/csrc/crx_kernels.hip b/car-racing_amd/csrc/crx_kernels.hip
--- a/car-racing_amd/csrc/crx_kernels.hip
+++ b/car-racing_amd/csrc/crx_kernels.hip
@@ -138,6 +138,21 @@
     double b_d, b_a, b_vlo, b_vhi, b_e;
 };
 
+struct NoInv {};
+template <class L>
+struct LoneInv {
+    static constexpr int RP = (L::MR + WAVE - 1) / WAVE, CP = (L::NV + WAVE - 1) / WAVE;
+    double m4[L::NZ], m5[L::NZ];
+    double mcol[L::NX];
+    double rLs, rWs, lap, os0, oe0, os1, oe1;
+    double csc;
+    double rsc[RP], rb[RP];
+    int riv[RP];
+    int rl[CP], rh[CP];
+    double cw[CP], xrv[CP];
+};
+template <class INV> constexpr bool HasInv = !std::is_same_v<INV, NoInv>;
+
 template <class L>
 __device__ __forceinline__ double row_scale(const double* sm, const int* si, int j, int N) {
     if constexpr (L::SLIM) {
@@ -215,27 +230,34 @@
 #define CLK() 0LL
 #endif
 
-template <int NOBS, int NMAX>
+template <int NOBS, int NMAX, class INV = NoInv>
 __device__ __forceinline__ void cbf_dist(const double* sm, const Ctx& c, int k, int o, double al, double& dsc,
-                                         double& dec, double& dsn, double& den) {
+                                         double& dec, double& dsn, double& den, const INV inv = INV()) {
     using L = Lay<NOBS, NMAX>;
     const int N1 = c.N + 1;
     const double sc = LD(L::Z + k * L::NZ + 4) + al * LD(L::dZ + k * L::NZ + 4);
     const double ec = LD(L::Z + k * L::NZ + 5) + al * LD(L::dZ + k * L::NZ + 5);
     const double sn = LD(L::Z + (k + 1) * L::NZ + 4) + al * LD(L::dZ + (k + 1) * L::NZ + 4);
     const double en = LD(L::Z + (k + 1) * L::NZ + 5) + al * LD(L::dZ + (k + 1) * L::NZ + 5);
+    if constexpr (HasInv<INV>) {
+        dsc = (sc - inv.os0 - inv.lap) * inv.rLs;
+        dec = (ec - inv.oe0) * inv.rWs;
+        dsn = (sn - inv.os1) * inv.rLs;
+        den = (en - inv.oe1) * inv.rWs;
+    } else {
     const double rLs = LD(L::cst + 16 + o), rWs = LD(L::cst + 16 + L::NO + o);
     dsc = (sc - LD(L::obs_s + o * N1 + k) - LD(L::cst + 8 + o)) * rLs;
     dec = (ec - LD(L::obs_e + o * N1 + k)) * rWs;
     dsn = (sn - LD(L::obs_s + o * N1 + k + 1)) * rLs;
     den = (en - LD(L::obs_e + o * N1 + k + 1)) * rWs;
-}
-
-template <int NOBS, int NMAX>
-__device__ __forceinline__ double cbf_value(const double* sm, const Ctx& c, int k, int o, double al) {
+    }
+}
+
+template <int NOBS, int NMAX, class INV = NoInv>
+__device__ __forceinline__ double cbf_value(const double* sm, const Ctx& c, int k, int o, double al, const INV inv = INV()) {
     using L = Lay<NOBS, NMAX>;
     double dsc, dec, dsn, den;
-    cbf_dist<NOBS, NMAX>(sm, c, k, o, al, dsc, dec, dsn, den);
+    cbf_dist<NOBS, NMAX>(sm, c, k, o, al, dsc, dec, dsn, den, inv);
     const int q = c.degree;
     const double gc = ipow_d(dsc, q) + ipow_d(dec, q), gn = ipow_d(dsn, q) + ipow_d(den, q);
     const double sk = LD(L::Z + k * L::NZ + 6 + o) + al * LD(L::dZ + k * L::NZ + 6 + o);
@@ -275,8 +297,8 @@
     return wave_sum(acc) + c.cconst;
 }
 
-template <int NOBS, int NMAX>
-__device__ __forceinline__ double cost_dir(const double* sm, const Ctx& c, double& qq) {
+template <int NOBS, int NMAX, class INV = NoInv>
+__device__ __forceinline__ double cost_dir(const double* sm, const Ctx& c, double& qq, const INV inv = INV()) {
     using L = Lay<NOBS, NMAX>;
     const int N = c.N;
     double acc = 0.0, q = 0.0;
@@ -285,8 +307,14 @@
         const bool isx = a < 6, isu = a >= L::NX && a < L::NX + 2, iss0 = a >= 6 && a < L::NX;
         const bool cpl = a == 5 && k >= 1;
         const double dv = LD(L::dZ + e), z = LD(L::Z + e);
-        const double w = sel(isx || isu, LD(L::cst + (isx ? a : (isu ? 6 + a - L::NX : 0))), 0.0);
-        const double ref = sel(isx, LD(L::xr + k * 6 + (isx ? a : 0)), 0.0);
+        double w, ref;
+        if constexpr (HasInv<INV>) {
+            w = sel(isx || isu, inv.cw[q_], 0.0);
+            ref = sel(isx, inv.xrv[q_], 0.0);
+        } else {
+            w = sel(isx || isu, LD(L::cst + (isx ? a : (isu ? 6 + a - L::NX : 0))), 0.0);
+            ref = sel(isx, LD(L::xr + k * 6 + (isx ? a : 0)), 0.0);
+        }
         const int ep = seli(cpl, e - L::NZ, e);
         const double de = z - LD(L::Z + ep), dd = dv - LD(L::dZ + ep);
         const double wk = sel(cpl, LD(L::wc + seli(cpl, k - 1, 0)), 0.0);
@@ -315,8 +343,8 @@
     }
 }
 
-template <int NOBS, int NMAX>
-__device__ __forceinline__ void first_order(double* sm, const int* si, const Ctx& c) {
+template <int NOBS, int NMAX, class INV = NoInv>
+__device__ __forceinline__ void first_order(double* sm, const int* si, const Ctx& c, const INV inv = INV()) {
     using L = Lay<NOBS, NMAX>;
     const int N = c.N;
     if (NOBS) {
@@ -329,18 +357,26 @@
             double* J = sm + L::Jc + (k * L::NO + o) * L::NZ;
             const bool here = o < c.nobs;
             double dsc, dec, dsn, den;
-            cbf_dist<NOBS, NMAX>(sm, c, k, o, 0.0, dsc, dec, dsn, den);
+            cbf_dist<NOBS, NMAX>(sm, c, k, o, 0.0, dsc, dec, dsn, den, inv);
             const int q = c.degree;
             const double qd = (double)q, qq = (double)(q * (q - 1));
             const double p2sn = ipow_d(dsn, q - 2), p2en = ipow_d(den, q - 2);
             const double p2sc = ipow_d(dsc, q - 2), p2ec = ipow_d(dec, q - 2);
-            const double rLs = LD(L::cst + 16 + o), rWs = LD(L::cst + 16 + L::NO + o);
+            double rLs, rWs;
+            if constexpr (HasInv<INV>) { rLs = inv.rLs; rWs = inv.rWs; }
+            else { rLs = LD(L::cst + 16 + o); rWs = LD(L::cst + 16 + L::NO + o); }
             const double gsn = qd * p2sn * dsn * rLs, gen = qd * p2en * den * rWs;
             const double gsc = qd * p2sc * dsc * rLs, gec = qd * p2ec * dec * rWs;
-            const double d = cbf_scale<L>(sm, k, o);
-            double m4[L::NZ], m5[L::NZ];
-#pragma unroll
-            for (int a = 0; a < L::NZ; a++) { m4[a] = LD(L::M + 4 * L::NZ + a); m5[a] = LD(L::M + 5 * L::NZ + a); }
+            double d, m4[L::NZ], m5[L::NZ];
+            if constexpr (HasInv<INV>) {
+                d = inv.csc;
+#pragma unroll
+                for (int a = 0; a < L::NZ; a++) { m4[a] = inv.m4[a]; m5[a] = inv.m5[a]; }
+            } else {
+                d = cbf_scale<L>(sm, k, o);
+#pragma unroll
+                for (int a = 0; a < L::NZ; a++) { m4[a] = LD(L::M + 4 * L::NZ + a); m5[a] = LD(L::M + 5 * L::NZ + a); }
+            }
             G[0] = sel(here, qq * p2sn * rLs * rLs, 0.0); G[1] = sel(here, qq * p2en * rWs * rWs, 0.0);
             G[2] = sel(here, qq * p2sc * rLs * rLs, 0.0); G[3] = sel(here, qq * p2ec * rWs * rWs, 0.0);
 #pragma unroll
@@ -361,14 +397,17 @@
         const bool isx = a < 6, isu = a >= L::NX && a < L::NX + 2, iss0 = a >= 6 && a < L::NX, iss1 = a >= L::NX + 2;
         const int o = iss0 ? a - 6 : (iss1 ? a - L::NX - 2 : 0);
         const bool sig_on = (o < c.nobs) && ((iss0 && k == 0) || (iss1 && k < N));
-        const double cw = LD(L::cst + (isx ? a : (isu ? 6 + a - L::NX : 0))), xrv = LD(L::xr + k * 6 + (isx ? a : 0));
+        double cw, xrv;
+        if constexpr (HasInv<INV>) { cw = inv.cw[q_]; xrv = inv.xrv[q_]; }
+        else { cw = LD(L::cst + (isx ? a : (isu ? 6 + a - L::NX : 0))); xrv = LD(L::xr + k * 6 + (isx ? a : 0)); }
         const double w2 = sel(isx || isu, 2.0 * cw, 0.0);
         const double ref = sel(isx, xrv, 0.0);
         double g = w2 * (LD(L::Z + e) - ref);
         g += (k == N && a == 4) ? c.lin_sN : 0.0;
         g += sig_on ? c.wsig : 0.0;
         int rl, rh;
-        coord_rows<L>(si, c, e, k, a, rl, rh);
+        if constexpr (HasInv<INV>) { rl = inv.rl[q_]; rh = inv.rh[q_]; }
+        else coord_rows<L>(si, c, e, k, a, rl, rh);
         const double nl = LD(L::rnu + (rl >= 0 ? rl : 0)), nh = LD(L::rnu + (rh >= 0 ? rh : 0));
         g -= sel(rl >= 0, nl, 0.0);
         g += sel(rh >= 0, nh, 0.0);
@@ -390,8 +429,8 @@
     SYNC();
 }
 
-template <int NOBS, int NMAX, int UNR = 1>
-__device__ __forceinline__ double dual_infeasibility(double* sm, const Ctx& c) {
+template <int NOBS, int NMAX, int UNR = 1, class INV = NoInv>
+__device__ __forceinline__ double dual_infeasibility(double* sm, const Ctx& c, const INV inv = INV()) {
     using L = Lay<NOBS, NMAX>;
     const int N = c.N;
     int lane = c.lane;
@@ -406,7 +445,10 @@
     const int la = in ? lane : 0;
     double mcol[L::NX];
 #pragma unroll
-    for (int i = 0; i < L::NX; i++) mcol[i] = LD(L::M + i * L::NZ + la);
+    for (int i = 0; i < L::NX; i++) {
+        if constexpr (HasInv<INV>) mcol[i] = inv.mcol[i];
+        else mcol[i] = LD(L::M + i * L::NZ + la);
+    }
     tot = LD(L::ga + N * L::NZ + la);
     double gk = LD(L::ga + (N - 1) * L::NZ + la);
     LD(SINK(in, L::ga + N * L::NZ + lane)) = 0.0;
@@ -482,8 +524,8 @@
     return wave_sum(S);
 }
 
-template <int NOBS, int NMAX>
-__device__ __forceinline__ void assemble_newton(double* sm, const int* si, const Ctx& c, double mu) {
+template <int NOBS, int NMAX, class INV = NoInv>
+__device__ __forceinline__ void assemble_newton(double* sm, const int* si, const Ctx& c, double mu, const INV inv = INV()) {
     using L = Lay<NOBS, NMAX>;
     const int N = c.N;
     ROWS(j, jv, c.lane, c.m) {
@@ -493,7 +535,9 @@
         LD(L::rtt + j) = rti;
         if constexpr (!L::SLIM) {
             const double sig = nu * rti;
-            const bool on = LD(L::rsc + j) != 0.0;
+            bool on;
+            if constexpr (HasInv<INV>) on = inv.rsc[q_] != 0.0;
+            else on = LD(L::rsc + j) != 0.0;
             LD(L::rsig + j) = sel(on, sig, 0.0);
             const double cj = LD(L::rc + j);
             LD(L::rw + j) = sel(on, nu - mu * rti + sig * (cj - t), 0.0);
@@ -509,11 +553,14 @@
         const bool isx = a < 6, isu = a >= L::NX && a < L::NX + 2, iss0 = a >= 6 && a < L::NX, iss1 = a >= L::NX + 2;
         const int o = iss0 ? a - 6 : (iss1 ? a - L::NX - 2 : 0);
         double g = LD(L::ga + e);
-        const double cw = LD(L::cst + (isx ? a : (isu ? 6 + a - L::NX : 0)));
+        double cw;
+        if constexpr (HasInv<INV>) cw = inv.cw[q_];
+        else cw = LD(L::cst + (isx ? a : (isu ? 6 + a - L::NX : 0)));
         double h = sel(isx || isu, 2.0 * cw, 0.0);
         h += ((iss0 && k == 0 && o >= c.nobs) || (iss1 && o >= c.nobs)) ? 1.0 : 0.0;
         int rl, rh;
-        coord_rows<L>(si, c, e, k, a, rl, rh);
+        if constexpr (HasInv<INV>) { rl = inv.rl[q_]; rh = inv.rh[q_]; }
+        else coord_rows<L>(si, c, e, k, a, rl, rh);
         const int il = rl >= 0 ? rl : 0, ih = rh >= 0 ? rh : 0;
         double sgl, sgh, wl, wh;
         if constexpr (L::SLIM) {
@@ -1285,20 +1332,24 @@
 };
 
 template <int NFIX> constexpr int StageUnroll = NFIX == 0 ? 1 : NFIX;
+template <int SPEC> constexpr int SpecWaves = SPEC == 1 ? 2 : 1;
 template <int NOBS, int NMAX, int DEG = 0, int NFIX = 0, int SPEC = 0, int QPM = 0>
-__global__ void __launch_bounds__(WAVE * (1 + SPEC)) __attribute__((amdgpu_waves_per_eu(MinWaves<NOBS, NMAX>::v))) CRX_KERNEL_EXTRA_ATTR
+__global__ void __launch_bounds__(WAVE * SpecWaves<SPEC>) __attribute__((amdgpu_waves_per_eu(SPEC == 2 ? 1 : MinWaves<NOBS, NMAX>::v, SPEC == 2 ? 1 : 0))) CRX_KERNEL_EXTRA_ATTR
 crx_solve_kernel(const crx_kparams kp) {
     static_assert(NFIX <= NMAX, "fixed horizon inside the layout");
     using L = Lay<NOBS, NMAX>;
-    static_assert(!SPEC || (NOBS > 0 && !L::SLIM && CRX_STATIC_LDS), "the speculating wave exists for the obstacle instantiations of the full, static layout");
+    constexpr bool TWO = SPEC == 1, LONE = SPEC == 2;
+    static_assert(!TWO || (NOBS > 0 && !L::SLIM && CRX_STATIC_LDS), "the speculating wave exists for the obstacle instantiations of the full, static layout");
+    static_assert(!LONE || (NOBS > 0 && !L::SLIM && NFIX > 0 && NMAX * NOBS <= WAVE), "the lone-wave form exists for the tuned obstacle instantiations of the full layout");
+    using Inv = std::conditional_t<LONE, LoneInv<L>, NoInv>;
     constexpr int NX = L::NX, NZ = L::NZ, NR = L::NR;
 #if CRX_STATIC_LDS
-    __shared__ __attribute__((aligned(16))) double sm[((SPEC ? L::BYTES_SPEC : L::BYTES) + 7) / 8];
+    __shared__ __attribute__((aligned(16))) double sm[((TWO ? L::BYTES_SPEC : L::BYTES) + 7) / 8];
 #else
     extern __shared__ __attribute__((aligned(16))) double sm[];
 #endif
     int* si = (int*)(sm + L::END_D);
-    const int lane = SPEC ? (int)(threadIdx.x & (WAVE - 1)) : (int)threadIdx.x, N = NFIX ? NFIX : kp.N;
+    const int lane = TWO ? (int)(threadIdx.x & (WAVE - 1)) : (int)threadIdx.x, N = NFIX ? NFIX : kp.N;
     if ((int)blockIdx.x >= kp.batch) return;
     const int b = kp.order ? min(max(kp.order[blockIdx.x], 0), kp.batch - 1) : (int)blockIdx.x;
     if (kp.active && kp.active[kp.active_div > 1 ? b / kp.active_div : b] == 0) {
@@ -1320,7 +1371,7 @@
             return;
         }
     }
-    if constexpr (SPEC) {
+    if constexpr (TWO) {
         if (threadIdx.x >= WAVE) {
             Ctx c1 = {};
             c1.N = N; c1.lane = lane;
@@ -1790,6 +1841,30 @@
     }
     f = cost_value<NOBS, NMAX>(sm, c, 0.0);
     } else {
+    Inv inv;
+    if constexpr (LONE) {
+        const int ec = lane < N * NOBS ? lane : 0;
+        const int kc = ec / L::NO, oc = ec - kc * L::NO, N1 = N + 1;
+#pragma unroll
+        for (int a = 0; a < NZ; a++) { inv.m4[a] = LD(L::M + 4 * NZ + a); inv.m5[a] = LD(L::M + 5 * NZ + a); }
+#pragma unroll
+        for (int i = 0; i < NX; i++) inv.mcol[i] = LD(L::M + i * NZ + (lane < NZ ? lane : 0));
+        inv.rLs = LD(L::cst + 16 + oc); inv.rWs = LD(L::cst + 16 + L::NO + oc); inv.lap = LD(L::cst + 8 + oc);
+        inv.os0 = LD(L::obs_s + oc * N1 + kc); inv.oe0 = LD(L::obs_e + oc * N1 + kc);
+        inv.os1 = LD(L::obs_s + oc * N1 + kc + 1); inv.oe1 = LD(L::obs_e + oc * N1 + kc + 1);
+        inv.csc = cbf_scale<L>(sm, kc, oc);
+        ROWS(j, jv, lane, m) {
+            (void)jv;
+            inv.rsc[q_] = row_scale<L>(sm, si, j, N); inv.rb[q_] = row_bound<L>(sm, c, j); inv.riv[q_] = RIVT(si, j);
+        }
+        COORDS(e, ev, lane, N * NZ + NX) {
+            (void)ev;
+            const int k = e / NZ, a = e - k * NZ;
+            const bool isx = a < 6, isu = a >= NX && a < NX + 2;
+            inv.cw[q_] = LD(L::cst + (isx ? a : (isu ? 6 + a - NX : 0))); inv.xrv[q_] = LD(L::xr + k * 6 + (isx ? a : 0));
+            coord_rows<L>(si, c, e, k, a, inv.rl[q_], inv.rh[q_]);
+        }
+    }
     if (NOBS && crash) {
         double sc = 0.0;
         for (int j = lane; j < m; j += WAVE) sc += LD(L::rt + j) * LD(L::rnu + j);
@@ -1809,7 +1884,7 @@
         double e_c = cmax;
         const double sd = fmax(smax, nus / fmax(mact, 1.0)) / smax;
         long long tc1 = CLK();
-        const double e_du = dual_infeasibility<NOBS, NMAX, (StageUnroll<NFIX> > 2 ? StageUnroll<NFIX> : 1)>(sm, c);
+        const double e_du = dual_infeasibility<NOBS, NMAX, (StageUnroll<NFIX> > 2 ? StageUnroll<NFIX> : 1)>(sm, c, inv);
         const double e_d = e_du / sd;
         long long tc2 = CLK();
         e_c /= sd;
@@ -1839,20 +1914,20 @@
         }
         const double tau = ipm_tau(mu, o.tau_min);
         long long tc3 = CLK();
-        assemble_newton<NOBS, NMAX>(sm, si, c, mu);
+        assemble_newton<NOBS, NMAX>(sm, si, c, mu, inv);
         long long tc4 = CLK();
         double dw = 0.0;
         long long tsub[4] = {0, 0, 0, 0};
         bool ok;
         int used_convex = 0;
         if (NOBS && crash && cvx_run > 0 && (cvx_run % CVX_PROBE) != 0) {
-            if constexpr (!SPEC) {
+            if constexpr (!TWO) {
                 for (int k = lane; k < N; k += WAVE) { LD(L::kS + 2 * k) = 0.0; LD(L::kE + 2 * k) = 0.0; }
                 SYNC();
             }
             used_convex = 1;
         }
-        if constexpr (SPEC) {
+        if constexpr (TWO) {
             double sdw = 0.0;
             int cz = used_convex, avail = (crash && !used_convex) ? 1 : 0, tries = 0;
             for (;;) {
@@ -1923,8 +1998,10 @@
         };
         ROWS(j, jv, lane, m) {
             const bool simple = !ROW_IS_CBF(j, N);
-            const int pk = RIVT(si, j);
-            const double sc = row_scale<L>(sm, si, j, N), jd = RIV_SGN(pk) * LD(L::dZ + RIV_IDX(pk));
+            int pk; double sc;
+            if constexpr (LONE) { pk = inv.riv[q_]; sc = inv.rsc[q_]; }
+            else { pk = RIVT(si, j); sc = row_scale<L>(sm, si, j, N); }
+            const double jd = RIV_SGN(pk) * LD(L::dZ + RIV_IDX(pk));
             row_step(j, jv && simple, simple, sc, jd);
         }
         if (NOBS) {
@@ -1933,14 +2010,16 @@
                 double jc = 0.0;
 #pragma unroll
                 for (int a = 0; a < NZ; a++) jc += J[a] * LD(L::dZ + k * NZ + a);
-                row_step(j, ev, true, cbf_scale<L>(sm, k, ob), jc);
+                double sc;
+                if constexpr (LONE) sc = inv.csc; else sc = cbf_scale<L>(sm, k, ob);
+                row_step(j, ev, true, sc, jc);
             }
         }
         wave_max2(rp_max, rd_max);
         const double a_p = (rp_max > tau) ? tau / rp_max : 1.0;
         const double a_d = (rd_max > tau) ? tau / rd_max : 1.0;
         double cost_qq;
-        double cost_d = cost_dir<NOBS, NMAX>(sm, c, cost_qq);
+        double cost_d = cost_dir<NOBS, NMAX>(sm, c, cost_qq, inv);
         wave_sum4(theta, Dphi, cost_d, cost_qq);
         Dphi += cost_d;
         const double phi0 = f - mu * logsum_t;
@@ -1948,6 +2027,8 @@
         long long tc7 = CLK();
         double al = a_p, fn = f, lt_acc = logsum_t;
         int acc = 0, ftype = 0;
+        double cbf_trial = 0.0;
+        (void)cbf_trial;
         const bool sw_try = (theta <= theta_min) && (Dphi < 0.0);
         const double sw_gap = sw_try ? IPM_S_PHI * log2_fast(-Dphi) - IPM_S_THETA * log2_fast(theta) : 0.0;
         for (int ls = 0; ls < IPM_MAX_BACKTRACK && al >= IPM_ALPHA_MIN; ls++) {
@@ -1966,14 +2047,23 @@
             };
             ROWS(j, jv, lane, m) {
                 const bool simple = !ROW_IS_CBF(j, N);
-                const double sc = row_scale<L>(sm, si, j, N), t = LD(L::rt + j), dt = LD(L::rdt + j), cj = LD(L::rc + j);
+                double sc;
+                if constexpr (LONE) sc = inv.rsc[q_]; else sc = row_scale<L>(sm, si, j, N);
+                const double t = LD(L::rt + j), dt = LD(L::rdt + j), cj = LD(L::rc + j);
                 ROW_LOADS_DONE();
                 row_trial(j, jv && simple, simple, sc, cj + al * (dt - (cj - t)), t, dt);
             }
             if (NOBS) {
                 CBF_ROWS(j, k, ob, ev, lane, N) {
-                    const double sc = cbf_scale<L>(sm, k, ob), t = LD(L::rt + j), dt = LD(L::rdt + j);
-                    row_trial(j, ev, true, sc, sc * cbf_value<NOBS, NMAX>(sm, c, k, ob, al), t, dt);
+                    double sc;
+                    if constexpr (LONE) sc = inv.csc; else sc = cbf_scale<L>(sm, k, ob);
+                    const double t = LD(L::rt + j), dt = LD(L::rdt + j);
+                    if constexpr (LONE) {
+                        cbf_trial = cbf_value<NOBS, NMAX>(sm, c, k, ob, al, inv);
+                        row_trial(j, ev, true, sc, sc * cbf_trial, t, dt);
+                    } else {
+                        row_trial(j, ev, true, sc, sc * cbf_value<NOBS, NMAX>(sm, c, k, ob, al), t, dt);
+                    }
                 }
             }
             lt_acc = lg.wave_total_with(thn);
@@ -2046,14 +2136,19 @@
             LD(SINK(own, L::rc + j)) = sel(on, v, 1.0);
         };
         ROWS(j, jv, lane, m) {
-            const int pk = RIVT(si, j);
-            const double sc = row_scale<L>(sm, si, j, N), v = RIV_SGN(pk) * (LD(L::Z + RIV_IDX(pk)) - row_bound<L>(sm, c, j));
+            int pk; double sc, v;
+            if constexpr (LONE) { pk = inv.riv[q_]; sc = inv.rsc[q_]; v = RIV_SGN(pk) * (LD(L::Z + RIV_IDX(pk)) - inv.rb[q_]); }
+            else { pk = RIVT(si, j); sc = row_scale<L>(sm, si, j, N); v = RIV_SGN(pk) * (LD(L::Z + RIV_IDX(pk)) - row_bound<L>(sm, c, j)); }
             row_accept(j, jv && !ROW_IS_CBF(j, N), sc, v);
         }
         if (NOBS) {
             CBF_ROWS(j, k, ob, ev, lane, N) {
-                const double sc = cbf_scale<L>(sm, k, ob);
-                row_accept(j, ev, sc, sc * cbf_value<NOBS, NMAX>(sm, c, k, ob, 0.0));
+                if constexpr (LONE) {
+                    row_accept(j, ev, inv.csc, inv.csc * cbf_trial);
+                } else {
+                    const double sc = cbf_scale<L>(sm, k, ob);
+                    row_accept(j, ev, sc, sc * cbf_value<NOBS, NMAX>(sm, c, k, ob, 0.0));
+                }
             }
         }
         SYNC();
@@ -2064,7 +2159,7 @@
         }
         nus = wave_sum(nus);
         e_p = th;
-        first_order<NOBS, NMAX>(sm, si, c);
+        first_order<NOBS, NMAX>(sm, si, c, inv);
         if (kp.trace && b == kp.trace_problem && it < (kp.trace_rows < 0 ? -kp.trace_rows : kp.trace_rows) && lane == 0 && kp.trace_rows > 0)
             kp.trace[(size_t)it * 16 + 8] = (double)(tph[0] + (CLK() - tc8));
         if (numax > 1e12 && th > 1e-6) { status = CRX_STALLED; it++; break; }
@@ -2114,7 +2209,7 @@
     break;
     }
     }
-    if constexpr (SPEC) {
+    if constexpr (TWO) {
         if (lane == 0) LD(L::ctl) = 0.0;
         __syncthreads();
     }
@@ -2202,9 +2297,9 @@
         if (kp.opts.qp_method != 0) return launch_t<NOBS, NMAX, DEG, NFIX, SPEC, 1>(kp, st);
     }
 #if CRX_STATIC_LDS
-    hipLaunchKernelGGL((crx_solve_kernel<NOBS, NMAX, DEG, NFIX, SPEC, QPM>), dim3(kp.batch), dim3(WAVE * (1 + SPEC)), 0, st, kp);
+    hipLaunchKernelGGL((crx_solve_kernel<NOBS, NMAX, DEG, NFIX, SPEC, QPM>), dim3(kp.batch), dim3(WAVE * SpecWaves<SPEC>), 0, st, kp);
 #else
-    static_assert(SPEC == 0, "the two-wave instantiations are static-LDS kernels");
+    static_assert(SPEC == 0, "the two-wave and lone-wave instantiations are static-LDS kernels");
     const size_t bytes = Lay<NOBS, NMAX>::BYTES;
     static int attr_set_on = -1;
     int dev = -1;
@@ -2218,7 +2313,7 @@
 #endif
     return hipGetLastError();
 }
-template <int NOBS, int NMAX, int DEG, int NFIX>
+template <int NOBS, int NMAX, int DEG, int NFIX, int SPEC = 0>
 static int occ_t() {
     int n = 0;
 #if CRX_STATIC_LDS
@@ -2227,7 +2322,7 @@
     const size_t bytes = Lay<NOBS, NMAX>::BYTES;
     if (hipFuncSetAttribute((const void*)crx_solve_kernel<NOBS, NMAX, DEG, NFIX>, hipFuncAttributeMaxDynamicSharedMemorySize, (int)bytes) != hipSuccess) return -1;
 #endif
-    if (hipOccupancyMaxActiveBlocksPerMultiprocessor(&n, crx_solve_kernel<NOBS, NMAX, DEG, NFIX>, WAVE, bytes) != hipSuccess) return -1;
+    if (hipOccupancyMaxActiveBlocksPerMultiprocessor(&n, crx_solve_kernel<NOBS, NMAX, DEG, NFIX, SPEC>, WAVE * SpecWaves<SPEC>, bytes) != hipSuccess) return -1;
     return n;
 }
 
@@ -2278,6 +2373,15 @@
     if (kp.N == 10) return launch_t<1, 12, 6, 10, 1>(kp, st);
     return hipErrorInvalidValue;
 }
+#elif defined(CRX_TU_LONE)
+hipError_t crx_launch_solve_lone(const crx_kparams& kp, hipStream_t st) {
+    if (kp.batch == 0) return hipSuccess;
+    if (kp.degree != 6) return hipErrorInvalidValue;
+    if (kp.N == 12) return launch_t<1, 12, 6, 12, 2>(kp, st);
+    if (kp.N == 10) return launch_t<1, 12, 6, 10, 2>(kp, st);
+    return hipErrorInvalidValue;
+}
+int crx_solve_resident_per_cu_lone(int N) { return N == 12 ? occ_t<1, 12, 6, 12, 2>() : (N == 10 ? occ_t<1, 12, 6, 10, 2>() : -1); }
 #else
 #if CRX_TU_GENERAL
 #define CRX_UNIT(name) name##_general
diff --git a/car-racing_amd/csrc/crx_kernels_lone.hip b/car-racing_amd/csrc/crx_kernels_lone.hip
--- /dev/null
+++ b/car-racing_amd/csrc/crx_kernels_lone.hip
@@ -0,0 +1,3 @@
+#define CRX_TU_OBSTACLES 1
+#define CRX_TU_LONE 1
+#include "crx_kernels.hip"
diff --git a/car-racing_amd/csrc/crx_kparams.h b/car-racing_amd/csrc/crx_kparams.h
--- a/car-racing_amd/csrc/crx_kparams.h
+++ b/car-racing_amd/csrc/crx_kparams.h
@@ -128,6 +128,8 @@
 #include <hip/hip_runtime.h>
 hipError_t crx_launch_solve(const crx_kparams& kp, int nobs_template, hipStream_t st);
 hipError_t crx_launch_solve_spec(const crx_kparams& kp, hipStream_t st);
+hipError_t crx_launch_solve_lone(const crx_kparams& kp, hipStream_t st);
+int crx_solve_resident_per_cu_lone(int N);
 hipError_t crx_launch_select(const crx_select_kparams& sp, hipStream_t st);
 hipError_t crx_launch_debug_reduce(const double* in, double* out, hipStream_t st);
 hipError_t crx_launch_lmpc_addtraj(const crx_lmpcprep_desc& d, int batch, const int32_t* crossed, double* log_x, const double* log_u,
```

After: 611,400, median of 6. 1.04x the previous value.
